# sThalham/PyraPose

Measured on AMD Instinct MI355X. Metric: images/sec 640x480 fwd+bwd (train step: fwd + losses + bwd + clipnorm-Adam), higher is better.
Workload: dtype bf16x3+f16c8

## Files before the change

include/pyrapose_hip.h:

```cpp
#ifndef PYRAPOSE_HIP_H
#define PYRAPOSE_HIP_H

#include <stddef.h>
#include <stdint.h>

#ifdef __cplusplus
extern "C" {
#endif

#define PP_OK 0
#define PP_ERR_ARG (-1)
#define PP_ERR_SHAPE (-2)
#define PP_ERR_ALIGN (-3)
#define PP_ERR_NOCTX (-4)
#define PP_ERR_UNSUPPORTED (-5)
#define PP_ERR_COMM (-6)

#define PP_MAX_SEG 5

typedef struct pp_ctx pp_ctx;

int pp_ctx_create(pp_ctx** out, int device, void* hip_stream);
void pp_ctx_destroy(pp_ctx* ctx);
int pp_ctx_set_stream(pp_ctx* ctx, void* hip_stream);
int pp_ctx_set_workspace(pp_ctx* ctx, void* device_buffer, size_t bytes);
int pp_row_block_list(pp_ctx* ctx, const float* x, int rows, int ld, int cols, unsigned char* flags, int* list);
int pp_row_block_list_planes(pp_ctx* ctx, const void* x_hi, const void* x_lo, int rows, int ld, int cols, unsigned char* flags, int* list);
int pp_row_block_list_planes_within(pp_ctx* ctx, const void* x_hi, const void* x_lo, int rows, int ld, int cols, const unsigned char* within,
                                    unsigned char* flags, int* list);
const char* pp_last_error_string(pp_ctx* ctx);
const char* pp_version(void);
int pp_device_info(pp_ctx* ctx, int* n_cu, char* name_host, int name_len);

typedef struct {
  int n_img;
  int n_seg;
  int h[PP_MAX_SEG];
  int w[PP_MAX_SEG];
} pp_rowspace;

typedef struct {
  pp_rowspace in;
  pp_rowspace out;
  int cin, cout;
  int kh, kw, stride;
  int pad_t, pad_l;
  int ld_x, ld_y, ld_w;
} pp_conv_desc;

int pp_conv2d_nhwc_fwd(pp_ctx* ctx, const pp_conv_desc* d, const float* x, const float* w,
                       const float* bias, const float* residual, int ld_res, int relu, float* y);

int pp_conv2d_nhwc_bwd_data(pp_ctx* ctx, const pp_conv_desc* d, const float* dy, const float* w,
                            const float* addend, int ld_add, const float* relu_src, int ld_rs, float* dx);

int pp_conv2d_nhwc_bwd_weight(pp_ctx* ctx, const pp_conv_desc* d, const float* x, const float* dy,
                              float* dw, float* dbias);

int pp_conv_split_weights_bf16x3(pp_ctx* ctx, const pp_conv_desc* d, const float* w, void* fwd_hi, void* fwd_lo,
                                 void* dgrad_hi, void* dgrad_lo);
typedef struct pp_split_job {
  const float* w;
  void* fwd_hi; void* fwd_lo; void* dg_hi; void* dg_lo;
  int taps, cin, cout, ld_w;
  int tile_begin, reserved;
} pp_split_job;
int pp_conv_split_weights_bf16x3_batch(pp_ctx* ctx, int n_jobs, const pp_split_job* jobs_dev, int total_tiles);
int pp_positive_row_blocks(pp_ctx* ctx, const pp_rowspace* rs, int A, int stride, const float* y_true, unsigned char* flags);
int pp_row_block_dilate(pp_ctx* ctx, const pp_conv_desc* d, const unsigned char* in_flags, unsigned char* out_flags);
int pp_split_planes_bf16x3(pp_ctx* ctx, size_t n, const float* src, void* hi, void* lo);
int pp_ctx_set_planes_format(pp_ctx* ctx, int fmt);
int pp_convert_planes(pp_ctx* ctx, size_t n, const void* src_hi, const void* src_lo, int src_fmt, void* dst_hi, void* dst_lo, int dst_fmt,
                      const float* scale2_dev, int scale_index, const void* relu_src_hi);
int pp_grad_scale_from_counts(pp_ctx* ctx, const int* counts_dev, int n_counts, float* scale2_dev);
int pp_grad_scale_from_counts_adj(pp_ctx* ctx, const int* counts_dev, int n_counts, float* scale2_dev, int log2_adjust);
int pp_split_planes_scaled_bf16x3(pp_ctx* ctx, size_t n, const float* src, void* hi, void* lo, const float* scale_dev);
int pp_ctx_set_grad_scale(pp_ctx* ctx, const float* scale2_dev);

typedef struct pp_conv_opts {
  void* capture_hi;
  void* capture_lo;
  const void* add_hi;
  const void* add_lo;
  const void* mask_hi;
  unsigned char* skip_flags;
  int* skip_list;
  const unsigned char* out_flags;
  int* out_list;
  int lazy_out;
  int lazy_in;
} pp_conv_opts;
#ifdef __cplusplus
static_assert(sizeof(pp_conv_opts) == 9 * sizeof(void*) + 2 * sizeof(int), "pp_conv_opts: pointers, then ints, no padding");
#else
_Static_assert(sizeof(pp_conv_opts) == 9 * sizeof(void*) + 2 * sizeof(int), "pp_conv_opts: pointers, then ints, no padding");
#endif

int pp_conv2d_nhwc_fwd_bf16x3(pp_ctx* ctx, const pp_conv_desc* d, const float* x, const void* x_hi, const void* x_lo,
                              const void* w_fwd_hi, const void* w_fwd_lo, const float* bias, const float* residual,
                              int ld_res, int relu, float* y, void* y_hi, void* y_lo, const pp_conv_opts* opts);
int pp_conv2d_nhwc_bwd_data_bf16x3(pp_ctx* ctx, const pp_conv_desc* d, const float* dy, const void* dy_hi,
                                   const void* dy_lo, const void* w_dgrad_hi, const void* w_dgrad_lo,
                                   const float* addend, int ld_add, const float* relu_src, int ld_rs, float* dx,
                                   void* dx_hi, void* dx_lo, const pp_conv_opts* opts);
int pp_conv2d_nhwc_bwd_weight_bf16x3(pp_ctx* ctx, const pp_conv_desc* d, const float* x, const float* dy,
                                     const void* x_hi, const void* x_lo, const void* dy_hi, const void* dy_lo,
                                     float* dw, float* dbias, const pp_conv_opts* opts);

#define PP_PLAN_FWD 0
#define PP_PLAN_BWD_DATA 1
#define PP_PLAN_BWD_WEIGHT 2
#define PP_PLAN_PLANES_IN 1u
#define PP_PLAN_PLANES_OUT 2u
#define PP_PLAN_F32_OUT 4u
#define PP_PLAN_CAPTURE 8u
#define PP_PLAN_LIST 16u
#define PP_PLAN_LAZY_IN 32u
#define PP_PLAN_LAZY_OUT 64u
int pp_conv_plan_text(const pp_conv_desc* d, int pass, unsigned forms, int planes_fmt, int n_cu, size_t ws_bytes, char* buf,
                      int buf_bytes);

typedef struct pp_comm pp_comm;
int pp_comm_available(void);
int pp_comm_unique_id(pp_ctx* ctx, void* id128);
int pp_comm_init(pp_ctx* ctx, int world, int rank, const void* id128, pp_comm** out);
int pp_comm_destroy(pp_comm* comm);
int pp_allreduce_bucket(pp_ctx* ctx, pp_comm* comm, float* buf, size_t count);
int pp_allreduce_counts(pp_ctx* ctx, pp_comm* comm, int* counts, int n);

int pp_maxpool3x3s2_fwd(pp_ctx* ctx, int n_img, int h, int w, int c, const float* x, int oh, int ow, float* y);
int pp_upsample_nearest_add_fwd(pp_ctx* ctx, int n_img, int sh, int sw, int th, int tw, int c,
                                const float* src, const float* other, float* out);
int pp_upsample_nearest_add_bwd(pp_ctx* ctx, int n_img, int sh, int sw, int th, int tw, int c,
                                const float* dtarget, const float* base, float* dsrc);
int pp_add_n(pp_ctx* ctx, size_t n, const float* a, const float* b, const float* c, float* out);
int pp_relu_fwd(pp_ctx* ctx, size_t n, const float* x, float* y);
typedef struct pp_tview {
  const float* f32;
  const void* hi;
  const void* lo;
} pp_tview;
int pp_add_n_v(pp_ctx* ctx, size_t n, const pp_tview* a, const pp_tview* b, const pp_tview* c, const pp_tview* out);
int pp_relu_fwd_v(pp_ctx* ctx, size_t n, const pp_tview* x, const pp_tview* y);
int pp_upsample_nearest_add_fwd_v(pp_ctx* ctx, int n_img, int sh, int sw, int th, int tw, int c, const pp_tview* src,
                                  const pp_tview* other, const pp_tview* out);
int pp_upsample_nearest_add_bwd_v(pp_ctx* ctx, int n_img, int sh, int sw, int th, int tw, int c, const pp_tview* dtarget,
                                  const pp_tview* base, const pp_tview* dsrc);
int pp_merge_planes_bf16x3(pp_ctx* ctx, size_t n, const void* hi, const void* lo, float* dst);
int pp_planes_stats(pp_ctx* ctx, const void* hi, const void* lo, long long rows, int ld, int cols, const unsigned char* within,
                    unsigned long long* stats5_dev);
int pp_pack_rgb_to_4(pp_ctx* ctx, size_t n_pixels, const float* x3, float* x4);
int pp_preprocess_caffe_u8(pp_ctx* ctx, int n_img, int H, int W, const int* sizes_hw_host, const unsigned char* images_u8,
                           float* x4);
int pp_warp_affine_u8(pp_ctx* ctx, int n_img, int H, int W, int channels, const double* mats_host, int interpolation, int border,
                      int cval, const unsigned char* src, unsigned char* dst);
int pp_resize_scale(int rows, int cols, int min_side, int max_side, double* scale);
int pp_resize_linear_u8(pp_ctx* ctx, int n_img, int SH, int SW, int channels, double scale, int DH, int DW, const unsigned char* src,
                        unsigned char* dst);
enum { PP_PHOTO_NONE = 0, PP_PHOTO_LUT = 1, PP_PHOTO_GRAY = 2, PP_PHOTO_HUESAT = 3, PP_PHOTO_BLEND = 4, PP_PHOTO_CONV = 5, PP_PHOTO_MEDIAN = 6,
       PP_PHOTO_BILATERAL = 7 };
typedef struct pp_photo_op {
  int kind;
  int k;
  int off0, off1;
  float f0, f1;
} pp_photo_op;
size_t pp_photo_workspace_bytes(int n_img, int H, int W);
int pp_photo_augment_u8(pp_ctx* ctx, int n_img, int H, int W, int channels, const int* op_offsets_host, const pp_photo_op* ops_host,
                        const unsigned char* pool_host, size_t pool_bytes, const unsigned char* pool_dev, const unsigned char* src,
                        unsigned char* dst, void* workspace, size_t workspace_bytes);
int pp_pack_rgb_to_4_padded(pp_ctx* ctx, int n_img, int H, int W, int Hp, int Wp, int pad, const float* x3, float* x4p);
int pp_preprocess_caffe_u8_padded(pp_ctx* ctx, int n_img, int H, int W, int Hp, int Wp, int pad, const int* sizes_hw_host,
                                  const unsigned char* images_u8, float* x4p);
int pp_stem7x7s2_fwd_bf16x3(pp_ctx* ctx, int n_img, int H, int W, int Hp, int Wp, const float* x4p, const void* w_hi,
                            const void* w_lo, int cout, const float* bias, int relu, float* y, int ld_y);

int pp_export_head(pp_ctx* ctx, const pp_rowspace* rs, int n_anchor, int n_val, const float* src, int ld,
                   int apply_sigmoid, float* out);

int pp_count_positives(pp_ctx* ctx, size_t rows_box, const float* y_box, size_t rows_cls, int c_cls,
                       const float* y_cls, size_t rows_mask, int c_mask, const float* y_mask, int* counts);
int pp_sigmoid_focal_fwd_bwd(pp_ctx* ctx, const pp_rowspace* rs, int n_anchor, int n_class,
                             const float* logits, int ld, const float* y_true, float alpha, float gamma,
                             const int* count, float loss_weight, float* loss_sum, float* dlogits);
int pp_orth_smoothl1_fwd_bwd(pp_ctx* ctx, const pp_rowspace* rs, int n_anchor, const float* pred, int ld,
                             const float* y_true, float weight, float sigma, const int* count,
                             float loss_weight, float* loss_sum, float* dpred);

typedef struct {
  long long offset;
  long long count;
  int ld;
  int trainable;
  long long scale_off;
// ... 178 lines not shown
```

pyrapose_amd/_lib.py:

```python
import ctypes as C
import os

_HERE = os.path.dirname(os.path.abspath(__file__))
LIB_PATH = os.path.join(_HERE, os.environ.get("PP_LIB") or "libpyrapose_hip.so")

PP_MAX_SEG = 5


class RowSpace(C.Structure):
    _fields_ = [("n_img", C.c_int), ("n_seg", C.c_int), ("h", C.c_int * PP_MAX_SEG), ("w", C.c_int * PP_MAX_SEG)]

    @classmethod
    def make(cls, n_img, shapes):
        rs = cls()
        rs.n_img = int(n_img)
        rs.n_seg = len(shapes)
        for i, (h, w) in enumerate(shapes):
            rs.h[i] = int(h)
            rs.w[i] = int(w)
        return rs

    def rows(self):
        return sum(self.n_img * self.h[i] * self.w[i] for i in range(self.n_seg))

# ... 13 lines not shown


class SplitJob(C.Structure):
    _fields_ = [("w", C.c_void_p), ("fwd_hi", C.c_void_p), ("fwd_lo", C.c_void_p), ("dg_hi", C.c_void_p), ("dg_lo", C.c_void_p),
                ("taps", C.c_int), ("cin", C.c_int), ("cout", C.c_int), ("ld_w", C.c_int), ("tile_begin", C.c_int), ("reserved", C.c_int)]


class TView(C.Structure):
    _fields_ = [("f32", C.c_void_p), ("hi", C.c_void_p), ("lo", C.c_void_p)]


class ConvOpts(C.Structure):
    _fields_ = [("capture_hi", C.c_void_p), ("capture_lo", C.c_void_p), ("add_hi", C.c_void_p), ("add_lo", C.c_void_p),
                ("mask_hi", C.c_void_p), ("skip_flags", C.c_void_p), ("skip_list", C.c_void_p), ("out_flags", C.c_void_p),
                ("out_list", C.c_void_p), ("lazy_out", C.c_int), ("lazy_in", C.c_int)]


def _load():
    if not os.path.exists(LIB_PATH):
        raise ImportError(
            "pyrapose_amd: %s not found. Build it with `python -c 'import __graft_entry__ as g; g.build()'` "
            "or `make -C pyrapose_amd/csrc`. There is no CPU fallback." % LIB_PATH)
    try:
        return C.CDLL(LIB_PATH)
    except OSError as e:
        raise ImportError("pyrapose_amd: cannot load %s: %s" % (LIB_PATH, e))


lib = _load()
if hasattr(lib, "pp_ctx_set_split_capture"):
    raise ImportError("pyrapose_amd: %s predates pp_conv_opts (it still exports pp_ctx_set_split_capture): rebuild it" % LIB_PATH)

_p = C.c_void_p
_i = C.c_int
_f = C.c_float
_d = C.c_double
_ll = C.c_longlong
_sz = C.c_size_t

_SIGS = {
    "pp_ctx_create": (_i, [C.POINTER(_p), _i, _p]),
    "pp_ctx_destroy": (None, [_p]),
    "pp_ctx_set_stream": (_i, [_p, _p]),
    "pp_last_error_string": (C.c_char_p, [_p]),
    "pp_version": (C.c_char_p, []),
    "pp_device_info": (_i, [_p, C.POINTER(_i), C.c_char_p, _i]),
    "pp_conv2d_nhwc_fwd": (_i, [_p, C.POINTER(ConvDesc), _p, _p, _p, _p, _i, _i, _p]),
    "pp_conv2d_nhwc_bwd_data": (_i, [_p, C.POINTER(ConvDesc), _p, _p, _p, _i, _p, _i, _p]),
    "pp_conv2d_nhwc_bwd_weight": (_i, [_p, C.POINTER(ConvDesc), _p, _p, _p, _p]),
    "pp_conv_split_weights_bf16x3": (_i, [_p, C.POINTER(ConvDesc), _p, _p, _p, _p, _p]),
    "pp_split_planes_bf16x3": (_i, [_p, _sz, _p, _p, _p]),
    "pp_ctx_set_planes_format": (_i, [_p, _i]),
    "pp_convert_planes": (_i, [_p, _sz, _p, _p, _i, _p, _p, _i, _p, _i, _p]),
    "pp_split_planes_scaled_bf16x3": (_i, [_p, _sz, _p, _p, _p, _p]),
    "pp_grad_scale_from_counts": (_i, [_p, _p, _i, _p]),
    "pp_grad_scale_from_counts_adj": (_i, [_p, _p, _i, _p, _i]),
    "pp_ctx_set_grad_scale": (_i, [_p, _p]),
    "pp_planes_stats": (_i, [_p, _p, _p, _ll, _i, _i, _p, _p]),
    "pp_comm_available": (_i, []),
    "pp_comm_unique_id": (_i, [_p, _p]),
    "pp_comm_init": (_i, [_p, _i, _i, _p, C.POINTER(_p)]),
    "pp_comm_destroy": (_i, [_p]),
    "pp_allreduce_bucket": (_i, [_p, _p, _p, C.c_size_t]),
    "pp_allreduce_counts": (_i, [_p, _p, _p, _i]),
    "pp_ctx_set_workspace": (_i, [_p, _p, C.c_size_t]),
    "pp_row_block_list": (_i, [_p, _p, _i, _i, _i, _p, _p]),
    "pp_positive_row_blocks": (_i, [_p, _p, _i, _i, _p, _p]),
    "pp_row_block_dilate": (_i, [_p, _p, _p, _p]),
    "pp_row_block_list_planes": (_i, [_p, _p, _p, _i, _i, _i, _p, _p]),
    "pp_row_block_list_planes_within": (_i, [_p, _p, _p, _i, _i, _i, _p, _p, _p]),
    "pp_add_n_v": (_i, [_p, _sz, C.POINTER(TView), C.POINTER(TView), C.POINTER(TView), C.POINTER(TView)]),
    "pp_relu_fwd_v": (_i, [_p, _sz, C.POINTER(TView), C.POINTER(TView)]),
    "pp_upsample_nearest_add_fwd_v": (_i, [_p, _i, _i, _i, _i, _i, _i, C.POINTER(TView), C.POINTER(TView), C.POINTER(TView)]),
    "pp_upsample_nearest_add_bwd_v": (_i, [_p, _i, _i, _i, _i, _i, _i, C.POINTER(TView), C.POINTER(TView), C.POINTER(TView)]),
    "pp_merge_planes_bf16x3": (_i, [_p, _sz, _p, _p, _p]),
    "pp_warp_affine_u8": (_i, [_p, _i, _i, _i, _i, C.POINTER(_d), _i, _i, _i, _p, _p]),
    "pp_photo_workspace_bytes": (_sz, [_i, _i, _i]),
    "pp_photo_augment_u8": (_i, [_p, _i, _i, _i, _i, _p, _p, _p, _sz, _p, _p, _p, _p, _sz]),
    "pp_resize_scale": (_i, [_i, _i, _i, _i, C.POINTER(_d)]),
    "pp_resize_linear_u8": (_i, [_p, _i, _i, _i, _i, _d, _i, _i, _p, _p]),
    "pp_conv_split_weights_bf16x3_batch": (_i, [_p, _i, _p, _i]),
    "pp_conv2d_nhwc_fwd_bf16x3": (_i, [_p, C.POINTER(ConvDesc), _p, _p, _p, _p, _p, _p, _p, _i, _i, _p, _p, _p, C.POINTER(ConvOpts)]),
    "pp_conv2d_nhwc_bwd_data_bf16x3": (_i, [_p, C.POINTER(ConvDesc), _p, _p, _p, _p, _p, _p, _i, _p, _i, _p, _p, _p, C.POINTER(ConvOpts)]),
    "pp_conv2d_nhwc_bwd_weight_bf16x3": (_i, [_p, C.POINTER(ConvDesc), _p, _p, _p, _p, _p, _p, _p, _p, C.POINTER(ConvOpts)]),
    "pp_conv_plan_text": (_i, [C.POINTER(ConvDesc), _i, C.c_uint, _i, _i, _sz, C.c_char_p, _i]),
    "pp_maxpool3x3s2_fwd": (_i, [_p, _i, _i, _i, _i, _p, _i, _i, _p]),
    "pp_upsample_nearest_add_fwd": (_i, [_p, _i, _i, _i, _i, _i, _i, _p, _p, _p]),
    "pp_upsample_nearest_add_bwd": (_i, [_p, _i, _i, _i, _i, _i, _i, _p, _p, _p]),
    "pp_add_n": (_i, [_p, _sz, _p, _p, _p, _p]),
    "pp_relu_fwd": (_i, [_p, C.c_size_t, _p, _p]),
    "pp_preprocess_caffe_u8": (_i, [_p, _i, _i, _i, C.POINTER(C.c_int), _p, _p]),
    "pp_preprocess_caffe_u8_padded": (_i, [_p, _i, _i, _i, _i, _i, _i, C.POINTER(C.c_int), _p, _p]),
    "pp_pack_rgb_to_4_padded": (_i, [_p, _i, _i, _i, _i, _i, _i, _p, _p]),
    "pp_stem7x7s2_fwd_bf16x3": (_i, [_p, _i, _i, _i, _i, _i, _p, _p, _p, _i, _p, _i, _p, _i]),
    "pp_pack_rgb_to_4": (_i, [_p, _sz, _p, _p]),
    "pp_export_head": (_i, [_p, C.POINTER(RowSpace), _i, _i, _p, _i, _i, _p]),
    "pp_count_positives": (_i, [_p, _sz, _p, _sz, _i, _p, _sz, _i, _p, _p]),
    "pp_sigmoid_focal_fwd_bwd": (_i, [_p, C.POINTER(RowSpace), _i, _i, _p, _i, _p, _f, _f, _p, _f, _p, _p]),
    "pp_orth_smoothl1_fwd_bwd": (_i, [_p, C.POINTER(RowSpace), _i, _p, _i, _p, _f, _f, _p, _f, _p, _p]),
    "pp_optimizer_create": (_i, [_p, C.POINTER(_p), C.POINTER(ParamDesc), _i, _ll]),
    "pp_optimizer_destroy": (None, [_p]),
    "pp_grad_global_norm": (_i, [_p, _p, _p, _p, _p, _p, _p]),
    "pp_adam_step_clipnorm": (_i, [_p, _p, _p, _p, _p, _p, _p, _p, _p, _f, _f, _f, _f, _f, _ll]),
    "pp_generate_base_anchors_host": (_i, [_i, C.POINTER(_f), _i, C.POINTER(_f), _i, C.POINTER(_d)]),
    "pp_anchors_shift_f64": (_i, [_p, _i, C.POINTER(_i), C.POINTER(_i), C.POINTER(_i), _i, C.POINTER(_d), _p]),
    "pp_anchors_shift_f32": (_i, [_p, _i, C.POINTER(_i), C.POINTER(_i), C.POINTER(_i), _i, C.POINTER(_d), _p]),
    "pp_compute_overlap_f64": (_i, [_p, _i, _p, _i, _p, _p]),
    "pp_compute_gt_annotations": (_i, [_p, _i, _p, _i, _p, _d, _d, _p, _p]),
    "pp_anchor_targets": (_i, [_p, _i, _p, _i, C.POINTER(_i), _p, _p, _p, _p, _p, _i, _i, C.POINTER(_i), C.POINTER(_i), _i, _d, _d,
                               _i, _i, _p, _p, _p]),
    "pp_project_box3d_host": (_i, [C.POINTER(_d), C.POINTER(_d), C.POINTER(_d), C.POINTER(_d)]),
    "pp_pil_nearest_index_host": (_i, [_i, _i, C.POINTER(_i)]),
    "pp_box3d_decode": (_i, [_p, _i, _i, _p, _p, _p]),
    "pp_score_threshold_compact": (_i, [_p, _i, _i, _i, _p, _f, _i, _p, _p]),
    "pp_filter_workspace_bytes": (_sz, [_i, _i, _i]),
    "pp_pose_error_workspace_bytes": (_sz, [_i, _i]),
    "pp_filter_detections": (_i, [_p, _i, _i, _p, _p, _p, _f, _f, _i, _p, _p, _p, _p, _p]),
    "pp_pose_add_f64": (_i, [_p, _i, _i, _p, _p, _p, _p, _p, _p, _p]),
    "pp_pose_adi_f64": (_i, [_p, _i, _i, _p, _p, _p, _p, _p, _p, _p]),
    "pp_filter_detections_batch": (_i, [_p, _i, _i, _i, _p, _p, _p, _f, _f, _i, _p, _p, _p, _p, _p]),
    "pp_render_workspace_bytes": (_sz, [_i, _i, _i, _i, _i]),
    "pp_render_depth_f32": (_i, [_p, _i, _i, _p, _i, _p, _p, _p, _p, _i, _i, _d, _d, _p, _sz, _p]),
    "pp_render_rgbd_workspace_bytes": (_sz, [_i, _i, _i, _i, _i]),
    "pp_render_rgbd": (_i, [_p, _i, _i, _p, _p, _p, _i, _p, _p, _p, _p, _i, _i, _d, _d, _i, _d, C.POINTER(_d), C.POINTER(_d), _p, _sz,
                            _p, _p, _p, _p]),
    "pp_render_rgbd_tex_workspace_bytes": (_sz, [_i, _i, _i, _i, _i, _i, _i]),
    "pp_render_rgbd_tex": (_i, [_p, _i, _i, _p, _p, _p, _i, _i, _i, _i, _p, _i, _p, _p, _p, _p, _i, _i, _d, _d, _i, _d, C.POINTER(_d),
                                C.POINTER(_d), _p, _sz, _p, _p, _p, _p]),
    "pp_scene_compose_u8": (_i, [_p, _i, _i, C.POINTER(_i), _p, _i, _i, _p, _p, _p, C.POINTER(C.c_ubyte), _i, _p]),
    "pp_vsd_workspace_bytes": (_sz, [_i, _i, _i]),
    "pp_vsd_f64": (_i, [_p, _i, _i, _i, _p, _ll, _p, _p, _p, _d, _d, _i, _p, _p, _p, _p]),
    "pp_vsd_multi_workspace_bytes": (_sz, [_i, _i, _i, _i]),
    "pp_vsd_multi_f64": (_i, [_p, _i, _i, _i, _p, _ll, _p, _p, _p, _d, _i, C.POINTER(_d), _i, _i, _p, _p, _p, _p, _p, _p]),
    "pp_scene_gt_workspace_bytes": (_sz, [_i, _i, _i]),
    "pp_scene_gt_info": (_i, [_p, _i, _i, C.POINTER(_i), _p, _i, _i, _i, _i, _i, _i, _p, _p, _p, _ll, _d, _p, _sz, _p, _p, _p, _p, _p,
                              _p, _p]),
    "pp_pose_reproj_f64": (_i, [_p, _i, _i, _p, _p, _p, _p, _p, _p, _p, _p]),
    "pp_pose_sym_workspace_bytes": (_sz, [_i, _i, _i]),
    "pp_pose_mssd_f64": (_i, [_p, _i, _i, _i, _p, _p, _p, _p, _p, _p, _p, _p, _p, _p]),
    "pp_pose_mspd_f64": (_i, [_p, _i, _i, _i, _p, _p, _p, _p, _p, _p, _p, _p, _p, _p, _p]),
    "pp_pnp_ransac_workspace_bytes": (_sz, [_i, _i]),
    "pp_pnp_ransac_f64": (_i, [_p, _i, _p, _i, _p, _p, _p, _i, _d, C.c_ulonglong, _i, _p, _p, _p, _p, _p, _p]),
    "pp_cloud_from_depth_workspace_bytes": (_sz, [_i, _i]),
    "pp_cloud_from_depth_f64": (_i, [_p, _i, _i, _p, _p, _i, _i, _p, _p, _d, _d, _d, _d, _d, _i, _p, _p, _p]),
    "pp_voxel_workspace_bytes": (_sz, [_i]),
    "pp_voxel_keys_f64": (_i, [_p, _i, _p, _d, _p, _p]),
    "pp_voxel_means_f64": (_i, [_p, _i, _p, _p, _p, _i, _p, _p, _p]),
    "pp_estimate_normals_workspace_bytes": (_sz, [_i, _i]),
    "pp_estimate_normals_f64": (_i, [_p, _i, _p, _d, _i, _p, _p, _p]),
    "pp_icp_workspace_bytes": (_sz, [_i, _i]),
    "pp_icp_f64": (_i, [_p, _i, _p, _p, _i, _p, _p, _p, _p, _d, _i, _d, _d, _i, _p, _sz, _p, _p, _p, _p, _p, _p, _p]),
    "pp_vote_stats_workspace_bytes": (_sz, [_i, _i]),
    "pp_vote_stats_f64": (_i, [_p, _i, _p, _i, _p, _i, _p, _p, _i, _d, _p, _p, _p, _p, _p, _p, _p]),
    "pp_pnp_refine_weighted_workspace_bytes": (_sz, [_i, _i]),
    "pp_pnp_refine_weighted_f64": (_i, [_p, _i, _p, _i, _p, _p, _p, _p, _p, _p, _i, _d, _d, _d, _p, _p, _p, _p, _p, _p, _p, _p, _p]),
    "pp_vote_cluster_workspace_bytes": (_sz, [_i, _i, _i, _i]),
    "pp_vote_cluster": (_i, [_p, _i, _i, _i, _i, _p, _p, _p, _p, _d, _i, _i, _i, _p, _p, _p, _p, _p, _p, _p]),
    "pp_pts_diameter_workspace_bytes": (_sz, [_i]),
    "pp_pts_diameter_f64": (_i, [_p, _i, _p, _p, _sz, _p, _p]),
    "pp_farthest_points_workspace_bytes": (_sz, [_i]),
    "pp_farthest_points_f64": (_i, [_p, _i, _i, _p, C.POINTER(_i), _p, _i, _i, _p, _p, _p, _sz, _p]),
    "pp_det_match": (_i, [_p, _i, _i, _i, _i, _p, _p, _p, _p, _p, _p, C.POINTER(_i), _p, _i, C.POINTER(_d), _i, _p, _p, _p]),
    "pp_det_pr_curve": (_i, [_p, _i, _i, _i, _ll, _p, _p, _p, _p, _p, _p, _p, _p, _p]),
    "pp_det_ap": (_i, [_p, _i, _i, _i, _p, _p, _p, _p, _i, _p, _p]),
}

# ... 26 lines not shown
```

pyrapose_amd/csrc/conv3.hip:

```cpp
#include "conv_common.h"
#include "conv4.h"

#define PP_CAT_(a, b) a##b
#define PP_CAT(a, b) PP_CAT_(a, b)
#if PP_FMT == 1
#define PP_API(name) PP_CAT(name, _fmt1)
#else
#define PP_API(name) PP_CAT(name, _fmt0)
#endif
namespace {
#include "planes_fmt.h"

#include "conv3_shared.h"

#ifndef PP_EPI_GF
#define PP_EPI_GF 4
#endif

template <int TM, int TN, bool AP, bool OP>
__global__ __launch_bounds__(256, (TM * TN >= 8) ? 2 : ((TM * TN == 4) ? 3 : 4)) void igemm3_kernel(
    const IgemmParams p, const float* __restrict__ g_src, const uint4* __restrict__ g_ahi, const uint4* __restrict__ g_alo,
    const uint4* __restrict__ g_whi, const uint4* __restrict__ g_wlo,
    const float* __restrict__ g_bias, const float* __restrict__ g_addend, const float* __restrict__ g_mask,
    float* __restrict__ g_out, uint2* __restrict__ g_ohi, uint2* __restrict__ g_olo, int w_rows, int w_ld8) {
// ... 48 lines not shown
        ra[i][1] = s4[1];
      } else {
        ra[i][0] = make_float4(0.f, 0.f, 0.f, 0.f);
        ra[i][1] = make_float4(0.f, 0.f, 0.f, 0.f);
      }
    }
#pragma unroll
    for (int i = 0; i < TN; ++i) {
      const int n = n0 + r0 + 64 * i;
      if (n < w_rows) {
        const long long off = ((long long)tap * w_rows + n) * w_ld8 + (red0 >> 3) + oct;
        rbh[i] = g_whi[off];
        rbl[i] = g_wlo[off];
      } else {
        rbh[i] = make_uint4(0u, 0u, 0u, 0u);
        rbl[i] = make_uint4(0u, 0u, 0u, 0u);
      }
    }
  };
  auto advance = [&]() {
    red0 += BK;
    if (red0 >= p.Cred) {
      red0 = 0;
      ++tap;
      ++tx;
      if (tx == p.kw) { tx = 0; ++ty; }
      set_tap();
    }
  };
  auto store_step = [&]() {
#pragma unroll
    for (int i = 0; i < TM; ++i) {
      uint4 hi, lo;
      if (AP) {
        hi = rah[i];
        lo = ral[i];
      } else {
        split8(ra[i][0], ra[i][1], &hi, &lo);
      }
      const int slot = oct * BM + ((r0 + 64 * i + 2 * oct) & (BM - 1));
      Ahi[slot] = hi;
      Alo[slot] = lo;
    }
#pragma unroll
    for (int i = 0; i < TN; ++i) {
      const int slot = oct * BN + ((r0 + 64 * i + 2 * oct) & (BN - 1));
      Bhi[slot] = rbh[i];
      Blo[slot] = rbl[i];
    }
  };

  floatx16 acc[TM][TN];
#pragma unroll
  for (int a = 0; a < TM; ++a)
#pragma unroll
    for (int b = 0; b < TN; ++b)
#pragma unroll
      for (int r = 0; r < 16; ++r) acc[a][b][r] = 0.f;

  const int il = lane & 31, h = lane >> 5;

  set_tap();
  load_step();
  store_step();
  __syncthreads();

  for (int step = 0; step < n_steps; ++step) {
    const bool more = step + 1 < n_steps;
    if (more) {
      advance();
      load_step();
    }
    mma_step<TM, TN, BM, BN, 0>(acc, Ahi, Alo, Bhi, Blo, wm * 32 * TM + il, wn * 32 * TN + il, h);
    __syncthreads();
    if (more) {
      store_step();
      __syncthreads();
    }
  }

  epilogue3<TM, TN, OP>(p, acc, smem, m0, n0, tid, wm, wn, il, h, g_bias, g_addend, g_mask, g_out, g_ohi, g_olo);
}

template <int TM, int TN, bool AP, bool OP, bool SC = false, bool RL = false>
__global__ __launch_bounds__(256, (TM * TN >= 8) ? 2 : ((TM * TN == 4) ? 3 : 4)) void igemm3f_kernel(
    const IgemmParams p, const void* __restrict__ g_a0, const void* __restrict__ g_a1, unsigned a_bytes,
    const void* __restrict__ g_whi, const void* __restrict__ g_wlo, unsigned w_bytes,
    const float* __restrict__ g_bias, const float* __restrict__ g_addend, const float* __restrict__ g_mask,
    float* __restrict__ g_out, uint2* __restrict__ g_ohi, uint2* __restrict__ g_olo, int w_rows, int w_ld8, int splits,
    float* __restrict__ g_ws, const int* __restrict__ g_rl = nullptr, const unsigned char* __restrict__ g_srcflags = nullptr) {
  constexpr int BM = 64 * TM, BN = 64 * TN, BK = 32, NO = BK / 8;
  constexpr int SMEM_U4 = 2 * NO * (BM + BN);
  constexpr int ES = 4;
  __shared__ __attribute__((aligned(16))) uint4 smem[SMEM_U4];
  uint4* Ahi = smem;
  uint4* Alo = Ahi + NO * BM;
  uint4* Bhi = Alo + NO * BM;
  uint4* Blo = Bhi + NO * BN;

  const int tid = threadIdx.x, lane = tid & 63, wave = tid >> 6;
  const int wm = wave >> 1, wn = wave & 1;
  int n_wg = (int)gridDim.x;
  if (RL) {
    n_wg = ((g_rl[0] + BM / 32 - 1) / (BM / 32)) * p.n_tiles_n * splits;
    if ((int)blockIdx.x >= n_wg) return;
  }
  const int lbs = xcd_remap((int)blockIdx.x, n_wg);
  const int split = lbs % splits, lb = lbs / splits;
  const int tile_n = lb % p.n_tiles_n, tile_m = lb / p.n_tiles_n;
  const int m0 = tile_m * BM, n0 = tile_n * BN;
  int rl_blk[BM / 32];
  if (RL) {
    const int count = g_rl[0];
#pragma unroll
    for (int j = 0; j < BM / 32; ++j) {
      const int e = tile_m * (BM / 32) + j;
      rl_blk[j] = e < count ? g_rl[1 + e] * 32 : ((p.M + 31) & ~31);
    }
  }
  const int oct = tid & 3, r0 = tid >> 2;
  const int n_taps = p.kh * p.kw;
  const int steps_per_tap = p.Cred / BK;
  const int all_steps = n_taps * steps_per_tap;
  const int s_begin = (int)((long long)all_steps * split / splits), s_end = (int)((long long)all_steps * (split + 1) / splits);

  const __amdgpu_buffer_rsrc_t rs_a0 = __builtin_amdgcn_make_buffer_rsrc(const_cast<void*>(g_a0), 0, a_bytes, 0x00020000);
  const __amdgpu_buffer_rsrc_t rs_a1 = __builtin_amdgcn_make_buffer_rsrc(const_cast<void*>(AP ? g_a1 : g_a0), 0, AP ? a_bytes - 16 : a_bytes, 0x00020000);
  const __amdgpu_buffer_rsrc_t rs_wh = __builtin_amdgcn_make_buffer_rsrc(const_cast<void*>(g_whi), 0, w_bytes, 0x00020000);
  const __amdgpu_buffer_rsrc_t rs_wl = __builtin_amdgcn_make_buffer_rsrc(const_cast<void*>(g_wlo), 0, w_bytes, 0x00020000);

  int a_base[TM], a_pitch[TM];
  unsigned a_valid[TM];
#pragma unroll
  for (int i = 0; i < TM; ++i) {
    const int t_row = r0 + 64 * i;
    const RowPos r = decode_row(p, RL ? rl_blk[t_row >> 5] + (t_row & 31) : m0 + t_row);
    a_base[i] = ((r.rowbase + r.ybase * r.SW + r.xbase) * p.ld_src + 8 * oct) * ES;
    a_pitch[i] = p.tsign * r.SW * p.ld_src * ES;
    unsigned v = 0;
    int t = 0;
    for (int ty = 0; ty < p.kh; ++ty)
      for (int tx = 0; tx < p.kw; ++tx, ++t) {
        const int sy = r.ybase + ty * p.tsign, sx = r.xbase + tx * p.tsign;
        bool ok = r.ok && (unsigned)sy < (unsigned)r.SH && (unsigned)sx < (unsigned)r.SW;
        if (RL && g_srcflags && ok) ok = g_srcflags[(r.rowbase + sy * r.SW + sx) >> 5] != 0;
        if (ok) v |= 1u << t;
      }
    a_valid[i] = v;
  }
  const int x_pitch = p.tsign * p.ld_src * ES;
  int b_base[TN];
#pragma unroll
  for (int i = 0; i < TN; ++i) {
    const int n = n0 + r0 + 64 * i;
    b_base[i] = n < w_rows ? (n * w_ld8 + oct) * 16 : PP_BUF_OOB;
  }
  const int b_tap = w_rows * w_ld8 * 16;

  float4 ra[TM][2];
  uint4 rah[TM], ral[TM];
  uint4 rbh[TN], rbl[TN];
  int tap = s_begin / steps_per_tap, red0 = (s_begin - tap * steps_per_tap) * BK;
  int ty = tap / p.kw, tx = tap - ty * p.kw;

  auto load_step = [&]() {
    const int a_uni = tx * x_pitch + red0 * ES;
#pragma unroll
    for (int i = 0; i < TM; ++i) {
      int vo = a_base[i] + __mul24(ty, a_pitch[i]) + a_uni;
      vo = ((a_valid[i] >> tap) & 1u) ? vo : PP_BUF_OOB;
      if (AP) {
        rah[i] = buf_load16(rs_a0, vo, 0);
        ral[i] = buf_load16(rs_a1, vo, 0);
      } else {
        const uint4 q0 = buf_load16(rs_a0, vo, 0), q1 = buf_load16(rs_a0, vo + 16, 0);
        ra[i][0] = *reinterpret_cast<const float4*>(&q0);
        ra[i][1] = *reinterpret_cast<const float4*>(&q1);
      }
    }
    const int b_uni = ((p.w_ty0 + p.w_tstep * ty) * p.w_kw + p.w_tx0 + p.w_tstep * tx) * b_tap + (red0 >> 3) * 16;
#pragma unroll
    for (int i = 0; i < TN; ++i) {
      rbh[i] = buf_load16(rs_wh, b_base[i], b_uni);
      rbl[i] = buf_load16(rs_wl, b_base[i], b_uni);
    }
  };
  auto advance = [&](bool more) {
    red0 += BK;
    const bool wrap = red0 >= p.Cred;
    red0 = wrap ? 0 : red0;
    tap += wrap ? 1 : 0;
    tx += wrap ? 1 : 0;
    const bool wx = tx == p.kw;
    tx = wx ? 0 : tx;
    ty += wx ? 1 : 0;
    red0 = more ? red0 : 0;
    tap = more ? tap : 0;
    tx = more ? tx : 0;
    ty = more ? ty : 0;
  };
  auto split_step = [&]() {
    if (!AP) {
#pragma unroll
      for (int i = 0; i < TM; ++i) split8(ra[i][0], ra[i][1], &rah[i], &ral[i]);
    }
  };
  auto store_step = [&]() {
#pragma unroll
    for (int i = 0; i < TM; ++i) {
      const int slot = oct * BM + ((r0 + 64 * i + 2 * oct) & (BM - 1));
      Ahi[slot] = rah[i];
      Alo[slot] = ral[i];
    }
#pragma unroll
    for (int i = 0; i < TN; ++i) {
      const int slot = oct * BN + ((r0 + 64 * i + 2 * oct) & (BN - 1));
      Bhi[slot] = rbh[i];
      Blo[slot] = rbl[i];
    }
  };

  floatx16 acc[TM][TN];
#pragma unroll
  for (int a = 0; a < TM; ++a)
#pragma unroll
    for (int b = 0; b < TN; ++b)
#pragma unroll
      for (int r = 0; r < 16; ++r) acc[a][b][r] = 0.f;

  const int il = lane & 31, h = lane >> 5;

  load_step();
  split_step();
  store_step();
  __syncthreads();

  for (int step = s_begin; step < s_end; ++step) {
    advance(step + 1 < s_end);
    load_step();
    __builtin_amdgcn_sched_barrier(0);
    mma_step<TM, TN, BM, BN, 2>(acc, Ahi, Alo, Bhi, Blo, wm * 32 * TM + il, wn * 32 * TN + il, h);
    split_step();
    __syncthreads();
    store_step();
    __syncthreads();
  }
  if (splits > 1) {
    float* slice = g_ws + (long long)split * (RL ? (((long long)p.M + 31) & ~31ll) : (long long)p.M) * p.ld_out;
#pragma unroll
    for (int a = 0; a < TM; ++a)
#pragma unroll
      for (int r = 0; r < 16; ++r) {
        const int trow = wm * 32 * TM + a * 32 + (r & 3) + 8 * (r >> 2) + 4 * h;
        const int m = m0 + trow;
        const bool row_ok = RL ? (rl_blk[trow >> 5] < p.M) : (m < p.M);
#pragma unroll
        for (int b = 0; b < TN; ++b) {
          const int co = n0 + wn * 32 * TN + b * 32 + il;
          if (row_ok && co < ((p.Nout + 3) & ~3)) slice[(long long)m * p.ld_out + co] = acc[a][b][r];
        }
      }
    return;
  }
  epilogue3<TM, TN, OP, PP_EPI_GF, SC, false, RL>(p, acc, smem, m0, n0, tid, wm, wn, il, h, g_bias, g_addend, g_mask, g_out, g_ohi, g_olo, rl_blk);
}

template <int TM, int TN, bool CAP, bool AP = false, bool OP = false>
__global__ __launch_bounds__(256, (TM * TN >= 8) ? 2 : ((TM * TN == 4) ? 3 : 4)) void igemm3x_kernel(
    const IgemmParams p, const void* __restrict__ g_a, const void* __restrict__ g_a1, unsigned a_bytes, const void* __restrict__ g_whi,
    const void* __restrict__ g_wlo, unsigned w_bytes, const float* __restrict__ g_bias, const float* __restrict__ g_addend,
    const float* __restrict__ g_mask, float* __restrict__ g_out, uint2* __restrict__ g_ohi, uint2* __restrict__ g_olo, int w_rows, int w_ld8,
    int splits, float* __restrict__ g_ws, void* __restrict__ g_chi, void* __restrict__ g_clo, const unsigned char* __restrict__ g_flags,
    int skip_halo) {
  static_assert(!(CAP && AP), "split capture is for f32 operands");
  constexpr int ES = 4;
  constexpr int BM = 64 * TM, BN = 64 * TN, BK = 32, NO = BK / 8;
  constexpr int AP1 = NO * BM + 1;
  constexpr int SMEM_U4 = 2 * AP1 + 2 * NO * BN;
  __shared__ __attribute__((aligned(16))) uint4 smem[SMEM_U4];
  uint4* Ahi = smem;
  uint4* Alo = Ahi + AP1;
  uint4* Bhi = Alo + AP1;
  uint4* Blo = Bhi + NO * BN;

  const int tid = threadIdx.x, lane = tid & 63, wave = tid >> 6;
  const int wm = wave >> 1, wn = wave & 1;
  const int lbs = xcd_remap((int)blockIdx.x, (int)gridDim.x);
  const int split = lbs % splits, lb = lbs / splits;
  const int tile_n = lb % p.n_tiles_n, tile_m = lb / p.n_tiles_n;
  const int m0 = p.m_off + tile_m * (BM - 2) - 1, n0 = tile_n * BN;
  const int oct = tid & 3, r0 = tid >> 2;
  const int il = lane & 31, h = lane >> 5;
  const int n_chunks = p.Cred / BK;
  const int all_groups = p.kh * n_chunks;
  const int g_begin = (int)((long long)all_groups * split / splits);
  int g_end = (int)((long long)all_groups * (split + 1) / splits);
  if (g_flags) {
    int lo = m0 - skip_halo, hi = m0 + BM - 1 + skip_halo;
    lo = lo < 0 ? 0 : lo;
    hi = hi > p.M - 1 ? p.M - 1 : hi;
    int any = 0;
    for (int b = lo >> 5; b <= (hi >> 5); ++b) any |= g_flags[b];
    g_end = any ? g_end : g_begin;
  }

  const __amdgpu_buffer_rsrc_t rs_a = __builtin_amdgcn_make_buffer_rsrc(const_cast<void*>(g_a), 0, a_bytes, 0x00020000);
  const __amdgpu_buffer_rsrc_t rs_a1 = __builtin_amdgcn_make_buffer_rsrc(const_cast<void*>(AP ? g_a1 : g_a), 0, AP ? a_bytes - 16 : a_bytes, 0x00020000);
  const __amdgpu_buffer_rsrc_t rs_wh = __builtin_amdgcn_make_buffer_rsrc(const_cast<void*>(g_whi), 0, w_bytes, 0x00020000);
  const __amdgpu_buffer_rsrc_t rs_wl = __builtin_amdgcn_make_buffer_rsrc(const_cast<void*>(g_wlo), 0, w_bytes, 0x00020000);

  int s_base[TM], s_pitch[TM];
#pragma unroll
  for (int i = 0; i < TM; ++i) {
    const int q = m0 + r0 + 64 * i;
    const RowPos r = decode_row(p, q < 0 ? 0 : q);
    const bool ok = q >= 0 && r.ok;
    const int x = r.xbase - p.off_x;
    s_base[i] = ((r.rowbase + r.ybase * r.SW + x) * p.ld_src + 8 * oct) * ES;
    int v = 0;
    for (int ty = 0; ty < p.kh; ++ty)
      if (ok && (unsigned)(r.ybase + ty * p.tsign) < (unsigned)r.SH) v |= 1 << ty;
    s_pitch[i] = (p.tsign * r.SW * p.ld_src * ES) | v;
  }
  unsigned f_valid[(TM + 1) / 2];
#pragma unroll
  for (int a = 0; a < (TM + 1) / 2; ++a) f_valid[a] = 0;
#pragma unroll
  for (int a = 0; a < TM; ++a) {
    const int q = m0 + wm * 32 * TM + a * 32 + il;
    const RowPos r = decode_row(p, q < 0 ? 0 : q);
    unsigned v = 0;
    int t = 0;
    for (int ty = 0; ty < p.kh; ++ty)
      for (int tx = 0; tx < 3; ++tx, ++t) {
        const int sy = r.ybase + ty * p.tsign, sx = r.xbase + tx * p.tsign;
        if (q >= 0 && r.ok && (unsigned)sy < (unsigned)r.SH && (unsigned)sx < (unsigned)r.SW) v |= 1u << t;
      }
    f_valid[a >> 1] |= v << (16 * (a & 1));
  }
  int b_base[TN];
#pragma unroll
  for (int i = 0; i < TN; ++i) {
    const int n = n0 + r0 + 64 * i;
    b_base[i] = n < w_rows ? (n * w_ld8 + oct) * 16 : PP_BUF_OOB;
  }
  const int b_tap = w_rows * w_ld8 * 16;

// ... 819 lines not shown
      break;
    case PP_IGEMM4X:
      if constexpr (TM == 2 && TN == 2) {
        auto go4 = [&](auto v) {
          hipLaunchKernelGGL((igemm4x_kernel<true, decltype(v)::value>), grid, dim3(512), 0, st, p, a.ahi, a.alo, a_bytes, a.whi, a.wlo, w_bytes, p.bias,
                             p.addend, p.mask_src, p.out, (uint2*)a.ohi, (uint2*)a.olo, a.w_rows, a.w_ld8);
        };
        if (pl.variant == 0) go4(std::integral_constant<int, 0>{});
        else if (pl.variant == 2) go4(std::integral_constant<int, 2>{});
        else if (pl.variant == 3) go4(std::integral_constant<int, 3>{});
        else if (pl.variant == 4) go4(std::integral_constant<int, 4>{});
        else if (pl.variant == 9) go4(std::integral_constant<int, 9>{});
        else go4(std::integral_constant<int, 1>{});
        if (pl.tail_splits > 1) {
          IgemmParams q = p;
          q.m_off = pl.tail_m_off;
          hipLaunchKernelGGL((igemm3x_kernel<TM, TN, false, true, false>), dim3(pl.tail_grid), wg, 0, st, q, a.ahi, a.alo, a_bytes, a.whi, a.wlo, w_bytes,
                             q.bias, q.addend, q.mask_src, q.out, no_hi, no_lo, a.w_rows, a.w_ld8, pl.tail_splits, a.ws, nullptr, nullptr,
                             (const unsigned char*)nullptr, pl.skip_halo);
          launch_splitk_finish(st, q, pl.tail_splits, a.ws, pl.finish_blocks, a.ohi, a.olo);
        }
      }
      return;
    case PP_IGEMM4X2:
      if constexpr (TM == 2 && TN == 2)
        hipLaunchKernelGGL((igemm4x_kernel<true, 1, 2>), grid, wg, 0, st, p, a.ahi, a.alo, a_bytes, a.whi, a.wlo, w_bytes, p.bias, p.addend, p.mask_src,
                           p.out, (uint2*)a.ohi, (uint2*)a.olo, a.w_rows, a.w_ld8);
      return;
    case PP_IGEMM4P:
      if constexpr (TM == 2 && TN == 2)
        PP_API(pp4_launch_igemm4p)(st, p, a.ahi, a.whi, a.wlo, a.w_rows, a.w_ld8, a.ohi, a.olo, splits, ws, pl.grid, pl.stages);
      break;
    case PP_IGEMM3X_PP:
      hipLaunchKernelGGL((igemm3x_kernel<TM, TN, false, true, true>), grid, wg, 0, st, p, a.ahi, a.alo, a_bytes, a.whi, a.wlo, w_bytes, p.bias, p.addend,
                         p.mask_src, p.out, (uint2*)a.ohi, (uint2*)a.olo, a.w_rows, a.w_ld8, splits, ws, nullptr, nullptr, a.flags, pl.skip_halo);
      break;
    case PP_IGEMM3X_PF:
      hipLaunchKernelGGL((igemm3x_kernel<TM, TN, false, true, false>), grid, wg, 0, st, p, a.ahi, a.alo, a_bytes, a.whi, a.wlo, w_bytes, p.bias, p.addend,
                         p.mask_src, p.out, no_hi, no_lo, a.w_rows, a.w_ld8, splits, ws, nullptr, nullptr, a.flags, pl.skip_halo);
      break;
    case PP_IGEMM3X_FP:
      if constexpr (TM <= 2)
        hipLaunchKernelGGL((igemm3x_kernel<TM, TN, false, false, true>), grid, wg, 0, st, p, (const void*)p.src, nullptr, a_bytes, a.whi, a.wlo, w_bytes,
                           p.bias, p.addend, p.mask_src, p.out, (uint2*)a.ohi, (uint2*)a.olo, a.w_rows, a.w_ld8, splits, ws, nullptr, nullptr, a.flags,
                           pl.skip_halo);
      break;
    case PP_IGEMM3X_FF:
      if constexpr (TM <= 2)
        hipLaunchKernelGGL((igemm3x_kernel<TM, TN, false>), grid, wg, 0, st, p, (const void*)p.src, nullptr, a_bytes, a.whi, a.wlo, w_bytes, p.bias,
                           p.addend, p.mask_src, p.out, no_hi, no_lo, a.w_rows, a.w_ld8, splits, ws, nullptr, nullptr, a.flags, pl.skip_halo);
      break;
    default: {
      void *const ohi = splits > 1 ? nullptr : a.ohi, *const olo = splits > 1 ? nullptr : a.olo;
      auto go = [&](auto ap, auto op) {
        constexpr bool AP = decltype(ap)::value, OP = decltype(op)::value;
        if (pl.family == PP_IGEMM3F)
          hipLaunchKernelGGL((igemm3f_kernel<TM, TN, AP, OP>), grid, wg, 0, st, p, AP ? a.ahi : (const void*)p.src, AP ? a.alo : nullptr, a_bytes, a.whi,
                             a.wlo, w_bytes, p.bias, p.addend, p.mask_src, p.out, (uint2*)ohi, (uint2*)olo, a.w_rows, a.w_ld8, splits, ws);
        else
          hipLaunchKernelGGL((igemm3_kernel<TM, TN, AP, OP>), grid, wg, 0, st, p, p.src, (const uint4*)(AP ? a.ahi : nullptr),
                             (const uint4*)(AP ? a.alo : nullptr), (const uint4*)a.whi, (const uint4*)a.wlo, p.bias, p.addend, p.mask_src, p.out,
                             (uint2*)ohi, (uint2*)olo, a.w_rows, a.w_ld8);
      };
      if (a.ahi && ohi) go(std::true_type{}, std::true_type{});
      else if (a.ahi) go(std::true_type{}, std::false_type{});
      else if (ohi) go(std::false_type{}, std::true_type{});
      else go(std::false_type{}, std::false_type{});
    }
  }
  if (pl.finish_blocks) launch_splitk_finish(st, p, splits, a.ws, pl.finish_blocks, a.ohi, a.olo);
}

static void dispatch3(pp_ctx* ctx, IgemmParams& p, const Igemm3Args& a) {
  const PpIgemmFacts f = igemm3_facts(ctx, p, a);
  const PpIgemmPlan pl = pp_plan_igemm(f);
  pp_plan_debug(f, pl);
  if (pl.tm == 4) launch_igemm3<4, 2>(ctx->stream, p, a, pl);
  else if (pl.tm == 2 && pl.tn == 2) launch_igemm3<2, 2>(ctx->stream, p, a, pl);
  else if (pl.tm == 1 && pl.tn == 2) launch_igemm3<1, 2>(ctx->stream, p, a, pl);
  else if (pl.tm == 2 && pl.tn == 1) launch_igemm3<2, 1>(ctx->stream, p, a, pl);
  else launch_igemm3<1, 1>(ctx->stream, p, a, pl);
}

static void dispatch3_rowlist(pp_ctx* ctx, IgemmParams& p, const Igemm3Args& a, int tm, const unsigned char* dy_flags, unsigned char* out_flags,
                              int* out_list, bool fill) {
  PpIgemmFacts f = igemm3_facts(ctx, p, a);
  f.listed = true;
  f.listed_tm = tm;
  const PpIgemmPlan pl = pp_plan_igemm(f);
  if (tm == 2) launch_igemm3_rowlist<2, 2>(ctx->stream, p, a, pl, dy_flags, out_flags, out_list, fill);
  else launch_igemm3_rowlist<1, 2>(ctx->stream, p, a, pl, dy_flags, out_flags, out_list, fill);
}


}
extern "C" int PP_API(pp_conv2d_nhwc_fwd_bf16x3)(pp_ctx* ctx, const pp_conv_desc* d, const float* x, const void* x_hi, const void* x_lo,
                                         const void* w_hi, const void* w_lo, const float* bias, const float* residual, int ld_res,
                                         int relu, float* y, void* y_hi, void* y_lo, const pp_conv_opts* opts) {
  PP_REQUIRE_CTX(ctx);
  int rc = pp_conv_opts_take(ctx, opts, PP_OPT_CAPTURE | PP_OPT_ADD | PP_OPT_OUT, "pp_conv2d_nhwc_fwd_bf16x3");
  if (rc) return rc;
  void *const chi = opts->capture_hi, *const clo = opts->capture_lo;
  const void *const ep_ah = opts->add_hi, *const ep_al = opts->add_lo;
  rc = check_desc(ctx, d, "pp_conv2d_nhwc_fwd_bf16x3");
  PP_CHECK_ARG(ctx, !(ep_ah && residual), PP_ERR_ARG, "pp_conv2d_nhwc_fwd_bf16x3: residual given both as f32 and as planes");
  PP_CHECK_ARG(ctx, !ep_ah || (ld_res % 4 == 0 && ld_res >= ((d->cout + 3) & ~3)), PP_ERR_SHAPE, "pp_conv2d_nhwc_fwd_bf16x3: residual planes");
  if (rc) return rc;
  PP_CHECK_ARG(ctx, !chi || (x && !x_hi && pp_is_packed(chi, clo)), PP_ERR_ARG, "pp_conv2d_nhwc_fwd_bf16x3: split capture needs the f32 operand");
  PP_CHECK_ARG(ctx, (x || (x_hi && x_lo)) && w_hi && w_lo && (y || (y_hi && y_lo)), PP_ERR_ARG, "pp_conv2d_nhwc_fwd_bf16x3: null tensor");
  PP_CHECK_ARG(ctx, (x_hi == nullptr) == (x_lo == nullptr), PP_ERR_ARG, "pp_conv2d_nhwc_fwd_bf16x3: x_hi and x_lo go together");
  PP_CHECK_ARG(ctx, d->cin % 32 == 0 && d->ld_x % 8 == 0, PP_ERR_SHAPE, "pp_conv2d_nhwc_fwd_bf16x3: cin %d must be a multiple of 32, ld_x of 8", d->cin);
  PP_CHECK_ARG(ctx, pp_is_packed(x_hi, x_lo) && pp_is_packed(y_hi, y_lo), PP_ERR_ALIGN,
               "pp_conv2d_nhwc_fwd_bf16x3: planes must be packed (lo = hi + 16 bytes, 16-byte aligned)");
  PP_CHECK_ARG(ctx, !y_hi || (d->cout % 8 == 0 && d->ld_y % 8 == 0), PP_ERR_SHAPE, "pp_conv2d_nhwc_fwd_bf16x3: output planes need cout, ld_y %% 8 == 0");
  PP_CHECK_ARG(ctx, !ep_ah || (ld_res % 8 == 0 && d->cout % 8 == 0), PP_ERR_SHAPE, "pp_conv2d_nhwc_fwd_bf16x3: residual planes need cout, ld_res %% 8 == 0");
  PP_CHECK_ARG(ctx, (!x || pp_is_aligned16(x)) && pp_is_aligned16(w_hi) && pp_is_aligned16(w_lo) && (!y || pp_is_aligned16(y)), PP_ERR_ALIGN,
               "pp_conv2d_nhwc_fwd_bf16x3: tensors must be 16-byte aligned");
  PP_CHECK_ARG(ctx, !residual || (ld_res % 4 == 0 && ld_res >= ((d->cout + 3) & ~3) && pp_is_aligned16(residual)), PP_ERR_SHAPE,
               "pp_conv2d_nhwc_fwd_bf16x3: residual");
  PP_CHECK_ARG(ctx, !bias || pp_is_aligned16(bias), PP_ERR_ALIGN, "pp_conv2d_nhwc_fwd_bf16x3: bias alignment");
  IgemmParams p;
  memset(&p, 0, sizeof(p));
  p.src = x; p.out = y; p.bias = bias; p.addend = residual; p.mask_src = nullptr;
  p.add_hi = ep_ah; p.add_lo = ep_al;
  igemm_geometry_fwd(ctx, d, p);
  p.ld_add = ld_res; p.ld_mask = 0;
  p.relu = relu;
  PP_CHECK_ARG(ctx, (y_hi == nullptr) == (y_lo == nullptr) && (!y_hi || (d->ld_y % 4 == 0 && pp_is_aligned16(y_hi) && pp_is_aligned16(y_lo))),
               PP_ERR_ARG, "pp_conv2d_nhwc_fwd_bf16x3: output planes");
  const Igemm3Args a = {x_hi, x_lo, w_hi, w_lo, d->cout, d->cin / 8, y_hi, y_lo, chi, clo, nullptr, ctx->ws};
  if (opts->out_flags) {
    const bool ok = fwd_listed_ok(d, igemm3_facts(ctx, p, a), residual != nullptr || ep_ah != nullptr);
    PP_CHECK_ARG(ctx, ok, PP_ERR_SHAPE, "pp_conv2d_nhwc_fwd_bf16x3: out_flags needs a 3x3 stride-1 'same' conv on plane-stored input");
    dispatch3_rowlist(ctx, p, a, 2, nullptr, const_cast<unsigned char*>(opts->out_flags) ,
                      opts->out_list, false);
    PP_CHECK_LAUNCH(ctx, "pp_conv2d_nhwc_fwd_bf16x3");
    return PP_OK;
  }
  dispatch3(ctx, p, a);
  PP_CHECK_LAUNCH(ctx, "pp_conv2d_nhwc_fwd_bf16x3");
  return PP_OK;
}
namespace {

}
extern "C" int PP_API(pp_row_block_dilate)(pp_ctx* ctx, const pp_conv_desc* d, const unsigned char* in_flags, unsigned char* out_flags) {
  PP_REQUIRE_CTX(ctx);
  int rc = check_desc(ctx, d, "pp_row_block_dilate");
  if (rc) return rc;
  PP_CHECK_ARG(ctx, in_flags && out_flags && in_flags != out_flags, PP_ERR_ARG, "pp_row_block_dilate: two distinct flag buffers");
  IgemmParams p;
  memset(&p, 0, sizeof(p));
  p.n_seg = d->in.n_seg;
  fill_segs(ctx, d, true, p.seg, &p.M, &p.src_rows);
  const bool same = d->stride == 1 && d->kh == 3 && d->kw == 3 && segs_same_grid(p.seg, p.n_seg);
  PP_CHECK_ARG(ctx, same, PP_ERR_SHAPE, "pp_row_block_dilate: 3x3 stride-1 conv on an unchanged grid");
  const int nb = (p.M + 31) / 32;
  hipLaunchKernelGGL(rl_dilate_kernel, dim3((unsigned)((nb + 255) / 256)), dim3(256), 0, ctx->stream, p, in_flags, out_flags, nb);
  PP_CHECK_LAUNCH(ctx, "pp_row_block_dilate");
  return PP_OK;
}
namespace {

}
extern "C" int PP_API(pp_stem7x7s2_fwd_bf16x3)(pp_ctx* ctx, int n_img, int H, int W, int Hp, int Wp, const float* x4p, const void* w_hi,
                                       const void* w_lo, int cout, const float* bias, int relu, float* y, int ld_y) {
  PP_REQUIRE_CTX(ctx);
  PP_CHECK_ARG(ctx, x4p && w_hi && w_lo && y && pp_is_aligned16(x4p) && pp_is_aligned16(y) && pp_is_aligned16(w_hi) && pp_is_aligned16(w_lo),
               PP_ERR_ARG, "pp_stem7x7s2_fwd_bf16x3: null / unaligned tensor");
  PP_CHECK_ARG(ctx, n_img > 0 && H > 0 && W > 0 && Hp >= H + 6 && Wp >= W + 8 && Wp % 2 == 0 && cout > 0 && ld_y % 4 == 0 && ld_y >= ((cout + 3) & ~3),
               PP_ERR_SHAPE, "pp_stem7x7s2_fwd_bf16x3: bad geometry");
  const int OH = (H + 6 - 7) / 2 + 1, OW = (W + 6 - 7) / 2 + 1;
  IgemmParams p;
  memset(&p, 0, sizeof(p));
  p.src = x4p; p.out = y; p.bias = bias;
  p.ld_src = 4; p.ld_out = ld_y;
  p.relu = relu;
  p.n_seg = 1;
  p.seg[0].row_begin = 0; p.seg[0].src_row_begin = 0;
  p.seg[0].OH = OH; p.seg[0].OW = OW; p.seg[0].SH = Hp; p.seg[0].SW = Wp;
  p.M = n_img * OH * OW;
  p.src_rows = (long long)n_img * Hp * Wp;
  p.Cred = 32; p.Nout = cout; p.w_tap_rows = 32;
  p.kh = 7; p.kw = 1;
  p.mul = 2; p.tsign = 1; p.off_y = 0; p.off_x = 0; p.div = 1;
  p.w_ty0 = 0; p.w_tx0 = 0; p.w_tstep = 1; p.w_kw = 1; p.w_taps = 7;
  const Igemm3Args a = {nullptr, nullptr, w_hi, w_lo, cout, 4, nullptr, nullptr, nullptr, nullptr, nullptr, ctx->ws};
  PP_CHECK_ARG(ctx, pp_igemm_fast_ok(igemm3_facts(ctx, p, a)), PP_ERR_SHAPE, "pp_stem7x7s2_fwd_bf16x3: frame too large for 31-bit offsets");
  dispatch3(ctx, p, a);
  PP_CHECK_LAUNCH(ctx, "pp_stem7x7s2_fwd_bf16x3");
  return PP_OK;
}
namespace {

}
extern "C" int PP_API(pp_conv2d_nhwc_bwd_data_bf16x3)(pp_ctx* ctx, const pp_conv_desc* d, const float* dy, const void* dy_hi, const void* dy_lo,
                                              const void* w_hi, const void* w_lo, const float* addend, int ld_add,
                                              const float* relu_src, int ld_rs, float* dx, void* dx_hi, void* dx_lo,
                                              const pp_conv_opts* opts) {
  PP_REQUIRE_CTX(ctx);
  int rc = pp_conv_opts_take(ctx, opts, PP_OPT_CAPTURE | PP_OPT_ADD | PP_OPT_MASK | PP_OPT_SKIP | PP_OPT_LAZY_OUT | PP_OPT_LAZY_IN,
                             "pp_conv2d_nhwc_bwd_data_bf16x3");
  if (rc) return rc;
  void *const chi = opts->capture_hi, *const clo = opts->capture_lo;
  unsigned char* const skip_flags = opts->skip_flags;
  const bool skip_scratch_ok = skip_flags != nullptr && opts->skip_list != nullptr;
  const void *const ep_ah = opts->add_hi, *const ep_al = opts->add_lo, *const ep_mh = opts->mask_hi;
  rc = check_desc(ctx, d, "pp_conv2d_nhwc_bwd_data_bf16x3");
  PP_CHECK_ARG(ctx, !(ep_ah && addend) && !(ep_mh && relu_src), PP_ERR_ARG,
               "pp_conv2d_nhwc_bwd_data_bf16x3: addend / relu_src given both as f32 and as planes");
  PP_CHECK_ARG(ctx, (!ep_ah || (ld_add >= d->cin && ld_add % 4 == 0)) && (!ep_mh || (ld_rs >= d->cin && ld_rs % 4 == 0)), PP_ERR_SHAPE,
               "pp_conv2d_nhwc_bwd_data_bf16x3: addend / relu_src planes");
  if (rc) return rc;
  PP_CHECK_ARG(ctx, !chi || (dy && !dy_hi && pp_is_packed(chi, clo)), PP_ERR_ARG, "pp_conv2d_nhwc_bwd_data_bf16x3: split capture needs the f32 operand");
  PP_CHECK_ARG(ctx, (dy || (dy_hi && dy_lo)) && w_hi && w_lo && (dx || (dx_hi && dx_lo)), PP_ERR_ARG, "pp_conv2d_nhwc_bwd_data_bf16x3: null tensor");
  PP_CHECK_ARG(ctx, (dy_hi == nullptr) == (dy_lo == nullptr) && d->ld_y % 8 == 0, PP_ERR_ARG, "pp_conv2d_nhwc_bwd_data_bf16x3: planes / ld_y");
  PP_CHECK_ARG(ctx, pp_is_packed(dy_hi, dy_lo) && pp_is_packed(dx_hi, dx_lo), PP_ERR_ALIGN,
               "pp_conv2d_nhwc_bwd_data_bf16x3: planes must be packed (lo = hi + 16 bytes, 16-byte aligned)");
  PP_CHECK_ARG(ctx, (!dx_hi || (d->cin % 8 == 0 && d->ld_x % 8 == 0)) && (!ep_ah || ld_add % 8 == 0) && (!ep_mh || ld_rs % 8 == 0), PP_ERR_SHAPE,
               "pp_conv2d_nhwc_bwd_data_bf16x3: planes need channel counts and leading dimensions %% 8 == 0");
  const int cred = (d->cout + 31) / 32 * 32;
  PP_CHECK_ARG(ctx, d->cin % 16 == 0 && d->ld_y >= cred && d->ld_y % 4 == 0, PP_ERR_SHAPE,
               "pp_conv2d_nhwc_bwd_data_bf16x3: dy needs ld_y >= %d (cout rounded up to 32, zero padded)", cred);
  PP_CHECK_ARG(ctx, (!dy || pp_is_aligned16(dy)) && pp_is_aligned16(w_hi) && pp_is_aligned16(w_lo) && (!dx || pp_is_aligned16(dx)), PP_ERR_ALIGN,
               "pp_conv2d_nhwc_bwd_data_bf16x3: tensors must be 16-byte aligned");
  PP_CHECK_ARG(ctx, (!addend || (ld_add >= d->cin && ld_add % 4 == 0 && pp_is_aligned16(addend))) &&
                        (!relu_src || (ld_rs >= d->cin && ld_rs % 4 == 0 && pp_is_aligned16(relu_src))),
               PP_ERR_SHAPE, "pp_conv2d_nhwc_bwd_data_bf16x3: addend / relu_src");
  IgemmParams p;
  memset(&p, 0, sizeof(p));
  p.src = dy; p.out = dx; p.bias = nullptr; p.addend = addend; p.mask_src = relu_src;
  p.add_hi = ep_ah; p.add_lo = ep_al; p.mask_hi = ep_mh;
  igemm_geometry_bwd_data(ctx, d, p);
  p.ld_add = ld_add; p.ld_mask = ld_rs;
  p.relu = 0;
  PP_CHECK_ARG(ctx, (dx_hi == nullptr) == (dx_lo == nullptr) && (!dx_hi || (d->ld_x % 4 == 0 && pp_is_aligned16(dx_hi) && pp_is_aligned16(dx_lo))),
               PP_ERR_ARG, "pp_conv2d_nhwc_bwd_data_bf16x3: output planes");
  const Igemm3Args a = {dy_hi, dy_lo, w_hi, w_lo, d->cin, cred / 8, dx_hi, dx_lo, chi, clo, skip_flags, ctx->ws};
  DgradRoute route;
  dgrad_route(d, p, igemm3_facts(ctx, p, a), skip_scratch_ok, &route);
  PP_CHECK_ARG(ctx, !opts->lazy_in || route.listed, PP_ERR_ARG,
               "pp_conv2d_nhwc_bwd_data_bf16x3: dy was declared lazy (unwritten outside its flagged blocks) but the listed-block launch "
               "does not apply to this call");
  const int nb = (p.M + 31) / 32;
  if (skip_scratch_ok && !route.listed) PP_HIP(ctx, hipMemsetAsync(skip_flags + nb, 1, (size_t)nb, ctx->stream));
  const Igemm3Args ac = {dy_hi, dy_lo, w_hi, w_lo, d->cin, cred / 8, dx_hi, dx_lo, nullptr, nullptr, nullptr, ctx->ws};
  if (route.classes && chi) split_capture_pass(ctx->stream, p, chi, clo);
  dgrad_launches(
      route, p,
      [&](IgemmParams& q, bool is_class, bool listed) {
        if (listed) dispatch3_rowlist(ctx, q, a, route.listed_tm, skip_flags, skip_flags + nb, opts->skip_list + nb + 1, !opts->lazy_out);
        else dispatch3(ctx, q, is_class ? ac : a);
      },
      [&](IgemmParams& q) {
        hipLaunchKernelGGL(class_fill_kernel, dim3(pp_finish_blocks(q.M, q.Nout, pp_cus(ctx->n_cu))), dim3(256), 0, ctx->stream, q, addend, relu_src,
                           dx, dx_hi, dx_lo);
      });
  PP_CHECK_LAUNCH(ctx, "pp_conv2d_nhwc_bwd_data_bf16x3");
  return PP_OK;
}
namespace {

typedef short shortx4 __attribute__((ext_vector_type(4)));


template <int TM, int TN, bool AP>
__global__ __launch_bounds__(256, (TM * TN == 4) ? 2 : 3) void wgrad3_kernel(const Wgrad3Params p, const float* __restrict__ g_src,
                                                                            const float* __restrict__ g_dy,
                                                                            const uint4* __restrict__ g_xhi, const uint4* __restrict__ g_xlo,
                                                                            const uint4* __restrict__ g_dhi, const uint4* __restrict__ g_dlo,
                                                                            float* __restrict__ g_dw, float* __restrict__ g_dbias) {
  constexpr int BM = 64 * TM, BN = 64 * TN, BK = 32;
  constexpr int PA = BM + 32, PB = BN + 32;
  __shared__ __attribute__((aligned(16))) unsigned short smem[2 * BK * (PA + PB)];
  unsigned short* Xhi = smem;
  unsigned short* Xlo = Xhi + BK * PA;
  unsigned short* Ghi = Xlo + BK * PA;
  unsigned short* Glo = Ghi + BK * PB;

  const int tid = threadIdx.x, lane = tid & 63, wave = tid >> 6;
  const float inv_g = p.inv_scale ? *p.inv_scale : 1.f;
  const int wm = wave >> 1, wn = wave & 1;
  int b = xcd_remap((int)blockIdx.x, (int)gridDim.x);
  const int tile_n = b % p.n_tiles_n;
  b /= p.n_tiles_n;
  const int tile_k = b % p.n_tiles_k;
  const int split = b / p.n_tiles_k;
  const int tap = tile_k / p.k_tiles_per_tap;
  const int ci0 = (tile_k - tap * p.k_tiles_per_tap) * BM;
  const int ty = tap / p.kw, tx = tap - ty * p.kw;
  const int n0 = tile_n * BN;
  const int m_begin = split * p.rows_per_split;
  const int m_end = min(p.M, m_begin + p.rows_per_split);
  const int n_steps = (m_end - m_begin + BK - 1) / BK;

  const int prow = tid >> 3, q8 = tid & 7;
  constexpr int QA = BM / 32, QB = BN / 32;
  struct WRow { int m, n, y, x, seg_end, sb, OH, OW, SH, SW; } w;
  auto decode = [&](int m) {
    w.m = m;
    int rbeg = p.seg[0].row_begin;
    w.sb = p.seg[0].src_row_begin; w.OH = p.seg[0].OH; w.OW = p.seg[0].OW; w.SH = p.seg[0].SH; w.SW = p.seg[0].SW;
    w.seg_end = p.n_seg > 1 ? p.seg[1].row_begin : p.M;
    for (int s = 1; s < p.n_seg; ++s) {
      if (m >= p.seg[s].row_begin) {
        rbeg = p.seg[s].row_begin; w.sb = p.seg[s].src_row_begin; w.OH = p.seg[s].OH; w.OW = p.seg[s].OW;
        w.SH = p.seg[s].SH; w.SW = p.seg[s].SW;
        w.seg_end = (s + 1 < p.n_seg) ? p.seg[s + 1].row_begin : p.M;
      }
    }
    const int local = m < p.M ? m - rbeg : 0;
    const int hw = w.OH * w.OW;
    w.n = local / hw;
    const int rem = local - w.n * hw;
    w.y = rem / w.OW;
    w.x = rem - w.y * w.OW;
  };
  decode(m_begin + prow);

  constexpr int OA = (BM / 64 > 0) ? BM / 64 : 1, OB = (BN / 64 > 0) ? BN / 64 : 1;
  float4 ra[QA], rb[QB];
  uint4 pah[OA], pal[OA], pbh[OB], pbl[OB];
  float4 bsum[QB];
#pragma unroll
  for (int j = 0; j < QB; ++j) bsum[j] = make_float4(0.f, 0.f, 0.f, 0.f);
  const bool do_bias = (g_dbias != nullptr) && (tile_k == 0);

  auto load_step = [&]() {
    const int sy = w.y * p.stride + ty - p.pad_t;
    const int sx = w.x * p.stride + tx - p.pad_l;
    const bool in_rng = w.m < m_end;
    const bool ok = in_rng && ((unsigned)sy < (unsigned)w.SH) && ((unsigned)sx < (unsigned)w.SW);
    const long long xrow = (long long)(w.sb + w.n * w.SH * w.SW + sy * w.SW + sx) * p.ld_src + ci0;
    if (AP) {
#pragma unroll
      for (int j = 0; j < OA; ++j) {
        const long long o8 = 2 * ((xrow >> 3) + q8 + 8 * j);
        pah[j] = ok ? g_xhi[o8] : make_uint4(0u, 0u, 0u, 0u);
        pal[j] = ok ? g_xlo[o8] : make_uint4(0u, 0u, 0u, 0u);
      }
#pragma unroll
      for (int j = 0; j < OB; ++j) {
// ... 501 lines not shown
```

pyrapose_amd/csrc/conv3_dispatch.hip:

```cpp
#include "conv_common.h"

extern "C" int pp_row_block_list_fmt0(pp_ctx* ctx, const float* x, int rows, int ld, int cols, unsigned char* flags, int* list);
extern "C" int pp_row_block_list_fmt1(pp_ctx* ctx, const float* x, int rows, int ld, int cols, unsigned char* flags, int* list);
extern "C" int pp_row_block_list_planes_within_fmt0(pp_ctx* ctx, const void* x_hi, const void* x_lo, int rows, int ld, int cols, const unsigned char* within, unsigned char* flags, int* list);
extern "C" int pp_row_block_list_planes_within_fmt1(pp_ctx* ctx, const void* x_hi, const void* x_lo, int rows, int ld, int cols, const unsigned char* within, unsigned char* flags, int* list);
extern "C" int pp_row_block_list_planes_fmt0(pp_ctx* ctx, const void* x_hi, const void* x_lo, int rows, int ld, int cols, unsigned char* flags, int* list);
extern "C" int pp_row_block_list_planes_fmt1(pp_ctx* ctx, const void* x_hi, const void* x_lo, int rows, int ld, int cols, unsigned char* flags, int* list);
extern "C" int pp_split_planes_bf16x3_fmt0(pp_ctx* ctx, size_t n, const float* src, void* hi, void* lo);
extern "C" int pp_split_planes_bf16x3_fmt1(pp_ctx* ctx, size_t n, const float* src, void* hi, void* lo);
extern "C" int pp_split_planes_scaled_bf16x3_fmt0(pp_ctx* ctx, size_t n, const float* src, void* hi, void* lo, const float* scale_dev);
extern "C" int pp_split_planes_scaled_bf16x3_fmt1(pp_ctx* ctx, size_t n, const float* src, void* hi, void* lo, const float* scale_dev);
extern "C" int pp_grad_scale_from_counts_fmt0(pp_ctx* ctx, const int* counts_dev, int n_counts, float* scale2_dev);
extern "C" int pp_grad_scale_from_counts_adj_fmt0(pp_ctx* ctx, const int* counts_dev, int n_counts, float* scale2_dev, int log2_adjust);
extern "C" int pp_grad_scale_from_counts_adj_fmt1(pp_ctx* ctx, const int* counts_dev, int n_counts, float* scale2_dev, int log2_adjust);
extern "C" int pp_grad_scale_from_counts_fmt1(pp_ctx* ctx, const int* counts_dev, int n_counts, float* scale2_dev);
extern "C" int pp_conv_split_weights_bf16x3_batch_fmt0(pp_ctx* ctx, int n_jobs, const pp_split_job* jobs_dev, int total_tiles);
extern "C" int pp_conv_split_weights_bf16x3_batch_fmt1(pp_ctx* ctx, int n_jobs, const pp_split_job* jobs_dev, int total_tiles);
extern "C" int pp_conv_split_weights_bf16x3_fmt0(pp_ctx* ctx, const pp_conv_desc* d, const float* w, void* fwd_hi, void* fwd_lo, void* dgrad_hi, void* dgrad_lo);
extern "C" int pp_conv_split_weights_bf16x3_fmt1(pp_ctx* ctx, const pp_conv_desc* d, const float* w, void* fwd_hi, void* fwd_lo, void* dgrad_hi, void* dgrad_lo);
extern "C" int pp_conv2d_nhwc_fwd_bf16x3_fmt0(pp_ctx* ctx, const pp_conv_desc* d, const float* x, const void* x_hi, const void* x_lo, const void* w_fwd_hi, const void* w_fwd_lo, const float* bias, const float* residual, int ld_res, int relu, float* y, void* y_hi, void* y_lo, const pp_conv_opts* opts);
extern "C" int pp_conv2d_nhwc_fwd_bf16x3_fmt1(pp_ctx* ctx, const pp_conv_desc* d, const float* x, const void* x_hi, const void* x_lo, const void* w_fwd_hi, const void* w_fwd_lo, const float* bias, const float* residual, int ld_res, int relu, float* y, void* y_hi, void* y_lo, const pp_conv_opts* opts);
extern "C" int pp_row_block_dilate_fmt0(pp_ctx* ctx, const pp_conv_desc* d, const unsigned char* in_flags, unsigned char* out_flags);
extern "C" int pp_row_block_dilate_fmt1(pp_ctx* ctx, const pp_conv_desc* d, const unsigned char* in_flags, unsigned char* out_flags);
extern "C" int pp_stem7x7s2_fwd_bf16x3_fmt0(pp_ctx* ctx, int n_img, int H, int W, int Hp, int Wp, const float* x4p, const void* w_hi, const void* w_lo, int cout, const float* bias, int relu, float* y, int ld_y);
extern "C" int pp_stem7x7s2_fwd_bf16x3_fmt1(pp_ctx* ctx, int n_img, int H, int W, int Hp, int Wp, const float* x4p, const void* w_hi, const void* w_lo, int cout, const float* bias, int relu, float* y, int ld_y);
extern "C" int pp_conv2d_nhwc_bwd_data_bf16x3_fmt0(pp_ctx* ctx, const pp_conv_desc* d, const float* dy, const void* dy_hi, const void* dy_lo, const void* w_dgrad_hi, const void* w_dgrad_lo, const float* addend, int ld_add, const float* relu_src, int ld_rs, float* dx, void* dx_hi, void* dx_lo, const pp_conv_opts* opts);
extern "C" int pp_conv2d_nhwc_bwd_data_bf16x3_fmt1(pp_ctx* ctx, const pp_conv_desc* d, const float* dy, const void* dy_hi, const void* dy_lo, const void* w_dgrad_hi, const void* w_dgrad_lo, const float* addend, int ld_add, const float* relu_src, int ld_rs, float* dx, void* dx_hi, void* dx_lo, const pp_conv_opts* opts);
extern "C" int pp_conv2d_nhwc_bwd_weight_bf16x3_fmt0(pp_ctx* ctx, const pp_conv_desc* d, const float* x, const float* dy, const void* x_hi, const void* x_lo, const void* dy_hi, const void* dy_lo, float* dw, float* dbias, const pp_conv_opts* opts);
extern "C" int pp_conv2d_nhwc_bwd_weight_bf16x3_fmt1(pp_ctx* ctx, const pp_conv_desc* d, const float* x, const float* dy, const void* x_hi, const void* x_lo, const void* dy_hi, const void* dy_lo, float* dw, float* dbias, const pp_conv_opts* opts);

extern "C" int pp_row_block_list(pp_ctx* ctx, const float* x, int rows, int ld, int cols, unsigned char* flags, int* list) {
  return (ctx && ctx->planes_fmt == 1) ? pp_row_block_list_fmt1(ctx, x, rows, ld, cols, flags, list) : pp_row_block_list_fmt0(ctx, x, rows, ld, cols, flags, list);
}
extern "C" int pp_row_block_list_planes_within(pp_ctx* ctx, const void* x_hi, const void* x_lo, int rows, int ld, int cols, const unsigned char* within, unsigned char* flags, int* list) {
  return (ctx && ctx->planes_fmt == 1) ? pp_row_block_list_planes_within_fmt1(ctx, x_hi, x_lo, rows, ld, cols, within, flags, list) : pp_row_block_list_planes_within_fmt0(ctx, x_hi, x_lo, rows, ld, cols, within, flags, list);
}
extern "C" int pp_row_block_list_planes(pp_ctx* ctx, const void* x_hi, const void* x_lo, int rows, int ld, int cols, unsigned char* flags, int* list) {
  return (ctx && ctx->planes_fmt == 1) ? pp_row_block_list_planes_fmt1(ctx, x_hi, x_lo, rows, ld, cols, flags, list) : pp_row_block_list_planes_fmt0(ctx, x_hi, x_lo, rows, ld, cols, flags, list);
}
extern "C" int pp_split_planes_bf16x3(pp_ctx* ctx, size_t n, const float* src, void* hi, void* lo) {
  return (ctx && ctx->planes_fmt == 1) ? pp_split_planes_bf16x3_fmt1(ctx, n, src, hi, lo) : pp_split_planes_bf16x3_fmt0(ctx, n, src, hi, lo);
}
extern "C" int pp_split_planes_scaled_bf16x3(pp_ctx* ctx, size_t n, const float* src, void* hi, void* lo, const float* scale_dev) {
  return (ctx && ctx->planes_fmt == 1) ? pp_split_planes_scaled_bf16x3_fmt1(ctx, n, src, hi, lo, scale_dev) : pp_split_planes_scaled_bf16x3_fmt0(ctx, n, src, hi, lo, scale_dev);
}
extern "C" int pp_grad_scale_from_counts(pp_ctx* ctx, const int* counts_dev, int n_counts, float* scale2_dev) {
  return (ctx && ctx->planes_fmt == 1) ? pp_grad_scale_from_counts_fmt1(ctx, counts_dev, n_counts, scale2_dev) : pp_grad_scale_from_counts_fmt0(ctx, counts_dev, n_counts, scale2_dev);
}
extern "C" int pp_grad_scale_from_counts_adj(pp_ctx* ctx, const int* counts_dev, int n_counts, float* scale2_dev, int log2_adjust) {
  return (ctx && ctx->planes_fmt == 1) ? pp_grad_scale_from_counts_adj_fmt1(ctx, counts_dev, n_counts, scale2_dev, log2_adjust) : pp_grad_scale_from_counts_adj_fmt0(ctx, counts_dev, n_counts, scale2_dev, log2_adjust);
}
extern "C" int pp_conv_split_weights_bf16x3_batch(pp_ctx* ctx, int n_jobs, const pp_split_job* jobs_dev, int total_tiles) {
  return (ctx && ctx->planes_fmt == 1) ? pp_conv_split_weights_bf16x3_batch_fmt1(ctx, n_jobs, jobs_dev, total_tiles) : pp_conv_split_weights_bf16x3_batch_fmt0(ctx, n_jobs, jobs_dev, total_tiles);
}
extern "C" int pp_conv_split_weights_bf16x3(pp_ctx* ctx, const pp_conv_desc* d, const float* w, void* fwd_hi, void* fwd_lo, void* dgrad_hi, void* dgrad_lo) {
  return (ctx && ctx->planes_fmt == 1) ? pp_conv_split_weights_bf16x3_fmt1(ctx, d, w, fwd_hi, fwd_lo, dgrad_hi, dgrad_lo) : pp_conv_split_weights_bf16x3_fmt0(ctx, d, w, fwd_hi, fwd_lo, dgrad_hi, dgrad_lo);
}
extern "C" int pp_conv2d_nhwc_fwd_bf16x3(pp_ctx* ctx, const pp_conv_desc* d, const float* x, const void* x_hi, const void* x_lo, const void* w_fwd_hi, const void* w_fwd_lo, const float* bias, const float* residual, int ld_res, int relu, float* y, void* y_hi, void* y_lo, const pp_conv_opts* opts) {
  return (ctx && ctx->planes_fmt == 1) ? pp_conv2d_nhwc_fwd_bf16x3_fmt1(ctx, d, x, x_hi, x_lo, w_fwd_hi, w_fwd_lo, bias, residual, ld_res, relu, y, y_hi, y_lo, opts) : pp_conv2d_nhwc_fwd_bf16x3_fmt0(ctx, d, x, x_hi, x_lo, w_fwd_hi, w_fwd_lo, bias, residual, ld_res, relu, y, y_hi, y_lo, opts);
}
extern "C" int pp_row_block_dilate(pp_ctx* ctx, const pp_conv_desc* d, const unsigned char* in_flags, unsigned char* out_flags) {
  return (ctx && ctx->planes_fmt == 1) ? pp_row_block_dilate_fmt1(ctx, d, in_flags, out_flags) : pp_row_block_dilate_fmt0(ctx, d, in_flags, out_flags);
}
extern "C" int pp_stem7x7s2_fwd_bf16x3(pp_ctx* ctx, int n_img, int H, int W, int Hp, int Wp, const float* x4p, const void* w_hi, const void* w_lo, int cout, const float* bias, int relu, float* y, int ld_y) {
  return (ctx && ctx->planes_fmt == 1) ? pp_stem7x7s2_fwd_bf16x3_fmt1(ctx, n_img, H, W, Hp, Wp, x4p, w_hi, w_lo, cout, bias, relu, y, ld_y) : pp_stem7x7s2_fwd_bf16x3_fmt0(ctx, n_img, H, W, Hp, Wp, x4p, w_hi, w_lo, cout, bias, relu, y, ld_y);
}
extern "C" int pp_conv2d_nhwc_bwd_data_bf16x3(pp_ctx* ctx, const pp_conv_desc* d, const float* dy, const void* dy_hi, const void* dy_lo, const void* w_dgrad_hi, const void* w_dgrad_lo, const float* addend, int ld_add, const float* relu_src, int ld_rs, float* dx, void* dx_hi, void* dx_lo, const pp_conv_opts* opts) {
  return (ctx && ctx->planes_fmt == 1) ? pp_conv2d_nhwc_bwd_data_bf16x3_fmt1(ctx, d, dy, dy_hi, dy_lo, w_dgrad_hi, w_dgrad_lo, addend, ld_add, relu_src, ld_rs, dx, dx_hi, dx_lo, opts) : pp_conv2d_nhwc_bwd_data_bf16x3_fmt0(ctx, d, dy, dy_hi, dy_lo, w_dgrad_hi, w_dgrad_lo, addend, ld_add, relu_src, ld_rs, dx, dx_hi, dx_lo, opts);
}
extern "C" int pp_conv2d_nhwc_bwd_weight_bf16x3(pp_ctx* ctx, const pp_conv_desc* d, const float* x, const float* dy, const void* x_hi, const void* x_lo, const void* dy_hi, const void* dy_lo, float* dw, float* dbias, const pp_conv_opts* opts) {
  return (ctx && ctx->planes_fmt == 1) ? pp_conv2d_nhwc_bwd_weight_bf16x3_fmt1(ctx, d, x, dy, x_hi, x_lo, dy_hi, dy_lo, dw, dbias, opts) : pp_conv2d_nhwc_bwd_weight_bf16x3_fmt0(ctx, d, x, dy, x_hi, x_lo, dy_hi, dy_lo, dw, dbias, opts);
}

extern "C" int pp_conv_plan_text(const pp_conv_desc* d, int pass, unsigned forms, int planes_fmt, int n_cu, size_t ws_bytes, char* buf,
                                 int buf_bytes) {
  if (!buf || buf_bytes <= 0 || pass < PP_PLAN_FWD || pass > PP_PLAN_BWD_WEIGHT) return PP_ERR_ARG;
  const int rc = check_desc(nullptr, d, "pp_conv_plan_text");
  if (rc) return rc;
  const bool planes_in = forms & PP_PLAN_PLANES_IN, planes_out = forms & PP_PLAN_PLANES_OUT, f32_out = (forms & PP_PLAN_F32_OUT) || !planes_out,
             capture = forms & PP_PLAN_CAPTURE, list = forms & PP_PLAN_LIST, lazy_in = forms & PP_PLAN_LAZY_IN;
  const bool ws = ws_bytes > 0;
  int at = 0;
  buf[0] = 0;
  if (pass == PP_PLAN_BWD_WEIGHT) {
    if (d->cin % 64 != 0) return PP_ERR_SHAPE;
    Wgrad3Params p;
    memset(&p, 0, sizeof(p));
    wgrad_geometry(nullptr, d, p);
    const PpWgradFacts f = wgrad_facts(p, planes_in, list, lazy_in, planes_fmt, n_cu, ws, (long long)ws_bytes, true, true);
    return pp_plan_print(buf, buf_bytes, at, f, pp_plan_wgrad(f), true);
  }
  IgemmParams p;
  memset(&p, 0, sizeof(p));
  if (pass == PP_PLAN_FWD) {
    if (d->cin % 32 != 0) return PP_ERR_SHAPE;
    igemm_geometry_fwd(nullptr, d, p);
    PpIgemmFacts f = igemm_facts(p, d->cout, d->cin / 8, planes_in, !planes_in, planes_out, f32_out, capture, false, n_cu, ws, (long long)ws_bytes);
    if (list) {
      if (!fwd_listed_ok(d, f, false)) return PP_ERR_SHAPE;
      f.listed = true;
      f.listed_tm = 2;
    }
    return pp_plan_print(buf, buf_bytes, at, f, pp_plan_igemm(f), true);
  }
  if (d->cin % 16 != 0) return PP_ERR_SHAPE;
  igemm_geometry_bwd_data(nullptr, d, p);
  const int w_rows = d->cin, w_ld8 = p.Cred / 8;
  const PpIgemmFacts f = igemm_facts(p, w_rows, w_ld8, planes_in, !planes_in, planes_out, f32_out, capture, list, n_cu, ws, (long long)ws_bytes);
  DgradRoute route;
  dgrad_route(d, p, f, list, &route);
  if (lazy_in && !route.listed) return pp_plan_append(buf, buf_bytes, at, "igemm3 refused: lazy dy without a listed-block launch\n");
  dgrad_launches(
      route, p,
      [&](IgemmParams& q, bool is_class, bool listed) {
        PpIgemmFacts fq = igemm_facts(q, w_rows, w_ld8, planes_in, !planes_in, planes_out, f32_out, capture && !is_class, list && !is_class, n_cu, ws,
                                      (long long)ws_bytes);
        fq.listed = listed;
        fq.listed_tm = route.listed_tm;
        at = pp_plan_print(buf, buf_bytes, at, fq, pp_plan_igemm(fq), true);
      },
      [&](IgemmParams& q) {
        at = pp_plan_append(buf, buf_bytes, at, "class M %d N %d: no taps class_fill | grid=%u\n", q.M, q.Nout,
                            pp_finish_blocks(q.M, q.Nout, pp_cus(n_cu)));
      });
  return at;
}
```

pyrapose_amd/csrc/conv_common.h:

```cpp
#pragma once
#include <stdlib.h>

#include <type_traits>

#include "conv_plan.h"
#include "pp_internal.h"

typedef float floatx16 __attribute__((ext_vector_type(16)));

struct SegGeo {
  int row_begin;
  int src_row_begin;
  int OH, OW;
  int SH, SW;
};

struct IgemmParams {
  const float* src;
  const float* wgt;
  float* out;
  const float* bias;
  const float* addend;
  const float* mask_src;
  int ld_src, ld_w, ld_out, ld_add, ld_mask;
// ... 126 lines not shown
               d->ld_w, d->cout);
  PP_CHECK_ARG(ctx, d->ld_x % 4 == 0 && d->ld_x >= d->cin, PP_ERR_SHAPE, "%s: ld_x %d < cin %d or not a multiple of 4", who, d->ld_x, d->cin);
  PP_CHECK_ARG(ctx, d->ld_y % 4 == 0 && d->ld_y >= ((d->cout + 3) & ~3), PP_ERR_SHAPE,
               "%s: ld_y %d must be a multiple of 4 and >= cout %d rounded up to 4", who, d->ld_y, d->cout);
  PP_CHECK_ARG(ctx, d->pad_t >= 0 && d->pad_l >= 0 && d->pad_t < d->kh && d->pad_l < d->kw, PP_ERR_SHAPE, "%s: bad padding", who);
  for (int s = 0; s < d->in.n_seg; ++s) {
    PP_CHECK_ARG(ctx, (d->out.h[s] - 1) * d->stride - d->pad_t < d->in.h[s] && (d->out.w[s] - 1) * d->stride - d->pad_l < d->in.w[s],
                 PP_ERR_SHAPE, "%s: output %dx%d does not fit input %dx%d", who, d->out.h[s], d->out.w[s], d->in.h[s], d->in.w[s]);
  }
  if (d->in.n_seg > 1) PP_CHECK_ARG(ctx, d->stride == 1, PP_ERR_SHAPE, "%s: multi-level row spaces need stride 1", who);
  return PP_OK;
}


static void igemm_geometry_fwd(pp_ctx* ctx, const pp_conv_desc* d, IgemmParams& p) {
  p.ld_src = d->ld_x; p.ld_w = d->ld_w; p.ld_out = d->ld_y;
  p.n_seg = d->in.n_seg;
  fill_segs(ctx, d, true, p.seg, &p.M, &p.src_rows);
  p.Cred = d->cin; p.Nout = d->cout; p.w_tap_rows = d->cin;
  p.kh = d->kh; p.kw = d->kw;
  p.mul = d->stride; p.tsign = 1; p.off_y = -d->pad_t; p.off_x = -d->pad_l; p.div = 1;
  p.w_ty0 = 0; p.w_tx0 = 0; p.w_tstep = 1; p.w_kw = d->kw; p.w_taps = d->kh * d->kw;
}
static void igemm_geometry_bwd_data(pp_ctx* ctx, const pp_conv_desc* d, IgemmParams& p) {
  p.ld_src = d->ld_y; p.ld_w = d->ld_w; p.ld_out = d->ld_x;
  p.n_seg = d->in.n_seg;
  fill_segs(ctx, d, false, p.seg, &p.M, &p.src_rows);
  p.Cred = (d->cout + 31) / 32 * 32; p.Nout = d->cin; p.w_tap_rows = d->cin;
  p.kh = d->kh; p.kw = d->kw;
  p.mul = 1; p.tsign = -1; p.off_y = d->pad_t; p.off_x = d->pad_l; p.div = d->stride;
  p.w_ty0 = 0; p.w_tx0 = 0; p.w_tstep = 1; p.w_kw = d->kw; p.w_taps = d->kh * d->kw;
}
static void wgrad_geometry(pp_ctx* ctx, const pp_conv_desc* d, Wgrad3Params& p) {
  p.ld_src = d->ld_x; p.ld_dy = d->ld_y; p.ld_w = d->ld_w;
  p.n_seg = d->in.n_seg;
  fill_segs(ctx, d, true, p.seg, &p.M, &p.src_rows);
  p.Cin = d->cin; p.Cout = d->cout;
  p.kh = d->kh; p.kw = d->kw; p.stride = d->stride; p.pad_t = d->pad_t; p.pad_l = d->pad_l;
}

static bool segs_same_grid(const SegGeo* seg, int n_seg) {
  bool same = true;
  for (int i = 0; i < n_seg && same; ++i) same = seg[i].OH == seg[i].SH && seg[i].OW == seg[i].SW && seg[i].row_begin == seg[i].src_row_begin;
  return same;
}

static PpIgemmFacts igemm_facts(const IgemmParams& p, int w_rows, int w_ld8, bool planes_in, bool f32_in, bool planes_out, bool f32_out,
                                bool capture, bool flags, int n_cu, bool ws, long long ws_bytes) {
  PpIgemmFacts f = {};
  f.M = p.M; f.Nout = p.Nout; f.Cred = p.Cred; f.kh = p.kh; f.kw = p.kw; f.ld_out = p.ld_out; f.ld_src = p.ld_src;
  f.w_rows = w_rows; f.w_ld8 = w_ld8; f.w_taps = p.w_taps; f.div = p.div; f.mul = p.mul; f.sc_on = p.sc_on; f.w_tstep = p.w_tstep; f.w_tx0 = p.w_tx0;
  f.src_rows = p.src_rows;
  for (int i = 0; i < p.n_seg; ++i) f.max_sw = p.seg[i].SW > f.max_sw ? p.seg[i].SW : f.max_sw;
  f.same_grid = segs_same_grid(p.seg, p.n_seg);
  f.planes_in = planes_in; f.f32_in = f32_in; f.planes_out = planes_out; f.f32_out = f32_out; f.capture = capture; f.flags = flags;
  f.n_cu = pp_cus(n_cu); f.ws = ws; f.ws_bytes = ws_bytes;
  return f;
}

static PpWgradFacts wgrad_facts(Wgrad3Params& p, bool planes, bool list, bool lazy_in, int fmt, int n_cu, bool ws, long long ws_bytes,
                                bool dw_aligned, bool dbias_aligned) {
  PpWgradFacts f = {};
  f.M = p.M; f.Cin = p.Cin; f.Cout = p.Cout; f.kh = p.kh; f.kw = p.kw; f.stride = p.stride; f.pad_t = p.pad_t; f.pad_l = p.pad_l;
  f.ld_src = p.ld_src; f.ld_dy = p.ld_dy; f.ld_w = p.ld_w; f.src_rows = p.src_rows;
  f.min_ow = f.min_hw = 1 << 30;
  f.list_levels_aligned = true;
  long long pos = 0;
  for (int i = 0; i < p.n_seg; ++i) {
    f.min_ow = p.seg[i].OW < f.min_ow ? p.seg[i].OW : f.min_ow;
    f.min_hw = p.seg[i].OH * p.seg[i].OW < f.min_hw ? p.seg[i].OH * p.seg[i].OW : f.min_hw;
    if (i + 1 < p.n_seg && p.seg[i + 1].row_begin % 32 != 0) f.list_levels_aligned = false;
    const long long rows = (i + 1 < p.n_seg ? p.seg[i + 1].row_begin : p.M) - p.seg[i].row_begin;
    p.pos_begin[i] = (int)pos;
    pos += rows / p.seg[i].OW * (p.seg[i].OW + 1);
  }
  p.Mp = (int)pos;
  f.Mp = pos;
  f.same_grid = segs_same_grid(p.seg, p.n_seg);
  f.planes = planes; f.list = list; f.lazy_in = lazy_in; f.fmt = fmt;
  f.n_cu = pp_cus(n_cu); f.ws = ws; f.ws_bytes = ws_bytes; f.dw_aligned = dw_aligned; f.dbias_aligned = dbias_aligned;
  return f;
}

static bool igemm_parity_classes(const pp_conv_desc* d, const IgemmParams& p, bool all_planes, IgemmParams cls[4]) {
  const int H = d->in.h[0], W = d->in.w[0];
  for (int c = 0; c < 4; ++c) {
    const int cy = c >> 1, cx = c & 1;
    IgemmParams& r = cls[c];
    r = p;
    r.div = 1;
    const int ty0 = (cy + d->pad_t) & 1, tx0 = (cx + d->pad_l) & 1;
    r.kh = ty0 < d->kh ? (d->kh - ty0 + 1) / 2 : 0;
    r.kw = tx0 < d->kw ? (d->kw - tx0 + 1) / 2 : 0;
    r.off_y = (cy + d->pad_t - ty0) / 2;
    r.off_x = (cx + d->pad_l - tx0) / 2;
    r.w_ty0 = ty0; r.w_tx0 = tx0; r.w_tstep = 2; r.w_kw = d->kw;
    if (r.kh == 0 || r.kw == 0) r.kh = r.kw = 0;
    r.seg[0].OH = (H - cy + 1) / 2;
    r.seg[0].OW = (W - cx + 1) / 2;
    r.M = d->in.n_img * r.seg[0].OH * r.seg[0].OW;
    r.sc_on = 1; r.sc_H = H; r.sc_W = W; r.sc_cy = cy; r.sc_cx = cx;
    if (r.M > 0 && r.kh > 0 &&
        !(pp_igemm_fast_ok(igemm_facts(r, d->cin, r.Cred / 8, all_planes, !all_planes, all_planes, !all_planes, false, false, 0, false, 0)) && r.M < (1 << 24)))
      return false;
  }
  return true;
}

static bool fwd_listed_ok(const pp_conv_desc* d, const PpIgemmFacts& f, bool residual) {
  return f.planes_in && f.f32_out != f.planes_out && !f.capture && !residual && d->stride == 1 && d->kh == 3 && d->kw == 3 && d->pad_t == 1 &&
         d->pad_l == 1 && pp_igemm_fast_ok(f) && f.same_grid;
}

struct DgradRoute {
  bool listed;
  int listed_tm;
  bool classes;
  IgemmParams cls[4];
};
static void dgrad_route(const pp_conv_desc* d, const IgemmParams& p, const PpIgemmFacts& f, bool skip_scratch, DgradRoute* r) {
  const bool all_f32 = f.f32_in && f.f32_out && !f.planes_in && !f.planes_out, all_planes = f.planes_in && f.planes_out && !f.f32_out;
  const PpDgradRouteFacts rf = {d->stride, d->kh, d->kw, d->pad_t, d->pad_l, d->in.n_seg, all_f32, all_planes, f.capture, p.bias != nullptr,
                                f.flags, skip_scratch, pp_igemm_fast_ok(f), f.same_grid};
  r->listed = pp_dgrad_listed_ok(rf);
  r->listed_tm = pp_conv_switches().sparse_dgrad == 22 ? 2 : 1;
  r->classes = pp_dgrad_classes_ok(rf) && igemm_parity_classes(d, p, all_planes, r->cls);
}
template <class Gemm, class Fill>
static void dgrad_launches(DgradRoute& r, IgemmParams& p, Gemm gemm, Fill fill) {
  if (!r.classes) {
    gemm(p, false, r.listed);
    return;
  }
  for (int c = 0; c < 4; ++c) {
    if (r.cls[c].M <= 0) continue;
    if (r.cls[c].kh > 0) gemm(r.cls[c], true, false);
    else fill(r.cls[c]);
  }
}
```

pyrapose_amd/csrc/conv_plan.h:

```cpp
#pragma once
#include <stdarg.h>
#include <stdio.h>
#include <stdlib.h>

struct PpConvSwitches {
  int gscale_log2;
  bool fast;
  bool xreuse;
  int sparse_dgrad_splits;
  int sparse_dgrad;
  int x_order;
  int dma_min;
  int dma_frac;
  bool dma_tail;
  int dma_tail_frac;
  bool x4;
  bool s2_classes;
  int wgrad3w_min;
  int wgrad3_sp_steps;
};
inline int pp_env_int(const char* name, int dflt) { const char* e = getenv(name); return e ? atoi(e) : dflt; }
inline bool pp_env_not0(const char* name) { const char* e = getenv(name); return !(e && e[0] == '0'); }
inline bool pp_env_is1(const char* name) { const char* e = getenv(name); return e && e[0] == '1'; }
inline const PpConvSwitches& pp_conv_switches() {
  static const PpConvSwitches s = []() {
    PpConvSwitches v;
    const int g = pp_env_int("PP_GSCALE_LOG2", 8);
    v.gscale_log2 = g < -20 ? -20 : (g > 30 ? 30 : g);
    v.fast = pp_env_not0("PP_CONV3_FAST");
    v.xreuse = pp_env_not0("PP_CONV3_XREUSE");
    v.sparse_dgrad_splits = pp_env_int("PP_SPARSE_DGRAD_SPLITS", 2);
    v.sparse_dgrad = pp_env_int("PP_SPARSE_DGRAD", 22);
    v.x_order = pp_env_int("PP_CONV3_X_ORDER", 1);
    v.dma_min = pp_env_int("PP_CONV3_DMA_MIN", 512);
    v.dma_frac = pp_env_int("PP_CONV3_DMA_FRAC", 1000);
    v.dma_tail = pp_env_not0("PP_CONV3_DMA_TAIL");
    v.dma_tail_frac = pp_env_int("PP_CONV3_DMA_TAIL_FRAC", 60);
    v.x4 = pp_env_is1("PP_CONV3_X4");
    v.s2_classes = pp_env_not0("PP_CONV3_S2CLASSES");
    const int wm = pp_env_int("PP_WGRAD3W_MIN", 0);
    v.wgrad3w_min = wm > 0 ? wm : 512;
    const int ss = pp_env_int("PP_WGRAD3_SP_STEPS", 0);
    v.wgrad3_sp_steps = ss > 0 ? ss : 1;
    return v;
  }();
  return s;
}
inline bool pp_sw_debug() { return getenv("PP_CONV_DEBUG") != nullptr; }
inline bool pp_sw_dma() { return pp_env_not0("PP_CONV3_DMA"); }
inline int pp_sw_dma_var() { return pp_env_int("PP_CONV3_DMA_VAR", 1); }
inline bool pp_sw_dma2() { return pp_env_is1("PP_CONV3_DMA2"); }
inline int pp_sw_dma2_min() { return pp_env_int("PP_CONV3_DMA2_MIN", 512); }
inline bool pp_sw_conv4p() { return pp_env_is1("PP_CONV4P"); }
inline int pp_sw_conv4p_nst() { const char* e = getenv("PP_CONV4P_NST"); return e && atoi(e) == 3 ? 3 : 4; }
inline int pp_sw_conv4p_splits() { return pp_env_int("PP_CONV4P_SPLITS", 0); }
inline bool pp_sw_wgrad_det() { return pp_env_is1("PP_WGRAD3_DETERMINISTIC"); }
inline int pp_sw_wgrad3r() { const char* e = getenv("PP_WGRAD3R"); return !e ? -1 : ((e[0] == '1' || e[0] == '2') ? e[0] - '0' : 0); }
inline bool pp_sw_tile(const char* name, char* a, char* b) {
  const char* e = getenv(name);
  if (!(e && e[0] && e[1] == ',' && e[2])) return false;
  *a = e[0];
  *b = e[2];
  return true;
}
inline int pp_sw_splits(const char* name) { const char* e = getenv(name); return e ? atoi(e) : 0; }

inline int pp_cus(int n_cu) { return n_cu > 0 ? n_cu : 256; }

inline double est_rounds(long long blocks, int slots, int cus) {
  static const double thr[5] = {1.0, 0.62, 0.78, 0.81, 0.82};
  const long long per_round = (long long)cus * slots;
  const long long full = blocks / per_round;
  const long long rem = blocks - full * per_round;
  const int s_idx = slots < 4 ? slots : 4;
  double t = (double)full * slots / thr[s_idx];
  if (rem > 0) {
    const int c = (int)((rem + cus - 1) / cus);
    t += (double)c / thr[c < 4 ? c : 4];
  }
  return t;
}

inline unsigned pp_finish_blocks(long long rows, int Nout, int n_cu) {
  const long long total = rows * ((Nout + 3) >> 2);
  long long blocks = (total + 255) / 256;
  if (blocks > (long long)n_cu * 8) blocks = (long long)n_cu * 8;
  return (unsigned)blocks;
}

struct PpIgemmFacts {
  int M, Nout, Cred, kh, kw, ld_out, ld_src, w_rows, w_ld8, w_taps, div, mul, sc_on, w_tstep, w_tx0;
  long long src_rows;
  int max_sw;
  bool same_grid;
  bool planes_in, f32_in, planes_out, f32_out, capture, flags;
  bool listed;
  int listed_tm;
  int n_cu;
  bool ws;
  long long ws_bytes;
};

enum PpIgemmFamily {
  PP_IGEMM3, PP_IGEMM3F, PP_IGEMM3F_CLASS, PP_IGEMM3X_CAPTURE, PP_IGEMM3X_PP, PP_IGEMM3X_PF, PP_IGEMM3X_FP, PP_IGEMM3X_FF, PP_IGEMM4X,
  PP_IGEMM4X2, PP_IGEMM4P, PP_IGEMM3F_LIST
};
static const char* const pp_igemm_family_name[] = {
    "igemm3", "igemm3f", "igemm3f[parity class]", "igemm3x[capture]", "igemm3x[planes->planes]", "igemm3x[planes->f32]",
    "igemm3x[f32->planes]", "igemm3x[f32->f32]", "igemm4x", "igemm4x<NWM=2>", "igemm4p", "igemm3f[row list]"};

struct PpIgemmPlan {
  int family;
  int tm, tn, splits;
  int n_tiles_n;
  unsigned grid;
  int x_ty_inner, skip_halo;
  int full_rt, tail_splits, variant;
  int tail_m_off;
  unsigned tail_grid;
  int stages;
  bool capture_first;
  unsigned finish_blocks;
  long long ws_need;
  int n_steps;
  bool may_split;
};

inline bool pp_igemm_fast_ok(const PpIgemmFacts& f) {
  const long long a_bytes = f.src_rows * (long long)f.ld_src * 4;
  const long long w_bytes = (long long)f.w_taps * f.w_rows * f.w_ld8 * 16;
  return pp_conv_switches().fast && f.div == 1 && f.kh * f.kw <= 31 && a_bytes < (1ll << 31) && w_bytes < (1ll << 31) &&
         (long long)f.max_sw * f.ld_src * 4 < (1ll << 23) && f.src_rows > 0;
}

inline bool pp_igemm_x_ok(const PpIgemmFacts& f) {
  return pp_conv_switches().xreuse && pp_igemm_fast_ok(f) && !f.sc_on && f.kw == 3 && f.mul == 1 && f.div == 1 && (f.f32_in || f.planes_in) &&
         (!f.planes_in || f.ld_src % 8 == 0) && f.w_tstep == 1 && f.w_tx0 == 0 && f.same_grid;
}

inline void pp_pick_tile3(const PpIgemmFacts& f, int n_steps, bool may_split, bool x_ok, int* tm, int* tn, int* splits) {
  static const int cand[5][2] = {{4, 2}, {2, 2}, {1, 2}, {2, 1}, {1, 1}};
  static const double eff[5] = {1.1, 1.0, 0.9, 0.9, 0.8};
  static const int slots[5] = {2, 3, 4, 4, 4};
  static const int split_cand[8] = {1, 2, 3, 4, 6, 8, 12, 16};
  const int M = f.M, Nout = f.Nout, ld_out = f.ld_out, cus = f.n_cu;
  const long long ws_bytes = f.ws_bytes;
  double best = 1e300;
  *splits = 1;
  for (int i = 0; i < 5; ++i) {
    const int bm = 64 * cand[i][0], bn = 64 * cand[i][1];
    const long long blocks = (long long)((M + bm - 1) / bm) * ((Nout + bn - 1) / bn);
    for (int si = 0; si < (may_split ? 8 : 1); ++si) {
      const int sp = split_cand[si];
      if (sp > 1 && (n_steps / sp < 8 || (long long)sp * M * ld_out * 4 > ws_bytes)) break;
      const double steps = (double)((n_steps + sp - 1) / sp) + 8.0;
      double t = est_rounds(blocks * sp, slots[i], cus) * steps * cand[i][0] * cand[i][1] / eff[i];
      if (sp > 1) {
        const double us = (double)M * Nout * (8.0 * sp + 12.0) / 4.0e6 + 4.0;
        t += us / 2.1 * 4.0;
      }
      if (t < best * 0.97) {
        best = t;
        *tm = cand[i][0];
        *tn = cand[i][1];
        *splits = sp;
      }
    }
  }
  if (x_ok && *tm == 4 && *splits == 1 && !pp_conv_switches().x4) {
    *tm = 2;
    *tn = 2;
  }
  char a, b;
  if (pp_sw_tile("PP_CONV3_TILE", &a, &b)) {
    *tm = a - '0';
    *tn = b - '0';
  }
  if (const int v = pp_sw_splits("PP_CONV3_SPLITS")) {
    if (v >= 1 && (v == 1 || (may_split && n_steps / v >= 1 && (long long)v * M * ld_out * 4 <= ws_bytes))) *splits = v;
  }
  if (*tm == 4) *tn = 2;
  else if (!((*tm == 2 || *tm == 1) && (*tn == 2 || *tn == 1))) *tm = *tn = 1;
}

inline void pp_plan_listed(const PpIgemmFacts& f, PpIgemmPlan* pl) {
  const int nb = (f.M + 31) / 32, BM = 64 * f.listed_tm, BN = 128;
  const int want_splits = pp_conv_switches().sparse_dgrad_splits;
  int splits = 1;
  if (f.ws && want_splits > 1 && (f.planes_out || f.f32_out)) {
    const long long slice_bytes = (long long)nb * 32 * f.ld_out * 4;
    splits = want_splits;
    while (splits > 1 && (pl->n_steps / splits < 24 || slice_bytes * splits > f.ws_bytes)) --splits;
// ... 54 lines not shown
  pl.grid = (unsigned)(((f.M + BM - 1) / BM) * pl.n_tiles_n * splits);
  pl.finish_blocks = splits > 1 ? pp_finish_blocks(f.M, f.Nout, n_cu) : 0u;
  pl.ws_need = splits > 1 ? (long long)splits * f.M * f.ld_out * 4 : 0;
  if (f.sc_on) {
    pl.family = PP_IGEMM3F_CLASS;
    return pl;
  }
  if (x_ok && (tm <= 2 || (f.planes_in && !f.capture))) {
    const int n_tiles_mx = (f.M + BM - 3) / (BM - 2);
    pl.skip_halo = f.max_sw + 1;
    pl.grid = (unsigned)(n_tiles_mx * pl.n_tiles_n * splits);
    pl.x_ty_inner = sw.x_order;
    const bool op = f.planes_out && splits == 1;
    if (tm <= 2 && f.capture) {
      pl.family = PP_IGEMM3X_CAPTURE;
      return pl;
    }
    if (tm == 2 && tn == 2 && pp_sw_dma() && f.planes_in && op && !f.flags && splits == 1 && f.kh == 3 && sw.x_order == 1 && f.w_rows % 128 == 0 &&
        f.Cred % 32 == 0) {
      const int BM4 = 256;
      const int n_tiles_m4 = (f.M + BM4 - 3) / (BM4 - 2);
      const int ntn = (f.Nout + 127) / 128;
      const int n_blk = n_tiles_m4 * ntn;
      const bool one_and_a_bit = n_blk > n_cu && n_blk < 2 * n_cu && (n_blk - n_cu) * 100 >= sw.dma_frac * n_cu;
      if (n_blk >= sw.dma_min || one_and_a_bit) {
        int full_rt = n_tiles_m4;
        const int rounds = (n_tiles_m4 * ntn) / n_cu;
        const int last = (n_tiles_m4 * ntn) % n_cu;
        if (sw.dma_tail && last != 0 && last * 100 < sw.dma_tail_frac * n_cu && rounds >= 2 && f.ws) full_rt = rounds * n_cu / ntn;
        const int m_split = full_rt * (BM4 - 2);
        int tail_splits = 0;
        if (full_rt < n_tiles_m4) {
          const int rem = f.M - m_split;
          const int n_rt = (rem + BM - 3) / (BM - 2);
          const int groups = f.kh * (f.Cred / 32);
          int sp = (3 * n_cu + n_rt * ntn - 1) / (n_rt * ntn);
          while (sp > 1 && (groups / sp < 4 || (long long)sp * rem * f.ld_out * 4 > f.ws_bytes)) --sp;
          if (sp > 1) tail_splits = sp;
          else full_rt = n_tiles_m4;
        }
        const int var = pp_sw_dma_var();
        pl.family = PP_IGEMM4X;
        pl.variant = (var == 0 || var == 2 || var == 3 || var == 4 || var == 9) ? var : 1;
        pl.n_tiles_n = ntn;
        pl.full_rt = full_rt;
        pl.grid = (unsigned)(full_rt * ntn);
        pl.tail_splits = tail_splits;
        if (tail_splits > 1) {
          const int rem = f.M - full_rt * (BM4 - 2);
          pl.tail_m_off = full_rt * (BM4 - 2);
          pl.tail_grid = (unsigned)(((rem + BM - 3) / (BM - 2)) * ntn * tail_splits);
          pl.finish_blocks = pp_finish_blocks(rem, f.Nout, n_cu);
          pl.ws_need = (long long)tail_splits * rem * f.ld_out * 4;
        }
        return pl;
      }
      if (pp_sw_dma2() && n_tiles_mx * ntn >= pp_sw_dma2_min()) {
        pl.family = PP_IGEMM4X2;
        pl.n_tiles_n = ntn;
        pl.grid = (unsigned)(n_tiles_mx * ntn);
        return pl;
      }
    }
    pl.family = f.planes_in ? (op ? PP_IGEMM3X_PP : PP_IGEMM3X_PF) : (op ? PP_IGEMM3X_FP : PP_IGEMM3X_FF);
    return pl;
  }
  pl.capture_first = f.capture;
  pl.family = fast ? PP_IGEMM3F : PP_IGEMM3;
  return pl;
}

struct PpDgradRouteFacts {
  int stride, kh, kw, pad_t, pad_l, n_seg;
  bool all_f32, all_planes, capture, bias, skip, skip_scratch, fast_ok, same_grid;
};
inline bool pp_dgrad_listed_ok(const PpDgradRouteFacts& r) {
  return r.skip && r.skip_scratch && pp_conv_switches().sparse_dgrad && (r.all_f32 || r.all_planes) && !r.capture && r.stride == 1 && r.kh == 3 &&
         r.kw == 3 && r.pad_t == 1 && r.pad_l == 1 && !r.bias && r.fast_ok && r.same_grid;
}
inline bool pp_dgrad_classes_ok(const PpDgradRouteFacts& r) {
  return r.stride == 2 && pp_conv_switches().s2_classes && (r.all_f32 || r.all_planes) && r.n_seg == 1;
}

struct PpWgradFacts {
  int M, Cin, Cout, kh, kw, stride, pad_t, pad_l, ld_src, ld_dy, ld_w;
  long long src_rows;
  int min_ow, min_hw;
  bool same_grid;
  bool list_levels_aligned;
  long long Mp;
  bool planes, list, lazy_in;
  int fmt;
  int n_cu;
  bool ws;
  long long ws_bytes;
  bool dw_aligned, dbias_aligned;
};

enum PpWgradFamily { PP_WGRAD3, PP_WGRAD3F_PLANES_LIST, PP_WGRAD3F_PLANES, PP_WGRAD3F_F32_LIST, PP_WGRAD3F_F32, PP_WGRAD3R, PP_WGRAD3W };
static const char* const pp_wgrad_family_name[] = {"wgrad3", "wgrad3f[planes, list]", "wgrad3f[planes]", "wgrad3f[f32, list]", "wgrad3f[f32]",
                                                   "wgrad3r", "wgrad3w"};

struct PpWgradPlan {
  int family;
  bool refused;
  int tm, tn;
  bool fast;
  int k_tiles_per_tap, n_tiles_k, n_tiles_n, tiles;
  int model_splits;
  int splits, rows_per_split, max_wraps, sp_min_steps;
  bool use_ws;
  long long ws_slice;
  unsigned grid, finish_blocks;
  long long ws_need;
};

inline bool pp_plan_wgrad3r(const PpWgradFacts& f, int variant, PpWgradPlan* pl) {
  if (!(f.kh == 3 && f.kw == 3 && f.stride == 1 && f.pad_t == 1 && f.pad_l == 1 && f.Cin % 128 == 0 && f.planes)) return false;
  if (variant == 2 && f.list) return false;
  if (!f.same_grid) return false;
  if (f.list && !f.list_levels_aligned) return false;
  const long long x_bytes = f.src_rows * (long long)f.ld_src * 4, d_bytes = (long long)f.M * f.ld_dy * 4;
  if (!(f.min_ow >= (f.list ? 12 : 2) && x_bytes < (1ll << 31) && d_bytes < (1ll << 31) && f.Mp < (1 << 24) && f.src_rows > 0)) return false;
  pl->k_tiles_per_tap = f.Cin / 128;
  pl->n_tiles_k = 3 * pl->k_tiles_per_tap;
  pl->n_tiles_n = (f.Cout + 127) / 128;
  const int tiles = pl->tiles = pl->n_tiles_k * pl->n_tiles_n;
  const int R = f.list ? f.M : (int)f.Mp;
  int max_splits = (R + 255) / 256;
  if (max_splits > 128) max_splits = 128;
  if (max_splits < 1) max_splits = 1;
  const double atomic_steps_per_split = 0.5 * (double)tiles * 3.0 * 128.0 * 128.0 * 4.0 / 1.3e6 / 1.0;
  int splits = 1;
  double best = 1e300;
  for (int sp = 1; sp <= max_splits; ++sp) {
    const double steps = (double)((R + sp - 1) / sp + 31) / 32.0 + 6.0;
    const double rounds = (double)(((long long)tiles * sp + f.n_cu - 1) / f.n_cu);
    const double cost = rounds * steps + atomic_steps_per_split * sp;
    if (cost < best * 0.995) {
      best = cost;
      splits = sp;
    }
  }
  if (const int v = pp_sw_splits("PP_WGRAD3R_SPLITS")) {
    if (v >= 1 && v <= max_splits) splits = v;
  }
  int rps = (R + splits - 1) / splits;
  rps = (rps + 31) / 32 * 32;
  splits = (R + rps - 1) / rps;
  pl->family = variant == 2 ? PP_WGRAD3W : PP_WGRAD3R;
  pl->tm = pl->tn = 2;
  pl->fast = true;
  pl->model_splits = pl->splits = splits;
  pl->rows_per_split = rps;
  pl->grid = (unsigned)(tiles * splits);
  return true;
}

inline PpWgradPlan pp_plan_wgrad(const PpWgradFacts& f) {
  const PpConvSwitches& sw = pp_conv_switches();
  PpWgradPlan pl = {};
  pl.sp_min_steps = sw.wgrad3_sp_steps;
  const bool det = pp_sw_wgrad_det();
  {
    const int e_r = pp_sw_wgrad3r();
    int variant = 0;
// ... 27 lines not shown
  }
  const int slots = fast ? ((TM * TN == 4) ? 3 : 4) : ((TM * TN == 4) ? 2 : 3);
  const double tile_work = (double)(TM * TN) / 4.0;
  const long long ws_slice = pl.ws_slice = (long long)f.kh * f.kw * f.Cin * f.ld_w + f.ld_w;
  const bool use_ws = pl.use_ws = fast && f.ws && f.ws_bytes >= ws_slice * 4 && f.dw_aligned && f.dbias_aligned && det;
  if (use_ws) {
    const long long fit = f.ws_bytes / (ws_slice * 4);
    if (max_splits > fit) max_splits = (int)fit;
  }
  const double atomic_us_per_split = use_ws ? (double)tiles * BM * BN * 4.0 * 2.0 / 4.0e6 : 0.5 * (double)tiles * BM * BN * 4.0 / 1.3e6;
  int splits = 1;
  double best = 1e300;
  for (int sp = 1; sp <= max_splits; ++sp) {
    const double steps = (double)((f.M + sp - 1) / sp + 31) / 32.0;
    const double cost = est_rounds((long long)tiles * sp, slots, cus) * steps * tile_work * 0.8 + atomic_us_per_split * sp;
    if (cost < best * 0.995) {
      best = cost;
      splits = sp;
    }
  }
  if (const int v = pp_sw_splits("PP_WGRAD3_SPLITS")) {
    if (v >= 1 && v <= max_splits) splits = v;
  }
  pl.model_splits = splits;
  int rps = (f.M + splits - 1) / splits;
  rps = (rps + 31) / 32 * 32;
  splits = (f.M + rps - 1) / rps;
  pl.splits = splits;
  pl.rows_per_split = rps;
  pl.grid = (unsigned)(tiles * splits);
  pl.family = !fast ? PP_WGRAD3
                    : (f.planes ? (f.list ? PP_WGRAD3F_PLANES_LIST : PP_WGRAD3F_PLANES) : (f.list ? PP_WGRAD3F_F32_LIST : PP_WGRAD3F_F32));
  if (use_ws && splits > 1) {
    const long long n4 = (ws_slice - f.ld_w) / 4;
    long long blocks = (n4 + f.ld_w / 4 + 255) / 256;
    if (blocks > (long long)cus * 8) blocks = (long long)cus * 8;
    pl.finish_blocks = (unsigned)blocks;
    pl.ws_need = (long long)splits * ws_slice * 4;
  }
  return pl;
}

inline int pp_plan_append(char* buf, int cap, int at, const char* fmt, ...) {
  if (at >= cap) return at;
  va_list ap;
  va_start(ap, fmt);
  const int n = vsnprintf(buf + at, (size_t)(cap - at), fmt, ap);
  va_end(ap);
  return n < 0 ? at : (at + n < cap ? at + n : cap);
}
inline int pp_plan_print(char* buf, int cap, int at, const PpIgemmFacts& f, const PpIgemmPlan& pl, bool detail) {
  if (pl.family == PP_IGEMM4P)
    at = pp_plan_append(buf, cap, at, "igemm4p M %d N %d steps %d -> %lld tiles x %d splits on %d CUs, %d stages", f.M, f.Nout, pl.n_steps,
                        (long long)((f.M + 127) / 128) * ((f.Nout + 127) / 128), pl.splits, f.n_cu, pl.stages);
  else if (pl.family == PP_IGEMM3F_LIST)
    at = pp_plan_append(buf, cap, at, "igemm3 M %d N %d steps %d -> tile %dx%d splits %d (listed blocks)", f.M, f.Nout, pl.n_steps, 64 * pl.tm,
                        64 * pl.tn, pl.splits);
  else
    at = pp_plan_append(buf, cap, at, "igemm3 M %d N %d steps %d -> tile %dx%d splits %d (may_split %d: ws %d planes_out %d out %d)", f.M, f.Nout,
                        pl.n_steps, 64 * pl.tm, 64 * pl.tn, pl.splits, (int)pl.may_split, (int)f.ws, (int)f.planes_out, (int)f.f32_out);
  at = pp_plan_append(buf, cap, at, " %s", pp_igemm_family_name[pl.family]);
  if (detail)
    at = pp_plan_append(buf, cap, at, " | grid=%u n_tiles_n=%d x_ty_inner=%d skip_halo=%d full_rt=%d tail_splits=%d tail_grid=%u tail_m_off=%d "
                        "variant=%d stages=%d capture_first=%d finish_blocks=%u ws_need=%lld",
                        pl.grid, pl.n_tiles_n, pl.x_ty_inner, pl.skip_halo, pl.full_rt, pl.tail_splits, pl.tail_grid, pl.tail_m_off, pl.variant,
                        pl.stages, (int)pl.capture_first, pl.finish_blocks, pl.ws_need);
  return pp_plan_append(buf, cap, at, "\n");
}
inline int pp_plan_print(char* buf, int cap, int at, const PpWgradFacts& f, const PpWgradPlan& pl, bool detail) {
  if (pl.refused) return pp_plan_append(buf, cap, at, "wgrad3 refused: lazy dy without a listed-block reduction\n");
  if (pl.family == PP_WGRAD3R || pl.family == PP_WGRAD3W)
    at = pp_plan_append(buf, cap, at, "wgrad3r tiles %d (3 taps each) splits %d (M %d)%s", pl.tiles, pl.splits, f.M, f.list ? " listed blocks" : "");
  else
    at = pp_plan_append(buf, cap, at, "wgrad3 tile %dx%d tiles %d splits %d (M %d) fast %d", 64 * pl.tm, 64 * pl.tn, pl.tiles, pl.model_splits, f.M,
                        (int)pl.fast);
  at = pp_plan_append(buf, cap, at, " %s", pp_wgrad_family_name[pl.family]);
  if (detail)
    at = pp_plan_append(buf, cap, at, " | grid=%u tile=%dx%d splits=%d rows_per_split=%d max_wraps=%d sp_min_steps=%d use_ws=%d ws_slice=%lld "
                        "finish_blocks=%u ws_need=%lld",
                        pl.grid, 64 * pl.tm, 64 * pl.tn, pl.splits, pl.rows_per_split, pl.max_wraps, pl.sp_min_steps, (int)pl.use_ws, pl.ws_slice,
                        pl.finish_blocks, pl.ws_need);
  return pp_plan_append(buf, cap, at, "\n");
}
template <class Facts, class Plan>
inline void pp_plan_debug(const Facts& f, const Plan& pl) {
  if (!pp_sw_debug()) return;
  char line[512];
  pp_plan_print(line, (int)sizeof(line), 0, f, pl, false);
  fputs(line, stderr);
}
```

pyrapose_amd/engine.py:

```python
import os as _os
from collections import OrderedDict

import numpy as np
import torch

from . import arch, ops
from ._lib import ParamDesc, RowSpace


def _ru(v, m):
    return (v + m - 1) // m * m


def tf_same_pad(n_in, k, s):
    out = -(-n_in // s)
    total = max((out - 1) * s + k - n_in, 0)
    return total // 2


class Op(object):
    __slots__ = ("fn", "kind", "name", "flops", "wrange", "lane", "reads", "waits", "done_ev", "out_blocks")

    def __init__(self, fn, kind, name="", flops=0.0, wrange=None, lane=0):
        self.fn, self.kind, self.name, self.flops, self.wrange, self.lane = fn, kind, name, flops, wrange, lane
# ... 199 lines not shown
                    raise ValueError("optimizer state of %s: shape %s, expected %s" % (key, a.shape, (s.cout,)))
                host[e["offset"]: e["offset"] + s.cout] = a
        buf.copy_(torch.from_numpy(host))


class Engine(object):
    def __init__(self, ctx, num_classes, batch, height, width, backbone="resnet50", weights=None, train=True, seed=0,
                 lr=1e-5, clipnorm=0.001, freeze_backbone=False, conv_mode=None, pyramid="sparse", anchor_params=None,
                 loss_params=None):
        self._own_ctx = ops.Context(ctx.device, ctx.stream)
        ctx = self._own_ctx
        self.ctx, self.C, self.B, self.H, self.W = ctx, int(num_classes), int(batch), int(height), int(width)
        lp = dict(box=(0.125, 3.0), cls=(0.25, 2.0), mask=(0.25, 2.0))
        lp.update(loss_params or {})
        self.loss_params = {k: (float(v[0]), float(v[1])) for k, v in lp.items()}
        assert pyramid in arch.PYRAMIDS, pyramid
        self.pyramid = pyramid
        from .utils import anchors as _ua
        if anchor_params is None:
            anchor_params = _ua.AnchorParameters.default if pyramid != "p3p7" else _ua.AnchorParameters.p3p7
        self.anchor_params = anchor_params
        self.A = anchor_params.num_anchors()
        assert len(anchor_params.sizes) == len(arch.PYRAMID_LEVELS[pyramid]), "anchor_params need one size / stride per pyramid level"
        self.backbone = backbone
        self.train = train
        self.lr, self.clipnorm = lr, clipnorm
        self.beta1, self.beta2, self.eps = 0.9, 0.999, 1e-7
        self.specs = arch.all_specs(self.C, backbone, pyramid, self.A)
        if freeze_backbone:
            for s in self.specs:
                if s.bn:
                    s.trainable = False
        self.params = ParamStore(self.specs, train)
        self.params.load(weights if weights is not None else arch.init_weights(self.C, seed, backbone, pyramid, self.A))
        mode = conv_mode or _os.environ.get("PP_CONV_MODE", "mixed")
        assert mode in ("f32", "bf16x3", "f16c8", "mixed"), mode
        if mode in ("f16c8", "mixed") and _os.environ.get("PP_PLANES", "1") == "0":
            mode = "bf16x3"
        self.arith = mode
        self.conv_mode = "f32" if mode == "f32" else "bf16x3"
        self.po = self.conv_mode == "bf16x3" and _os.environ.get("PP_PLANES", "1") != "0"
        self.use_act_planes = False
        self.capture = (self.conv_mode == "bf16x3" and not self.po and _os.environ.get("PP_CAPTURE", "0") == "1")
        self.sparse_bwd = tuple(t for t in _os.environ.get("PP_SPARSE_BWD", "reg").split(",") if t and t != "0") \
            if self.conv_mode == "bf16x3" else ()
        self.sparse_fwd = (self.train and self.po and "reg" in self.sparse_bwd and _os.environ.get("PP_SPARSE_FWD", "0") == "1")
        self._sparse_fwd_now = False
        self.capture_min_cin = int(_os.environ.get("PP_CAPTURE_MIN_CIN", "64"))
        self.capture_skip = tuple(t for t in _os.environ.get("PP_CAPTURE_SKIP", "").split(",") if t)
        self.planes = OrderedDict()
        self.fwd_ops, self.graph_ops, self.bwd_ops = [], [], []
        os = _os
        self.n_lanes = max(1, min(3, int(os.environ.get("PP_LANES", "2"))))
        self.streams = [ctx.stream] + [torch.cuda.Stream(device=ctx.device) for _ in range(self.n_lanes - 1)]
        self.ctxs = [ctx] + [ops.Context(ctx.device, st) for st in self.streams[1:]]
        ws_mb = int(os.environ.get("PP_SPLITK_MB", "256"))
        if self.conv_mode == "bf16x3" and ws_mb > 0:
            for c in self.ctxs:
                c.set_workspace(ws_mb << 20)
        self.gscale = None
        import math as _math
        ratio = max(self.loss_params["box"][0] / 0.125, self.loss_params["cls"][0] / 0.25, self.loss_params["mask"][0] / 0.25, 1.0)
        self.gscale_adjust = -int(_math.ceil(_math.log2(ratio)))
        from ._lib import MISSING as _missing
        if self.train and self.po and self.arith in ("f16c8", "mixed") and "pp_grad_scale_from_counts" not in _missing:
            self.gscale = torch.ones((2,), dtype=torch.float32, device="cuda")
            for c in self.ctxs:
                ops.set_grad_scale(c.twin(1), self.gscale)
        self._lane = 0
        self.trunk_lanes = os.environ.get("PP_TRUNK_LANES", "1") != "0"
        self.prefix_lane = None
        self.n_prefix_early = 0
        self._prefetched = None
        frozen_prefix = all(not sp.trainable for sp in self.specs if sp.name == "conv1" or sp.name.startswith("res2"))
        if self.train and frozen_prefix and self.conv_mode == "bf16x3" and os.environ.get("PP_PREFETCH", "0") == "1":
            pst = torch.cuda.Stream(device=ctx.device)
            self.streams.append(pst)
            self.ctxs.append(ops.Context(ctx.device, pst))
            if ws_mb > 0:
                self.ctxs[-1].set_workspace(ws_mb << 20)
            self.prefix_lane = len(self.streams) - 1
        self.acts = OrderedDict()
        self._plane_grads = []
        self.step_count = 0
        self._build_forward()
        self.levels = arch.level_shapes(self.H, self.W, arch.PYRAMID_LEVELS[pyramid])
        assert [tuple(s) for s in self.pyr.shapes] == [tuple(s) for s in self.levels], (self.pyr.shapes, self.levels)
        self.N = sum(h * w for h, w in self.levels) * self.A
        self.M3 = self.levels[0][0] * self.levels[0][1]
        f32 = dict(dtype=torch.float32, device="cuda")
        self.out_box = torch.empty((self.B, self.N, 16), **f32)
        self.out_cls = torch.empty((self.B, self.N, self.C), **f32)
        self.out_mask = torch.empty((self.B, self.M3, self.C), **f32)
        self.anchors_f32 = None
        if train:
            self.counts = torch.zeros((4,), dtype=torch.int32, device="cuda")
            self.loss_sums = torch.zeros((4,), **f32)
            self.gnorm_sq = torch.zeros((1,), **f32)
            self.y_box = torch.zeros((self.B, self.N, 17), **f32)
            self.y_cls = torch.zeros((self.B, self.N, self.C + 1), **f32)
            self.y_mask = torch.zeros((self.B, self.M3, self.C + 1), **f32)
            self.opt = ops.Optimizer(ctx, self.params.descs(), self.params.total)
            self._build_backward()
        self.grad_sync = None
        self.refresh_planes()

    def close(self):
        opt = getattr(self, "opt", None)
        if opt is not None:
            opt.close()
            self.opt = None
        st = getattr(self, "streams", None)
        if st and getattr(self, "ctxs", None):
            for side in st[1:]:
                st[0].wait_stream(side)
        for c in getattr(self, "ctxs", []):
            c.close()
        self.ctxs = []
        self.fwd_ops, self.bwd_ops, self.graph_ops = [], [], []

    def _enter(self):
        cur = torch.cuda.current_stream(self.ctx.device)
        if cur.cuda_stream != self.streams[0].cuda_stream:
            self.streams[0].wait_stream(cur)
        return cur

    def _leave(self, cur):
        if cur.cuda_stream != self.streams[0].cuda_stream:
            cur.wait_stream(self.streams[0])

    def _new_act(self, name, shapes, C, ld=None, needs_grad=False, relu=False, t=None, pl=None, planes=False, fmt=0):
        a = Act(name, self.B, shapes, C, ld, t, needs_grad, relu, pl, planes, fmt)
        self.acts[name] = a
        return a

    def _fmt(self, spec_name):
        if self.arith == "f16c8":
            return 1
        if self.arith == "mixed":
            return 0 if spec_name.startswith(("conv1", "res")) else 1
        return 0

    def _convert(self, x, fmt):
        if x.pl is None or x.fmt == fmt:
            return x
        cache = x.__dict__.setdefault("_converted", {})
        if fmt in cache:
            return cache[fmt]
        out = self._new_act(x.name + ":fmt%d" % fmt, x.shapes, x.C, x.ld, x.needs_grad, False, planes=True, fmt=fmt)
        lane = self._lane
        ctx = self.ctxs[lane]
        self._push(Op(lambda: ops.convert_planes(ctx, x.pl, x.fmt, out.pl, fmt), "pointwise", "convert:" + x.name, lane=lane), (x,), out)
        self.graph_ops.append(dict(kind="convert", y=out, x=x))
        cache[fmt] = out
        return out

    def _on(self, lane):
        eng = self

        class _Lane(object):
            def __enter__(self_):
                self_.prev = eng._lane
                eng._lane = (lane % eng.n_lanes) if eng.trunk_lanes else eng._lane

            def __exit__(self_, *exc):
                eng._lane = self_.prev
# ... 300 lines not shown
        vx, vo = x.view(), out.view()
        self._push(Op(lambda: ops.relu_fwd_v(ctx, vx, vo), "pointwise", name, lane=lane), (x,), out)
        self.graph_ops.append(dict(kind="relu", y=out, x=x))
        return out

    def _upadd(self, name, src, other):
        (sh, sw), (th, tw) = src.shapes[0], other.shapes[0]
        other = self._convert(other, src.fmt)
        out = self._new_act(name, [(th, tw)], src.C, src.ld, src.needs_grad or other.needs_grad, planes=self.po, fmt=src.fmt)
        lane, B = self._lane, self.B
        ctx = self.ctxs[lane].twin(src.fmt)
        vs, vt, vo = src.view(), other.view(), out.view()
        self._push(Op(lambda: ops.upsample_add_fwd_v(ctx, B, sh, sw, th, tw, src.C, vs, vt, vo), "pointwise", name, lane=lane),
                   (src, other), out)
        self.graph_ops.append(dict(kind="upadd", y=out, src=src, other=other))
        return out

    def _add(self, name, ins):
        ins = [ins[0]] + [self._convert(i, ins[0].fmt) for i in ins[1:]]
        out = self._new_act(name, ins[0].shapes, ins[0].C, ins[0].ld, any(i.needs_grad for i in ins), planes=self.po, fmt=ins[0].fmt)
        lane = self._lane
        ctx = self.ctxs[lane].twin(ins[0].fmt)
        va, vb, vc = ins[0].view(), ins[1].view(), (ins[2].view() if len(ins) > 2 else None)
        vo = out.view()
        self._push(Op(lambda: ops.add_n_v(ctx, va, vb, vc, vo), "pointwise", name, lane=lane), ins, out)
        self.graph_ops.append(dict(kind="add", y=out, ins=ins))
        return out

    def _new_grad(self, rows, ld, fmt=0):
        if self.po and ld % 8 == 0:
            g = Grad(None, _new_planes(rows, ld), fmt)
            self._plane_grads.append(g)
            return g
        return Grad(torch.empty((rows, ld), dtype=torch.float32, device="cuda"))

    def _finalize(self, act, producer=None):
        ctx = self.ctx.twin(act.fmt)
        grads = [c[1] for c in act.contribs if c[0] in ("tensor", "masked")]
        dgrads = [c for c in act.contribs if c[0] == "dgrad"]
        if any(c[0] == "masked" for c in act.contribs):
            assert len(act.contribs) == 1, act.name
            return grads[0]
        if not grads and not dgrads:
            return None
        acc = None
        if len(grads) == 1:
            acc = grads[0]
        elif len(grads) > 1:
            acc = self._new_grad(act.rows, act.ld, act.fmt)
            srcs, rest = grads[:3], grads[3:]
            while True:
                va, vb, vc = srcs[0].view(), (srcs[1].view() if len(srcs) > 1 else None), (srcs[2].view() if len(srcs) > 2 else None)
                vo = ops.tview(acc.t, acc.pl)
                self.bwd_ops.append(Op(lambda va=va, vb=vb, vc=vc, vo=vo: ops.add_n_v(ctx, va, vb, vc, vo), "pointwise", "add:" + act.name))
                if not rest:
                    break
                srcs, rest = [acc] + rest[:2], rest[2:]
        if act.relu and not dgrads:
            raise NotImplementedError("relu output %s without a data-gradient consumer" % act.name)
        if not dgrads:
            return acc
        for i, (_, op, gy) in enumerate(dgrads):
            last = i == len(dgrads) - 1
            mask = act if (act.relu and last) else None
            pl = op.get("planes")
            if pl is not None and pl["dg_hi"] is not None:
                gcap = op.get("g_cap")
                sk = op.get("skip")
                in_place = (sk is not None and i > 0 and mask is None and acc is not None and gcap is None
                            and _os.environ.get("PP_SPARSE_INPLACE", "1") != "0")
                out = acc if in_place else self._new_grad(act.rows, act.ld, act.fmt)
                lazy_out = (sk is not None and len(dgrads) == 1 and acc is None and gcap is None and gy.pl is not None and out.pl is not None
                            and self._lazy_reader(producer) and _os.environ.get("PP_SPARSE_WITHIN", "1") != "0"
                            and _os.environ.get("PP_SPARSE_LAZY", "1") != "0" and _os.environ.get("PP_SPARSE_DGRAD", "22") != "0")
                lazy_in = bool(gy.lazy)
                dy_t, dy_pl = (None, gy.pl) if gy.pl is not None else (gy.t, None)
                a_t = a_pl = m_t = m_hi = None
                if acc is not None:
                    a_t, a_pl = (acc.t, None) if acc.t is not None else (None, acc.pl)
                if mask is not None:
                    m_t, m_hi = (mask.t, None) if mask.t is not None else (None, mask.pl[0])
                if gcap is not None:
                    assert dy_t is not None
                self.bwd_ops.append(Op(lambda d=op["desc"], dy_t=dy_t, dy_pl=dy_pl, dh=pl["dg_hi"], dl=pl["dg_lo"], a_t=a_t, a_pl=a_pl, m_t=m_t,
                                       m_hi=m_hi, out=out, gcap=gcap, sk=sk, lazy_out=lazy_out, lazy_in=lazy_in:
                                       ops.conv_bwd_data3(ctx, d, dy_t, dh, dl, a_t, m_t, out.t, dy_pl, out.pl, gcap, sk, a_pl, m_hi,
                                                          lazy_out=lazy_out, lazy_in=lazy_in), "conv_dgrad",
                                       op["spec"].name, op["flops"]))
                out.within = sk[0][sk[0].numel() // 2:] if (sk is not None and acc is None and _os.environ.get("PP_SPARSE_WITHIN", "1") != "0") else None
                out.lazy = lazy_out
                assert not lazy_out or out.within is not None
                pw = op.pop("pending_wgrad", None)
                if pw is not None:
                    self.bwd_ops.append(pw)
            else:
                assert gy.t is not None and (acc is None or acc.t is not None) and (mask is None or mask.t is not None), act.name
                out = Grad(torch.empty((act.rows, act.ld), dtype=torch.float32, device="cuda"))
                self.bwd_ops.append(Op(lambda d=op["desc"], gy=gy, w=op["w"], a=(acc.t if acc is not None else None),
                                       m=(mask.t if mask is not None else None), out=out:
                                       ops.conv_bwd_data(ctx, d, gy.t, w, a, m, out.t), "conv_dgrad", op["spec"].name, op["flops"]))
            acc = out
        return acc

    def _lazy_reader(self, producer):
        if producer is None or producer.get("kind") != "conv" or producer.get("residual") is not None:
            return False
        s_, pl_, x_, y_ = producer["spec"], producer.get("planes"), producer["x"], producer["y"]
        geo = (_os.environ.get("PP_CONV3_FAST", "1") != "0" and min(h * w for h, w in x_.shapes) >= 32 and x_.rows < (1 << 24)
               and x_.rows * x_.ld * 4 < (1 << 31) and y_.rows * y_.ld * 4 < (1 << 31) and list(x_.shapes) == list(y_.shapes))
        return self._sparse_layer(s_) and pl_ is not None and pl_["dg_hi"] is not None and x_.pl is not None and y_.pl is not None and geo

    def _build_backward(self):
        ctx, P = self.ctx, self.params
        f32 = dict(dtype=torch.float32, device="cuda")
        self.g_reg = torch.zeros((self.reg_out.rows, self.reg_out.ld), **f32)
        self.g_cls = torch.zeros((self.cls_out.rows, self.cls_out.ld), **f32)
        self.g_mask = torch.zeros((self.mask_out.rows, self.mask_out.ld), **f32)
        for out, gt in ((self.reg_out, self.g_reg), (self.cls_out, self.g_cls), (self.mask_out, self.g_mask)):
            g = Grad(gt, None, out.fmt)
            if self.po and out.ld % 8 == 0:
                g.pl = _new_planes(out.rows, out.ld)
                sctx, sc = ctx.twin(out.fmt), (self.gscale if out.fmt == 1 else None)
                self.bwd_ops.append(Op(lambda gt=gt, pl=g.pl, sctx=sctx, sc=sc: ops.split_planes3(sctx, gt, pl[0], pl[1], sc), "pointwise",
                                       "split:" + out.name))
            out.contribs.append(("tensor", g))
        for op in reversed(self.graph_ops):
            kind = op["kind"]
            if kind == "stop":
                break
            y = op["y"]
            if not y.needs_grad:
                continue
            g = self._finalize(y, op)
            if g is None:
                continue
            if kind == "convert":
                x = op["x"]
                if x.needs_grad:
                    gx = self._new_grad(x.rows, x.ld, x.fmt)
                    assert g.pl is not None and gx.pl is not None, x.name
                    sc, idx = (self.gscale, 1) if (g.fmt == 1 and x.fmt == 0) else ((self.gscale, 0) if (g.fmt == 0 and x.fmt == 1) else (None, 0))
                    lone = x.relu and not any(o is not op and o.get("kind") == "conv" and o.get("x") is x for o in self.graph_ops)
                    mhi = x.pl[0] if lone else None
                    self.bwd_ops.append(Op(lambda g=g, gx=gx, sc=sc, idx=idx, mhi=mhi: ops.convert_planes(ctx, g.pl, g.fmt, gx.pl, gx.fmt, sc, idx, mhi),
                                           "pointwise", "convert_bwd:" + x.name))
                    x.contribs.append(("masked" if lone else "tensor", gx))
                continue
            if kind == "conv":
                s, x = op["spec"], op["x"]
                lctx = ctx.twin(y.fmt)
                if self._sparse_layer(s) and g.contiguous() and len(g.shape()) == 2:
                    nb = (g.shape()[0] + 31) // 32
                    skip = op["skip"] = (torch.zeros((2 * nb,), dtype=torch.uint8, device="cuda"),
                                         torch.zeros((2 * (nb + 1),), dtype=torch.int32, device="cuda"))
                    cols = min((y.C + 3) // 4 * 4, g.shape()[1])
                    if g.t is not None:
                        self.bwd_ops.append(Op(lambda gt=g.t, cols=cols, skip=skip, lctx=lctx: ops.row_block_list(lctx, gt, cols, skip[0], skip[1]),
                                               "pointwise", "rowblocks:" + s.name))
                    else:
                        self.bwd_ops.append(Op(lambda gp=g.pl, cols=cols, skip=skip, within=g.within, lctx=lctx:
                                               ops.row_block_list_planes(lctx, gp, cols, skip[0], skip[1], within),
                                               "pointwise", "rowblocks:" + s.name))
                if s.trainable:
                    dw = P.view(P.grad, s.name + "/kernel")
                    db = P.view(P.grad, s.name + "/bias") if s.bias else None
                    ek = P.entries[s.name + "/kernel"]
                    eb = P.entries[s.name + "/bias"]
                    wr = (ek["offset"], eb["offset"] + eb["count"])
                    wl = 1 % self.n_lanes
                    wctx = self.ctxs[wl].twin(y.fmt)
                    pl_ = op.get("planes")
# ... 325 lines not shown
```

pyrapose_amd/ops.py:

```python
import collections
import ctypes as C

import numpy as np
import torch

from ._lib import ConvDesc, ConvOpts, ParamDesc, RowSpace, TView, check, lib
from ._lib import check as check_status


def _ptr(t):
    if t is None:
        return None
    assert t.is_cuda, "pyrapose_amd ops need device tensors"
    return C.c_void_p(t.data_ptr())


class Context:

    def __init__(self, device=0, stream=None):
        if not torch.cuda.is_available():
            raise RuntimeError("pyrapose_amd: no GPU visible (torch.cuda.is_available() is False); "
                               "the HIP path has no CPU fallback")
        self.device = int(device)
        torch.cuda.set_device(self.device)
        self.handle = C.c_void_p()
        s = stream if stream is not None else torch.cuda.current_stream(self.device)
        self.stream = s
        check(lib.pp_ctx_create(C.byref(self.handle), self.device, C.c_void_p(s.cuda_stream)), None, "pp_ctx_create")

        self.planes_fmt = 0
        self._twin = None

    def use_stream(self, stream):
        for c in (self, self._twin):
            if c is not None:
                c.stream = stream
                check(lib.pp_ctx_set_stream(c.handle, C.c_void_p(stream.cuda_stream)), c.handle, "pp_ctx_set_stream")

    def twin(self, fmt):
        if int(fmt) == self.planes_fmt:
            return self
        if self._twin is None:
            t = Context(self.device, self.stream)
            set_planes_format(t, fmt)
            t._twin = self
            ws = getattr(self, "workspace", None)
            t.workspace = ws
            if ws is not None:
                check(lib.pp_ctx_set_workspace(t.handle, _ptr(ws), ws.numel() * 4), t.handle, "pp_ctx_set_workspace")
            self._twin = t
        assert self._twin.planes_fmt == int(fmt)
        return self._twin

    def set_workspace(self, nbytes):
        self.workspace = torch.empty((int(nbytes) // 4,), dtype=torch.float32, device="cuda:%d" % self.device) if nbytes else None
        for c in (self, self._twin):
            if c is not None:
                c.workspace = self.workspace
                check(lib.pp_ctx_set_workspace(c.handle, _ptr(self.workspace), (int(nbytes) // 4) * 4 if nbytes else 0), c.handle,
                      "pp_ctx_set_workspace")

    def device_info(self):
        n = C.c_int(0)
        buf = C.create_string_buffer(128)
        check(lib.pp_device_info(self.handle, C.byref(n), buf, 128), self.handle)
        return n.value, buf.value.decode()

    def close(self):
        t, self._twin = self._twin, None
        if t is not None and t.handle:
            t._twin = None
            t.close()
        if self.handle:
            lib.pp_ctx_destroy(self.handle)
            self.handle = C.c_void_p()


def make_conv_desc(n_img, in_shapes, out_shapes, cin, cout, k, stride, pad_t, pad_l, ld_x, ld_y, ld_w):
    d = ConvDesc()
    d.in_ = RowSpace.make(n_img, in_shapes)
    d.out = RowSpace.make(n_img, out_shapes)
    d.cin, d.cout, d.kh, d.kw, d.stride = cin, cout, k, k, stride
    d.pad_t, d.pad_l, d.ld_x, d.ld_y, d.ld_w = pad_t, pad_l, ld_x, ld_y, ld_w
    return d


PLAN_FWD, PLAN_BWD_DATA, PLAN_BWD_WEIGHT = 0, 1, 2
PLAN_PLANES_IN, PLAN_PLANES_OUT, PLAN_F32_OUT, PLAN_CAPTURE, PLAN_LIST, PLAN_LAZY_IN, PLAN_LAZY_OUT = 1, 2, 4, 8, 16, 32, 64


def conv_plan_text(d, pass_, forms=0, planes_fmt=1, n_cu=256, ws_bytes=0):
    buf = C.create_string_buffer(4096)
    n = lib.pp_conv_plan_text(C.byref(d), int(pass_), int(forms), int(planes_fmt), int(n_cu), int(ws_bytes), buf, len(buf))
    check(min(n, 0), None, "pp_conv_plan_text")
    return buf.value.decode()


def conv_fwd(ctx, d, x, w, bias, residual, relu, y):
    ld_res = residual.stride(0) if residual is not None else 0
    check(lib.pp_conv2d_nhwc_fwd(ctx.handle, C.byref(d), _ptr(x), _ptr(w), _ptr(bias), _ptr(residual), ld_res,
                                 int(bool(relu)), _ptr(y)), ctx.handle, "pp_conv2d_nhwc_fwd")


def conv_bwd_data(ctx, d, dy, w, addend, relu_src, dx):
    ld_add = addend.stride(0) if addend is not None else 0
    ld_rs = relu_src.stride(0) if relu_src is not None else 0
    check(lib.pp_conv2d_nhwc_bwd_data(ctx.handle, C.byref(d), _ptr(dy), _ptr(w), _ptr(addend), ld_add, _ptr(relu_src),
                                      ld_rs, _ptr(dx)), ctx.handle, "pp_conv2d_nhwc_bwd_data")


def conv_bwd_weight(ctx, d, x, dy, dw, dbias):
    check(lib.pp_conv2d_nhwc_bwd_weight(ctx.handle, C.byref(d), _ptr(x), _ptr(dy), _ptr(dw), _ptr(dbias)), ctx.handle,
          "pp_conv2d_nhwc_bwd_weight")


def conv_split_weights3(ctx, d, w, fwd_hi, fwd_lo, dg_hi, dg_lo):
    check(lib.pp_conv_split_weights_bf16x3(ctx.handle, C.byref(d), _ptr(w), _ptr(fwd_hi), _ptr(fwd_lo), _ptr(dg_hi), _ptr(dg_lo)),
          ctx.handle, "pp_conv_split_weights_bf16x3")


class SplitWeightsBatch(object):

    def __init__(self, jobs):
        from ._lib import SplitJob
        jobs = list(jobs)
        arr = (SplitJob * max(len(jobs), 1))()
        tiles = 0
        self._keep = jobs
        for i, (d, w, fh, fl, dh, dl) in enumerate(jobs):
            if d.cin % 32:
                raise ValueError("SplitWeightsBatch: cin %d must be a multiple of 32" % d.cin)
            j = arr[i]
            j.w, j.fwd_hi, j.fwd_lo, j.dg_hi, j.dg_lo = [(t.data_ptr() if t is not None else None) for t in (w, fh, fl, dh, dl)]
            j.taps, j.cin, j.cout, j.ld_w, j.tile_begin = d.kh * d.kw, d.cin, d.cout, d.ld_w, tiles
            tiles += j.taps * (d.cin // 32) * ((d.cout + 31) // 32)
        self.n, self.tiles = len(jobs), tiles
        host = torch.frombuffer(bytearray(bytes(arr)), dtype=torch.uint8)
        self.table = host.cuda()

    def run(self, ctx):
        check(lib.pp_conv_split_weights_bf16x3_batch(ctx.handle, self.n, _ptr(self.table), self.tiles), ctx.handle,
              "pp_conv_split_weights_bf16x3_batch")


def new_planes(rows, ld, device="cuda", fill=0):
    assert ld % 8 == 0, ld
    base = torch.full((rows, ld // 8, 2, 8), fill, dtype=torch.int16, device=device)
    return base[:, :, 0, :], base[:, :, 1, :]


def planes_ld(planes):
    return planes[0].stride(0) // 2


def set_planes_format(ctx, fmt):
    check(lib.pp_ctx_set_planes_format(ctx.handle, int(fmt)), ctx.handle, "pp_ctx_set_planes_format")
    ctx.planes_fmt = int(fmt)


def convert_planes(ctx, src, src_fmt, dst, dst_fmt, scale2=None, scale_index=0, relu_src_hi=None):
    n = src[0].numel()
    check(lib.pp_convert_planes(ctx.handle, n, _ptr(src[0]), _ptr(src[1]), int(src_fmt), _ptr(dst[0]), _ptr(dst[1]), int(dst_fmt), _ptr(scale2),
                                int(scale_index), _ptr(relu_src_hi)), ctx.handle, "pp_convert_planes")


def planes_to_f32(planes, fmt=0):
    hi, lo = planes
    rows = hi.shape[0]
    if fmt == 0:
        return (hi.contiguous().view(torch.bfloat16).float() + lo.contiguous().view(torch.bfloat16).float()).reshape(rows, -1)
# ... 63 lines not shown
    t, planes = v._keep
    return (t if t is not None else planes[0]).numel()


def add_n_v(ctx, a, b, c, out):
    null = TView()
    check(lib.pp_add_n_v(ctx.handle, _numel(a), C.byref(a), C.byref(b if b is not None else null), C.byref(c if c is not None else null),
                         C.byref(out)), ctx.handle, "pp_add_n_v")


def relu_fwd_v(ctx, x, y):
    check(lib.pp_relu_fwd_v(ctx.handle, _numel(x), C.byref(x), C.byref(y)), ctx.handle, "pp_relu_fwd_v")


def upsample_add_fwd_v(ctx, n_img, sh, sw, th, tw, c, src, other, out):
    null = TView()
    check(lib.pp_upsample_nearest_add_fwd_v(ctx.handle, n_img, sh, sw, th, tw, c, C.byref(src), C.byref(other if other is not None else null),
                                            C.byref(out)), ctx.handle, "pp_upsample_nearest_add_fwd_v")


def upsample_add_bwd_v(ctx, n_img, sh, sw, th, tw, c, dtarget, base, dsrc):
    null = TView()
    check(lib.pp_upsample_nearest_add_bwd_v(ctx.handle, n_img, sh, sw, th, tw, c, C.byref(dtarget), C.byref(base if base is not None else null),
                                            C.byref(dsrc)), ctx.handle, "pp_upsample_nearest_add_bwd_v")


def merge_planes3(ctx, planes, dst):
    check(lib.pp_merge_planes_bf16x3(ctx.handle, dst.numel(), _ptr(planes[0]), _ptr(planes[1]), _ptr(dst)), ctx.handle, "pp_merge_planes_bf16x3")


def planes_stats(ctx, planes, cols, stats, within=None):
    hi, lo = planes
    check(lib.pp_planes_stats(ctx.handle, _ptr(hi), _ptr(lo), int(hi.shape[0]), planes_ld(planes), int(cols), _ptr(within), _ptr(stats)), ctx.handle,
          "pp_planes_stats")
    return stats


def positive_row_blocks(ctx, rs, n_anchor, y_true, flags):
    check(lib.pp_positive_row_blocks(ctx.handle, C.byref(rs), int(n_anchor), int(y_true.shape[-1]), _ptr(y_true), _ptr(flags)), ctx.handle,
          "pp_positive_row_blocks")
    return flags


def row_block_dilate(ctx, d, in_flags, out_flags):
    check(lib.pp_row_block_dilate(ctx.handle, C.byref(d), _ptr(in_flags), _ptr(out_flags)), ctx.handle, "pp_row_block_dilate")
    return out_flags


def _conv_opts(capture=None, add=None, mask_hi=None, skip=None, out=None, lazy_out=False, lazy_in=False):
    if capture is None and add is None and mask_hi is None and skip is None and out is None and not (lazy_out or lazy_in):
        return None
    o = ConvOpts()
    o.capture_hi, o.capture_lo = map(_ptr, capture or (None, None))
    o.add_hi, o.add_lo = map(_ptr, add or (None, None))
    o.mask_hi = _ptr(mask_hi)
    o.skip_flags, o.skip_list = map(_ptr, skip or (None, None))
    o.out_flags, o.out_list = map(_ptr, out or (None, None))
    o.lazy_out, o.lazy_in = int(bool(lazy_out)), int(bool(lazy_in))
    return C.byref(o)


def conv_fwd3(ctx, d, x, w_hi, w_lo, bias, residual, relu, y, x_planes=None, y_planes=None, x_capture=None, res_planes=None,
              out_blocks=None):
    ld_res = residual.stride(0) if residual is not None else (planes_ld(res_planes) if res_planes is not None else 0)
    xh, xl = x_planes if x_planes is not None else (None, None)
    yh, yl = y_planes if y_planes is not None else (None, None)
    check(lib.pp_conv2d_nhwc_fwd_bf16x3(ctx.handle, C.byref(d), _ptr(x), _ptr(xh), _ptr(xl), _ptr(w_hi), _ptr(w_lo), _ptr(bias),
                                        _ptr(residual), ld_res, int(bool(relu)), _ptr(y), _ptr(yh), _ptr(yl),
                                        _conv_opts(capture=x_capture, add=res_planes, out=out_blocks)), ctx.handle,
          "pp_conv2d_nhwc_fwd_bf16x3")


def conv_bwd_data3(ctx, d, dy, w_hi, w_lo, addend, relu_src, dx, dy_planes=None, dx_planes=None, dy_capture=None, dy_skip=None,
                   addend_planes=None, relu_src_hi=None, lazy_out=False, lazy_in=False):
    ld_add = addend.stride(0) if addend is not None else (planes_ld(addend_planes) if addend_planes is not None else 0)
    ld_rs = relu_src.stride(0) if relu_src is not None else (relu_src_hi.stride(0) // 2 if relu_src_hi is not None else 0)
    dh, dl = dy_planes if dy_planes is not None else (None, None)
    xh, xl = dx_planes if dx_planes is not None else (None, None)
    check(lib.pp_conv2d_nhwc_bwd_data_bf16x3(ctx.handle, C.byref(d), _ptr(dy), _ptr(dh), _ptr(dl), _ptr(w_hi), _ptr(w_lo), _ptr(addend),
                                             ld_add, _ptr(relu_src), ld_rs, _ptr(dx), _ptr(xh), _ptr(xl),
                                             _conv_opts(capture=dy_capture, add=addend_planes, mask_hi=relu_src_hi, skip=dy_skip,
                                                        lazy_out=lazy_out, lazy_in=lazy_in)), ctx.handle,
          "pp_conv2d_nhwc_bwd_data_bf16x3")


def conv_bwd_weight3(ctx, d, x, dy, dw, dbias, x_planes=None, dy_planes=None, dy_skip=None, lazy_in=False):
    xh, xl = x_planes if x_planes is not None else (None, None)
    dh, dl = dy_planes if dy_planes is not None else (None, None)
    check(lib.pp_conv2d_nhwc_bwd_weight_bf16x3(ctx.handle, C.byref(d), _ptr(x), _ptr(dy), _ptr(xh), _ptr(xl), _ptr(dh), _ptr(dl),
                                               _ptr(dw), _ptr(dbias), _conv_opts(skip=dy_skip, lazy_in=lazy_in)), ctx.handle,
          "pp_conv2d_nhwc_bwd_weight_bf16x3")


def maxpool3x3s2(ctx, n_img, h, w, c, x, oh, ow, y):
    check(lib.pp_maxpool3x3s2_fwd(ctx.handle, n_img, h, w, c, _ptr(x), oh, ow, _ptr(y)), ctx.handle, "pp_maxpool3x3s2_fwd")


def upsample_add_fwd(ctx, n_img, sh, sw, th, tw, c, src, other, out):
    check(lib.pp_upsample_nearest_add_fwd(ctx.handle, n_img, sh, sw, th, tw, c, _ptr(src), _ptr(other), _ptr(out)),
          ctx.handle, "pp_upsample_nearest_add_fwd")


def upsample_add_bwd(ctx, n_img, sh, sw, th, tw, c, dtarget, base, dsrc):
    check(lib.pp_upsample_nearest_add_bwd(ctx.handle, n_img, sh, sw, th, tw, c, _ptr(dtarget), _ptr(base), _ptr(dsrc)),
          ctx.handle, "pp_upsample_nearest_add_bwd")


def add_n(ctx, a, b, c, out):
    check(lib.pp_add_n(ctx.handle, a.numel(), _ptr(a), _ptr(b), _ptr(c), _ptr(out)), ctx.handle, "pp_add_n")


def relu_fwd(ctx, x, y):
    check(lib.pp_relu_fwd(ctx.handle, x.numel(), _ptr(x), _ptr(y)), ctx.handle, "pp_relu_fwd")


def warp_affine_u8(ctx, images_u8, matrices, interpolation="linear", border="replicate", cval=0, out=None):
    B, H, W = images_u8.shape[:3]
    ch = images_u8.shape[3] if images_u8.dim() == 4 else 1
    m = np.ascontiguousarray(np.asarray(matrices, np.float64).reshape(B, -1)[:, :6])
    if out is None:
        out = torch.empty_like(images_u8)
    check(lib.pp_warp_affine_u8(ctx.handle, B, H, W, ch, m.ctypes.data_as(C.POINTER(C.c_double)), {"nearest": 0, "linear": 1}[interpolation],
                                {"constant": 0, "replicate": 1}[border], int(cval), _ptr(images_u8), _ptr(out)), ctx.handle, "pp_warp_affine_u8")
    return out


def photo_augment_u8(ctx, images_u8, programs, out=None):
    if images_u8.dim() != 4:
        raise ValueError("photo_augment_u8: a [B,H,W,3] batch, got %s" % (tuple(images_u8.shape),))
    B, H, W, ch = images_u8.shape
    assert images_u8.dtype == torch.uint8 and images_u8.is_contiguous()
    if len(programs) != B:
        raise ValueError("photo_augment_u8: %d programs for %d images" % (len(programs), B))
    if out is None:
        out = torch.empty_like(images_u8)
    nbytes = int(programs.pool.size)
    pool_dev = programs.pinned_pool().to(images_u8.device, non_blocking=True)
    ws = torch.empty(lib.pp_photo_workspace_bytes(B, H, W), dtype=torch.uint8, device=images_u8.device)
    offs, recs = programs.op_offsets, programs.ops
    check(lib.pp_photo_augment_u8(ctx.handle, B, H, W, ch, offs.ctypes.data, recs.ctypes.data if recs.size else None,
                                  programs.pool.ctypes.data if nbytes else None, nbytes, _ptr(pool_dev), _ptr(images_u8), _ptr(out), _ptr(ws),
                                  ws.numel()), ctx.handle, "pp_photo_augment_u8")
    return out


def resize_scale(rows, cols, min_side=480, max_side=640):
    s = C.c_double(0)
    check(lib.pp_resize_scale(int(rows), int(cols), int(min_side), int(max_side), C.byref(s)), None, "pp_resize_scale")
    return s.value


def resize_linear_u8(ctx, images_u8, scale):
    B, H, W = images_u8.shape[:3]
    ch = images_u8.shape[3] if images_u8.dim() == 4 else 1
    dh, dw = int(np.rint(H * scale)), int(np.rint(W * scale))
    out = torch.empty((B, dh, dw) + ((ch,) if images_u8.dim() == 4 else ()), dtype=torch.uint8, device=images_u8.device)
    check(lib.pp_resize_linear_u8(ctx.handle, B, H, W, ch, float(scale), dh, dw, _ptr(images_u8), _ptr(out)), ctx.handle, "pp_resize_linear_u8")
    return out


def preprocess_caffe_u8(ctx, images_u8, sizes_hw, x4):
    Bn, H, W, _ = images_u8.shape
    assert images_u8.dtype == torch.uint8 and images_u8.is_contiguous()
    arr = (C.c_int * (2 * Bn))(*[int(v) for hw in sizes_hw for v in hw])
    check(lib.pp_preprocess_caffe_u8(ctx.handle, Bn, H, W, arr, _ptr(images_u8), _ptr(x4)), ctx.handle, "pp_preprocess_caffe_u8")

# ... 789 lines not shown
```

Measured before the change: 603.6.

## Merge stride-2 dgrad parity classes into a single kernel launch

Adds a merged stride-2 backward-data path. All four output parity classes are ordered by tap count and dispatched from one grid, and each workgroup picks its class from block-range offsets. Before, each class was launched separately with its own fill path. This cuts launch count and lets the class grids fill the GPU together, at the cost of per-block class lookup and no capture or skip support on this route. The engine selects it for stride-2 convs without capture or skip, when the library reports merging enabled and the planner does not refuse.

```diff
diff --git a/include/pyrapose_hip.h b/include/pyrapose_hip.h
--- a/include/pyrapose_hip.h
+++ b/include/pyrapose_hip.h
@@ -103,6 +103,11 @@
                                    const void* dy_lo, const void* w_dgrad_hi, const void* w_dgrad_lo,
                                    const float* addend, int ld_add, const float* relu_src, int ld_rs, float* dx,
                                    void* dx_hi, void* dx_lo, const pp_conv_opts* opts);
+int pp_conv2d_nhwc_bwd_data_s2_bf16x3(pp_ctx* ctx, const pp_conv_desc* d, const float* dy, const void* dy_hi,
+                                      const void* dy_lo, const void* w_dgrad_hi, const void* w_dgrad_lo,
+                                      const float* addend, int ld_add, const float* relu_src, int ld_rs, float* dx,
+                                      void* dx_hi, void* dx_lo, const pp_conv_opts* opts);
+int pp_conv_s2_merged(void);
 int pp_conv2d_nhwc_bwd_weight_bf16x3(pp_ctx* ctx, const pp_conv_desc* d, const float* x, const float* dy,
                                      const void* x_hi, const void* x_lo, const void* dy_hi, const void* dy_lo,
                                      float* dw, float* dbias, const pp_conv_opts* opts);
@@ -110,6 +115,7 @@
 #define PP_PLAN_FWD 0
 #define PP_PLAN_BWD_DATA 1
 #define PP_PLAN_BWD_WEIGHT 2
+#define PP_PLAN_BWD_DATA_S2 3
 #define PP_PLAN_PLANES_IN 1u
 #define PP_PLAN_PLANES_OUT 2u
 #define PP_PLAN_F32_OUT 4u
diff --git a/pyrapose_amd/_lib.py b/pyrapose_amd/_lib.py
--- a/pyrapose_amd/_lib.py
+++ b/pyrapose_amd/_lib.py
@@ -119,6 +119,8 @@
     "pp_conv_split_weights_bf16x3_batch": (_i, [_p, _i, _p, _i]),
     "pp_conv2d_nhwc_fwd_bf16x3": (_i, [_p, C.POINTER(ConvDesc), _p, _p, _p, _p, _p, _p, _p, _i, _i, _p, _p, _p, C.POINTER(ConvOpts)]),
     "pp_conv2d_nhwc_bwd_data_bf16x3": (_i, [_p, C.POINTER(ConvDesc), _p, _p, _p, _p, _p, _p, _i, _p, _i, _p, _p, _p, C.POINTER(ConvOpts)]),
+    "pp_conv2d_nhwc_bwd_data_s2_bf16x3": (_i, [_p, C.POINTER(ConvDesc), _p, _p, _p, _p, _p, _p, _i, _p, _i, _p, _p, _p, C.POINTER(ConvOpts)]),
+    "pp_conv_s2_merged": (_i, []),
     "pp_conv2d_nhwc_bwd_weight_bf16x3": (_i, [_p, C.POINTER(ConvDesc), _p, _p, _p, _p, _p, _p, _p, _p, C.POINTER(ConvOpts)]),
     "pp_conv_plan_text": (_i, [C.POINTER(ConvDesc), _i, C.c_uint, _i, _i, _sz, C.c_char_p, _i]),
     "pp_maxpool3x3s2_fwd": (_i, [_p, _i, _i, _i, _i, _p, _i, _i, _p]),
diff --git a/pyrapose_amd/csrc/conv3.hip b/pyrapose_amd/csrc/conv3.hip
--- a/pyrapose_amd/csrc/conv3.hip
+++ b/pyrapose_amd/csrc/conv3.hip
@@ -154,13 +154,13 @@
   epilogue3<TM, TN, OP>(p, acc, smem, m0, n0, tid, wm, wn, il, h, g_bias, g_addend, g_mask, g_out, g_ohi, g_olo);
 }
 
-template <int TM, int TN, bool AP, bool OP, bool SC = false, bool RL = false>
-__global__ __launch_bounds__(256, (TM * TN >= 8) ? 2 : ((TM * TN == 4) ? 3 : 4)) void igemm3f_kernel(
-    const IgemmParams p, const void* __restrict__ g_a0, const void* __restrict__ g_a1, unsigned a_bytes,
+template <int TM, int TN, bool AP, bool OP, bool SC, bool RL, bool MG>
+__device__ __forceinline__ void igemm3f_body(
+    const IgemmParams& p, const int bid, const int n_wg_in, const void* __restrict__ g_a0, const void* __restrict__ g_a1, unsigned a_bytes,
     const void* __restrict__ g_whi, const void* __restrict__ g_wlo, unsigned w_bytes,
     const float* __restrict__ g_bias, const float* __restrict__ g_addend, const float* __restrict__ g_mask,
     float* __restrict__ g_out, uint2* __restrict__ g_ohi, uint2* __restrict__ g_olo, int w_rows, int w_ld8, int splits,
-    float* __restrict__ g_ws, const int* __restrict__ g_rl = nullptr, const unsigned char* __restrict__ g_srcflags = nullptr) {
+    float* __restrict__ g_ws, const int* __restrict__ g_rl, const unsigned char* __restrict__ g_srcflags) {
   constexpr int BM = 64 * TM, BN = 64 * TN, BK = 32, NO = BK / 8;
   constexpr int SMEM_U4 = 2 * NO * (BM + BN);
   constexpr int ES = 4;
@@ -172,12 +172,12 @@
 
   const int tid = threadIdx.x, lane = tid & 63, wave = tid >> 6;
   const int wm = wave >> 1, wn = wave & 1;
-  int n_wg = (int)gridDim.x;
+  int n_wg = n_wg_in;
   if (RL) {
     n_wg = ((g_rl[0] + BM / 32 - 1) / (BM / 32)) * p.n_tiles_n * splits;
-    if ((int)blockIdx.x >= n_wg) return;
-  }
-  const int lbs = xcd_remap((int)blockIdx.x, n_wg);
+    if (bid >= n_wg) return;
+  }
+  const int lbs = xcd_remap(bid, n_wg);
   const int split = lbs % splits, lb = lbs / splits;
   const int tile_n = lb % p.n_tiles_n, tile_m = lb / p.n_tiles_n;
   const int m0 = tile_m * BM, n0 = tile_n * BN;
@@ -233,7 +233,7 @@
   uint4 rah[TM], ral[TM];
   uint4 rbh[TN], rbl[TN];
   int tap = s_begin / steps_per_tap, red0 = (s_begin - tap * steps_per_tap) * BK;
-  int ty = tap / p.kw, tx = tap - ty * p.kw;
+  int ty = tap / (MG ? max(p.kw, 1) : p.kw), tx = tap - ty * p.kw;
 
   auto load_step = [&]() {
     const int a_uni = tx * x_pitch + red0 * ES;
@@ -302,9 +302,11 @@
 
   const int il = lane & 31, h = lane >> 5;
 
-  load_step();
-  split_step();
-  store_step();
+  if (!MG || s_begin < s_end) {
+    load_step();
+    split_step();
+    store_step();
+  }
   __syncthreads();
 
   for (int step = s_begin; step < s_end; ++step) {
@@ -335,6 +337,34 @@
     return;
   }
   epilogue3<TM, TN, OP, PP_EPI_GF, SC, false, RL>(p, acc, smem, m0, n0, tid, wm, wn, il, h, g_bias, g_addend, g_mask, g_out, g_ohi, g_olo, rl_blk);
+}
+
+template <int TM, int TN, bool AP, bool OP, bool SC = false, bool RL = false>
+__global__ __launch_bounds__(256, (TM * TN >= 8) ? 2 : ((TM * TN == 4) ? 3 : 4)) void igemm3f_kernel(
+    const IgemmParams p, const void* __restrict__ g_a0, const void* __restrict__ g_a1, unsigned a_bytes,
+    const void* __restrict__ g_whi, const void* __restrict__ g_wlo, unsigned w_bytes,
+    const float* __restrict__ g_bias, const float* __restrict__ g_addend, const float* __restrict__ g_mask,
+    float* __restrict__ g_out, uint2* __restrict__ g_ohi, uint2* __restrict__ g_olo, int w_rows, int w_ld8, int splits,
+    float* __restrict__ g_ws, const int* __restrict__ g_rl = nullptr, const unsigned char* __restrict__ g_srcflags = nullptr) {
+  igemm3f_body<TM, TN, AP, OP, SC, RL, false>(p, (int)blockIdx.x, (int)gridDim.x, g_a0, g_a1, a_bytes, g_whi, g_wlo, w_bytes, g_bias, g_addend,
+                                              g_mask, g_out, g_ohi, g_olo, w_rows, w_ld8, splits, g_ws, g_rl, g_srcflags);
+}
+
+template <int TM, int TN, bool AP, bool OP>
+__global__ __launch_bounds__(256, (TM * TN >= 8) ? 2 : ((TM * TN == 4) ? 3 : 4)) void igemm3m_kernel(
+    const IgemmParams p0, const PpS2Merged g, const void* __restrict__ g_a0, const void* __restrict__ g_a1, unsigned a_bytes,
+    const void* __restrict__ g_whi, const void* __restrict__ g_wlo, unsigned w_bytes, const float* __restrict__ g_addend,
+    const float* __restrict__ g_mask, float* __restrict__ g_out, uint2* __restrict__ g_ohi, uint2* __restrict__ g_olo, int w_rows, int w_ld8) {
+  const int bid = (int)blockIdx.x;
+  PpS2Class c = g.c[0];
+#pragma unroll
+  for (int j = 1; j < 4; ++j)
+    if (j < g.n_cls && bid >= g.c[j].blk_begin) c = g.c[j];
+  IgemmParams p = p0;
+  p.n_seg = 1;
+  igemm_set_class(p, c);
+  igemm3f_body<TM, TN, AP, OP, true, false, true>(p, bid - c.blk_begin, c.tiles, g_a0, g_a1, a_bytes, g_whi, g_wlo, w_bytes, nullptr, g_addend, g_mask,
+                                                  g_out, g_ohi, g_olo, w_rows, w_ld8, 1, nullptr, nullptr, nullptr);
 }
 
 template <int TM, int TN, bool CAP, bool AP = false, bool OP = false>
@@ -1320,6 +1350,27 @@
   else launch_igemm3<1, 1>(ctx->stream, p, a, pl);
 }
 
+template <int TM, int TN>
+static void launch_igemm3m(hipStream_t st, IgemmParams& p, const Igemm3Args& a, const DgradS2Route& r) {
+  const dim3 grid(r.g.grid), wg(256);
+  const unsigned a_bytes = (unsigned)(p.src_rows * (long long)p.ld_src * 4), w_bytes = (unsigned)((long long)p.w_taps * a.w_rows * a.w_ld8 * 16);
+  p.n_tiles_n = r.pl.n_tiles_n;
+  if (a.ahi)
+    hipLaunchKernelGGL((igemm3m_kernel<TM, TN, true, true>), grid, wg, 0, st, p, r.g, a.ahi, a.alo, a_bytes, a.whi, a.wlo, w_bytes, p.addend, p.mask_src,
+                       p.out, (uint2*)a.ohi, (uint2*)a.olo, a.w_rows, a.w_ld8);
+  else
+    hipLaunchKernelGGL((igemm3m_kernel<TM, TN, false, false>), grid, wg, 0, st, p, r.g, (const void*)p.src, nullptr, a_bytes, a.whi, a.wlo, w_bytes,
+                       p.addend, p.mask_src, p.out, (uint2*)nullptr, (uint2*)nullptr, a.w_rows, a.w_ld8);
+}
+static void dispatch3m(pp_ctx* ctx, IgemmParams& p, const Igemm3Args& a, const DgradS2Route& r) {
+  pp_plan_debug(r.f, r.pl, r.g);
+  if (r.pl.tm == 4) launch_igemm3m<4, 2>(ctx->stream, p, a, r);
+  else if (r.pl.tm == 2 && r.pl.tn == 2) launch_igemm3m<2, 2>(ctx->stream, p, a, r);
+  else if (r.pl.tm == 1 && r.pl.tn == 2) launch_igemm3m<1, 2>(ctx->stream, p, a, r);
+  else if (r.pl.tm == 2 && r.pl.tn == 1) launch_igemm3m<2, 1>(ctx->stream, p, a, r);
+  else launch_igemm3m<1, 1>(ctx->stream, p, a, r);
+}
+
 static void dispatch3_rowlist(pp_ctx* ctx, IgemmParams& p, const Igemm3Args& a, int tm, const unsigned char* dy_flags, unsigned char* out_flags,
                               int* out_list, bool fill) {
   PpIgemmFacts f = igemm3_facts(ctx, p, a);
@@ -1431,40 +1482,40 @@
 }
 namespace {
 
-}
-extern "C" int PP_API(pp_conv2d_nhwc_bwd_data_bf16x3)(pp_ctx* ctx, const pp_conv_desc* d, const float* dy, const void* dy_hi, const void* dy_lo,
-                                              const void* w_hi, const void* w_lo, const float* addend, int ld_add,
-                                              const float* relu_src, int ld_rs, float* dx, void* dx_hi, void* dx_lo,
-                                              const pp_conv_opts* opts) {
+static int bwd_data_impl(pp_ctx* ctx, const char* who, bool merged, const pp_conv_desc* d, const float* dy, const void* dy_hi, const void* dy_lo,
+                         const void* w_hi, const void* w_lo, const float* addend, int ld_add, const float* relu_src, int ld_rs, float* dx,
+                         void* dx_hi, void* dx_lo, const pp_conv_opts* opts) {
   PP_REQUIRE_CTX(ctx);
-  int rc = pp_conv_opts_take(ctx, opts, PP_OPT_CAPTURE | PP_OPT_ADD | PP_OPT_MASK | PP_OPT_SKIP | PP_OPT_LAZY_OUT | PP_OPT_LAZY_IN,
-                             "pp_conv2d_nhwc_bwd_data_bf16x3");
+  int rc = pp_conv_opts_take(ctx, opts,
+                             merged ? (PP_OPT_ADD | PP_OPT_MASK)
+                                    : (PP_OPT_CAPTURE | PP_OPT_ADD | PP_OPT_MASK | PP_OPT_SKIP | PP_OPT_LAZY_OUT | PP_OPT_LAZY_IN),
+                             who);
   if (rc) return rc;
   void *const chi = opts->capture_hi, *const clo = opts->capture_lo;
   unsigned char* const skip_flags = opts->skip_flags;
   const bool skip_scratch_ok = skip_flags != nullptr && opts->skip_list != nullptr;
   const void *const ep_ah = opts->add_hi, *const ep_al = opts->add_lo, *const ep_mh = opts->mask_hi;
-  rc = check_desc(ctx, d, "pp_conv2d_nhwc_bwd_data_bf16x3");
+  rc = check_desc(ctx, d, who);
   PP_CHECK_ARG(ctx, !(ep_ah && addend) && !(ep_mh && relu_src), PP_ERR_ARG,
-               "pp_conv2d_nhwc_bwd_data_bf16x3: addend / relu_src given both as f32 and as planes");
+               "%s: addend / relu_src given both as f32 and as planes", who);
   PP_CHECK_ARG(ctx, (!ep_ah || (ld_add >= d->cin && ld_add % 4 == 0)) && (!ep_mh || (ld_rs >= d->cin && ld_rs % 4 == 0)), PP_ERR_SHAPE,
-               "pp_conv2d_nhwc_bwd_data_bf16x3: addend / relu_src planes");
+               "%s: addend / relu_src planes", who);
   if (rc) return rc;
-  PP_CHECK_ARG(ctx, !chi || (dy && !dy_hi && pp_is_packed(chi, clo)), PP_ERR_ARG, "pp_conv2d_nhwc_bwd_data_bf16x3: split capture needs the f32 operand");
-  PP_CHECK_ARG(ctx, (dy || (dy_hi && dy_lo)) && w_hi && w_lo && (dx || (dx_hi && dx_lo)), PP_ERR_ARG, "pp_conv2d_nhwc_bwd_data_bf16x3: null tensor");
-  PP_CHECK_ARG(ctx, (dy_hi == nullptr) == (dy_lo == nullptr) && d->ld_y % 8 == 0, PP_ERR_ARG, "pp_conv2d_nhwc_bwd_data_bf16x3: planes / ld_y");
+  PP_CHECK_ARG(ctx, !chi || (dy && !dy_hi && pp_is_packed(chi, clo)), PP_ERR_ARG, "%s: split capture needs the f32 operand", who);
+  PP_CHECK_ARG(ctx, (dy || (dy_hi && dy_lo)) && w_hi && w_lo && (dx || (dx_hi && dx_lo)), PP_ERR_ARG, "%s: null tensor", who);
+  PP_CHECK_ARG(ctx, (dy_hi == nullptr) == (dy_lo == nullptr) && d->ld_y % 8 == 0, PP_ERR_ARG, "%s: planes / ld_y", who);
   PP_CHECK_ARG(ctx, pp_is_packed(dy_hi, dy_lo) && pp_is_packed(dx_hi, dx_lo), PP_ERR_ALIGN,
-               "pp_conv2d_nhwc_bwd_data_bf16x3: planes must be packed (lo = hi + 16 bytes, 16-byte aligned)");
+               "%s: planes must be packed (lo = hi + 16 bytes, 16-byte aligned)", who);
   PP_CHECK_ARG(ctx, (!dx_hi || (d->cin % 8 == 0 && d->ld_x % 8 == 0)) && (!ep_ah || ld_add % 8 == 0) && (!ep_mh || ld_rs % 8 == 0), PP_ERR_SHAPE,
-               "pp_conv2d_nhwc_bwd_data_bf16x3: planes need channel counts and leading dimensions %% 8 == 0");
+               "%s: planes need channel counts and leading dimensions %% 8 == 0", who);
   const int cred = (d->cout + 31) / 32 * 32;
   PP_CHECK_ARG(ctx, d->cin % 16 == 0 && d->ld_y >= cred && d->ld_y % 4 == 0, PP_ERR_SHAPE,
-               "pp_conv2d_nhwc_bwd_data_bf16x3: dy needs ld_y >= %d (cout rounded up to 32, zero padded)", cred);
+               "%s: dy needs ld_y >= %d (cout rounded up to 32, zero padded)", who, cred);
   PP_CHECK_ARG(ctx, (!dy || pp_is_aligned16(dy)) && pp_is_aligned16(w_hi) && pp_is_aligned16(w_lo) && (!dx || pp_is_aligned16(dx)), PP_ERR_ALIGN,
-               "pp_conv2d_nhwc_bwd_data_bf16x3: tensors must be 16-byte aligned");
+               "%s: tensors must be 16-byte aligned", who);
   PP_CHECK_ARG(ctx, (!addend || (ld_add >= d->cin && ld_add % 4 == 0 && pp_is_aligned16(addend))) &&
                         (!relu_src || (ld_rs >= d->cin && ld_rs % 4 == 0 && pp_is_aligned16(relu_src))),
-               PP_ERR_SHAPE, "pp_conv2d_nhwc_bwd_data_bf16x3: addend / relu_src");
+               PP_ERR_SHAPE, "%s: addend / relu_src", who);
   IgemmParams p;
   memset(&p, 0, sizeof(p));
   p.src = dy; p.out = dx; p.bias = nullptr; p.addend = addend; p.mask_src = relu_src;
@@ -1473,13 +1524,24 @@
   p.ld_add = ld_add; p.ld_mask = ld_rs;
   p.relu = 0;
   PP_CHECK_ARG(ctx, (dx_hi == nullptr) == (dx_lo == nullptr) && (!dx_hi || (d->ld_x % 4 == 0 && pp_is_aligned16(dx_hi) && pp_is_aligned16(dx_lo))),
-               PP_ERR_ARG, "pp_conv2d_nhwc_bwd_data_bf16x3: output planes");
+               PP_ERR_ARG, "%s: output planes", who);
   const Igemm3Args a = {dy_hi, dy_lo, w_hi, w_lo, d->cin, cred / 8, dx_hi, dx_lo, chi, clo, skip_flags, ctx->ws};
+  if (merged) {
+    DgradS2Route s2;
+    dgrad_s2_route(d, p, igemm3_facts(ctx, p, a), &s2);
+    PP_CHECK_ARG(ctx, s2.ok, PP_ERR_ARG,
+                 "%s: needs stride 2, one level, operands all float32 or all planes, and classes the branch-free loop can run "
+                 "(pp_conv2d_nhwc_bwd_data_bf16x3 takes every other call)", who);
+    IgemmParams q = s2.cls[0];
+    dispatch3m(ctx, q, a, s2);
+    PP_CHECK_LAUNCH(ctx, who);
+    return PP_OK;
+  }
   DgradRoute route;
   dgrad_route(d, p, igemm3_facts(ctx, p, a), skip_scratch_ok, &route);
   PP_CHECK_ARG(ctx, !opts->lazy_in || route.listed, PP_ERR_ARG,
-               "pp_conv2d_nhwc_bwd_data_bf16x3: dy was declared lazy (unwritten outside its flagged blocks) but the listed-block launch "
-               "does not apply to this call");
+               "%s: dy was declared lazy (unwritten outside its flagged blocks) but the listed-block launch "
+               "does not apply to this call", who);
   const int nb = (p.M + 31) / 32;
   if (skip_scratch_ok && !route.listed) PP_HIP(ctx, hipMemsetAsync(skip_flags + nb, 1, (size_t)nb, ctx->stream));
   const Igemm3Args ac = {dy_hi, dy_lo, w_hi, w_lo, d->cin, cred / 8, dx_hi, dx_lo, nullptr, nullptr, nullptr, ctx->ws};
@@ -1494,8 +1556,23 @@
         hipLaunchKernelGGL(class_fill_kernel, dim3(pp_finish_blocks(q.M, q.Nout, pp_cus(ctx->n_cu))), dim3(256), 0, ctx->stream, q, addend, relu_src,
                            dx, dx_hi, dx_lo);
       });
-  PP_CHECK_LAUNCH(ctx, "pp_conv2d_nhwc_bwd_data_bf16x3");
+  PP_CHECK_LAUNCH(ctx, who);
   return PP_OK;
+}
+}
+extern "C" int PP_API(pp_conv2d_nhwc_bwd_data_bf16x3)(pp_ctx* ctx, const pp_conv_desc* d, const float* dy, const void* dy_hi, const void* dy_lo,
+                                              const void* w_hi, const void* w_lo, const float* addend, int ld_add,
+                                              const float* relu_src, int ld_rs, float* dx, void* dx_hi, void* dx_lo,
+                                              const pp_conv_opts* opts) {
+  return bwd_data_impl(ctx, "pp_conv2d_nhwc_bwd_data_bf16x3", false, d, dy, dy_hi, dy_lo, w_hi, w_lo, addend, ld_add, relu_src, ld_rs, dx, dx_hi,
+                       dx_lo, opts);
+}
+extern "C" int PP_API(pp_conv2d_nhwc_bwd_data_s2_bf16x3)(pp_ctx* ctx, const pp_conv_desc* d, const float* dy, const void* dy_hi, const void* dy_lo,
+                                                 const void* w_hi, const void* w_lo, const float* addend, int ld_add,
+                                                 const float* relu_src, int ld_rs, float* dx, void* dx_hi, void* dx_lo,
+                                                 const pp_conv_opts* opts) {
+  return bwd_data_impl(ctx, "pp_conv2d_nhwc_bwd_data_s2_bf16x3", true, d, dy, dy_hi, dy_lo, w_hi, w_lo, addend, ld_add, relu_src, ld_rs, dx,
+                       dx_hi, dx_lo, opts);
 }
 namespace {
 
diff --git a/pyrapose_amd/csrc/conv3_dispatch.hip b/pyrapose_amd/csrc/conv3_dispatch.hip
--- a/pyrapose_amd/csrc/conv3_dispatch.hip
+++ b/pyrapose_amd/csrc/conv3_dispatch.hip
@@ -25,7 +25,9 @@
 extern "C" int pp_stem7x7s2_fwd_bf16x3_fmt0(pp_ctx* ctx, int n_img, int H, int W, int Hp, int Wp, const float* x4p, const void* w_hi, const void* w_lo, int cout, const float* bias, int relu, float* y, int ld_y);
 extern "C" int pp_stem7x7s2_fwd_bf16x3_fmt1(pp_ctx* ctx, int n_img, int H, int W, int Hp, int Wp, const float* x4p, const void* w_hi, const void* w_lo, int cout, const float* bias, int relu, float* y, int ld_y);
 extern "C" int pp_conv2d_nhwc_bwd_data_bf16x3_fmt0(pp_ctx* ctx, const pp_conv_desc* d, const float* dy, const void* dy_hi, const void* dy_lo, const void* w_dgrad_hi, const void* w_dgrad_lo, const float* addend, int ld_add, const float* relu_src, int ld_rs, float* dx, void* dx_hi, void* dx_lo, const pp_conv_opts* opts);
+extern "C" int pp_conv2d_nhwc_bwd_data_s2_bf16x3_fmt0(pp_ctx* ctx, const pp_conv_desc* d, const float* dy, const void* dy_hi, const void* dy_lo, const void* w_dgrad_hi, const void* w_dgrad_lo, const float* addend, int ld_add, const float* relu_src, int ld_rs, float* dx, void* dx_hi, void* dx_lo, const pp_conv_opts* opts);
 extern "C" int pp_conv2d_nhwc_bwd_data_bf16x3_fmt1(pp_ctx* ctx, const pp_conv_desc* d, const float* dy, const void* dy_hi, const void* dy_lo, const void* w_dgrad_hi, const void* w_dgrad_lo, const float* addend, int ld_add, const float* relu_src, int ld_rs, float* dx, void* dx_hi, void* dx_lo, const pp_conv_opts* opts);
+extern "C" int pp_conv2d_nhwc_bwd_data_s2_bf16x3_fmt1(pp_ctx* ctx, const pp_conv_desc* d, const float* dy, const void* dy_hi, const void* dy_lo, const void* w_dgrad_hi, const void* w_dgrad_lo, const float* addend, int ld_add, const float* relu_src, int ld_rs, float* dx, void* dx_hi, void* dx_lo, const pp_conv_opts* opts);
 extern "C" int pp_conv2d_nhwc_bwd_weight_bf16x3_fmt0(pp_ctx* ctx, const pp_conv_desc* d, const float* x, const float* dy, const void* x_hi, const void* x_lo, const void* dy_hi, const void* dy_lo, float* dw, float* dbias, const pp_conv_opts* opts);
 extern "C" int pp_conv2d_nhwc_bwd_weight_bf16x3_fmt1(pp_ctx* ctx, const pp_conv_desc* d, const float* x, const float* dy, const void* x_hi, const void* x_lo, const void* dy_hi, const void* dy_lo, float* dw, float* dbias, const pp_conv_opts* opts);
 
@@ -68,13 +70,18 @@
 extern "C" int pp_conv2d_nhwc_bwd_data_bf16x3(pp_ctx* ctx, const pp_conv_desc* d, const float* dy, const void* dy_hi, const void* dy_lo, const void* w_dgrad_hi, const void* w_dgrad_lo, const float* addend, int ld_add, const float* relu_src, int ld_rs, float* dx, void* dx_hi, void* dx_lo, const pp_conv_opts* opts) {
   return (ctx && ctx->planes_fmt == 1) ? pp_conv2d_nhwc_bwd_data_bf16x3_fmt1(ctx, d, dy, dy_hi, dy_lo, w_dgrad_hi, w_dgrad_lo, addend, ld_add, relu_src, ld_rs, dx, dx_hi, dx_lo, opts) : pp_conv2d_nhwc_bwd_data_bf16x3_fmt0(ctx, d, dy, dy_hi, dy_lo, w_dgrad_hi, w_dgrad_lo, addend, ld_add, relu_src, ld_rs, dx, dx_hi, dx_lo, opts);
 }
+extern "C" int pp_conv2d_nhwc_bwd_data_s2_bf16x3(pp_ctx* ctx, const pp_conv_desc* d, const float* dy, const void* dy_hi, const void* dy_lo, const void* w_dgrad_hi, const void* w_dgrad_lo, const float* addend, int ld_add, const float* relu_src, int ld_rs, float* dx, void* dx_hi, void* dx_lo, const pp_conv_opts* opts) {
+  return (ctx && ctx->planes_fmt == 1) ? pp_conv2d_nhwc_bwd_data_s2_bf16x3_fmt1(ctx, d, dy, dy_hi, dy_lo, w_dgrad_hi, w_dgrad_lo, addend, ld_add, relu_src, ld_rs, dx, dx_hi, dx_lo, opts) : pp_conv2d_nhwc_bwd_data_s2_bf16x3_fmt0(ctx, d, dy, dy_hi, dy_lo, w_dgrad_hi, w_dgrad_lo, addend, ld_add, relu_src, ld_rs, dx, dx_hi, dx_lo, opts);
+}
 extern "C" int pp_conv2d_nhwc_bwd_weight_bf16x3(pp_ctx* ctx, const pp_conv_desc* d, const float* x, const float* dy, const void* x_hi, const void* x_lo, const void* dy_hi, const void* dy_lo, float* dw, float* dbias, const pp_conv_opts* opts) {
   return (ctx && ctx->planes_fmt == 1) ? pp_conv2d_nhwc_bwd_weight_bf16x3_fmt1(ctx, d, x, dy, x_hi, x_lo, dy_hi, dy_lo, dw, dbias, opts) : pp_conv2d_nhwc_bwd_weight_bf16x3_fmt0(ctx, d, x, dy, x_hi, x_lo, dy_hi, dy_lo, dw, dbias, opts);
 }
 
+extern "C" int pp_conv_s2_merged(void) { return pp_sw_s2_merged() ? 1 : 0; }
+
 extern "C" int pp_conv_plan_text(const pp_conv_desc* d, int pass, unsigned forms, int planes_fmt, int n_cu, size_t ws_bytes, char* buf,
                                  int buf_bytes) {
-  if (!buf || buf_bytes <= 0 || pass < PP_PLAN_FWD || pass > PP_PLAN_BWD_WEIGHT) return PP_ERR_ARG;
+  if (!buf || buf_bytes <= 0 || pass < PP_PLAN_FWD || pass > PP_PLAN_BWD_DATA_S2) return PP_ERR_ARG;
   const int rc = check_desc(nullptr, d, "pp_conv_plan_text");
   if (rc) return rc;
   const bool planes_in = forms & PP_PLAN_PLANES_IN, planes_out = forms & PP_PLAN_PLANES_OUT, f32_out = (forms & PP_PLAN_F32_OUT) || !planes_out,
@@ -107,6 +114,13 @@
   igemm_geometry_bwd_data(nullptr, d, p);
   const int w_rows = d->cin, w_ld8 = p.Cred / 8;
   const PpIgemmFacts f = igemm_facts(p, w_rows, w_ld8, planes_in, !planes_in, planes_out, f32_out, capture, list, n_cu, ws, (long long)ws_bytes);
+  if (pass == PP_PLAN_BWD_DATA_S2) {
+    DgradS2Route s2;
+    s2.ok = false;
+    if (!(forms & (PP_PLAN_LIST | PP_PLAN_LAZY_IN | PP_PLAN_LAZY_OUT))) dgrad_s2_route(d, p, f, &s2);
+    if (!s2.ok) return pp_plan_append(buf, buf_bytes, at, "igemm3 s2 refused: not a stride-2, one-level, all-f32 or all-planes data gradient\n");
+    return pp_plan_print(buf, buf_bytes, at, s2.f, s2.pl, s2.g, true);
+  }
   DgradRoute route;
   dgrad_route(d, p, f, list, &route);
   if (lazy_in && !route.listed) return pp_plan_append(buf, buf_bytes, at, "igemm3 refused: lazy dy without a listed-block launch\n");
diff --git a/pyrapose_amd/csrc/conv_common.h b/pyrapose_amd/csrc/conv_common.h
--- a/pyrapose_amd/csrc/conv_common.h
+++ b/pyrapose_amd/csrc/conv_common.h
@@ -232,24 +232,25 @@
   return f;
 }
 
+__host__ __device__ __forceinline__ void igemm_set_class(IgemmParams& r, const PpS2Class& c) {
+  r.kh = c.kh; r.kw = c.kw;
+  r.off_y = c.off_y; r.off_x = c.off_x;
+  r.w_ty0 = c.w_ty0; r.w_tx0 = c.w_tx0;
+  r.seg[0].OH = c.OH; r.seg[0].OW = c.OW;
+  r.M = c.M;
+  r.sc_cy = c.cy; r.sc_cx = c.cx;
+}
 static bool igemm_parity_classes(const pp_conv_desc* d, const IgemmParams& p, bool all_planes, IgemmParams cls[4]) {
   const int H = d->in.h[0], W = d->in.w[0];
+  PpS2Class geo[4];
+  pp_s2_classes(d->in.n_img, H, W, d->kh, d->kw, d->pad_t, d->pad_l, geo);
   for (int c = 0; c < 4; ++c) {
-    const int cy = c >> 1, cx = c & 1;
     IgemmParams& r = cls[c];
     r = p;
     r.div = 1;
-    const int ty0 = (cy + d->pad_t) & 1, tx0 = (cx + d->pad_l) & 1;
-    r.kh = ty0 < d->kh ? (d->kh - ty0 + 1) / 2 : 0;
-    r.kw = tx0 < d->kw ? (d->kw - tx0 + 1) / 2 : 0;
-    r.off_y = (cy + d->pad_t - ty0) / 2;
-    r.off_x = (cx + d->pad_l - tx0) / 2;
-    r.w_ty0 = ty0; r.w_tx0 = tx0; r.w_tstep = 2; r.w_kw = d->kw;
-    if (r.kh == 0 || r.kw == 0) r.kh = r.kw = 0;
-    r.seg[0].OH = (H - cy + 1) / 2;
-    r.seg[0].OW = (W - cx + 1) / 2;
-    r.M = d->in.n_img * r.seg[0].OH * r.seg[0].OW;
-    r.sc_on = 1; r.sc_H = H; r.sc_W = W; r.sc_cy = cy; r.sc_cx = cx;
+    r.w_tstep = 2; r.w_kw = d->kw;
+    igemm_set_class(r, geo[c]);
+    r.sc_on = 1; r.sc_H = H; r.sc_W = W;
     if (r.M > 0 && r.kh > 0 &&
         !(pp_igemm_fast_ok(igemm_facts(r, d->cin, r.Cred / 8, all_planes, !all_planes, all_planes, !all_planes, false, false, 0, false, 0)) && r.M < (1 << 24)))
       return false;
@@ -276,6 +277,30 @@
   r->listed_tm = pp_conv_switches().sparse_dgrad == 22 ? 2 : 1;
   r->classes = pp_dgrad_classes_ok(rf) && igemm_parity_classes(d, p, all_planes, r->cls);
 }
+struct DgradS2Route {
+  bool ok;
+  IgemmParams cls[4];
+  PpIgemmFacts f;
+  PpIgemmPlan pl;
+  PpS2Merged g;
+};
+static void dgrad_s2_route(const pp_conv_desc* d, const IgemmParams& p, const PpIgemmFacts& f_all, DgradS2Route* r) {
+  const bool all_f32 = f_all.f32_in && f_all.f32_out && !f_all.planes_in && !f_all.planes_out,
+             all_planes = f_all.planes_in && f_all.planes_out && !f_all.f32_out;
+  const PpDgradRouteFacts rf = {d->stride, d->kh, d->kw, d->pad_t, d->pad_l, d->in.n_seg, all_f32, all_planes, f_all.capture, p.bias != nullptr,
+                                f_all.flags, false, pp_igemm_fast_ok(f_all), f_all.same_grid};
+  r->ok = pp_dgrad_s2_ok(rf) && !f_all.capture && !f_all.flags && igemm_parity_classes(d, p, all_planes, r->cls);
+  if (!r->ok) return;
+  PpS2Class geo[4];
+  pp_s2_classes(d->in.n_img, d->in.h[0], d->in.w[0], d->kh, d->kw, d->pad_t, d->pad_l, geo);
+  const PpS2Merged order = pp_s2_merge(geo, 64, 64, p.Nout);
+  const IgemmParams& heavy = r->cls[2 * order.c[0].cy + order.c[0].cx];
+  r->f = igemm_facts(heavy, f_all.w_rows, f_all.w_ld8, all_planes, !all_planes, all_planes, !all_planes, false, false, f_all.n_cu, f_all.ws,
+                     f_all.ws_bytes);
+  r->pl = pp_plan_igemm(r->f);
+  r->g = pp_s2_merge(geo, 64 * r->pl.tm, 64 * r->pl.tn, p.Nout);
+  r->ok = r->pl.family == PP_IGEMM3F_CLASS && r->pl.splits == 1 && order.c[0].kh > 0;
+}
 template <class Gemm, class Fill>
 static void dgrad_launches(DgradRoute& r, IgemmParams& p, Gemm gemm, Fill fill) {
   if (!r.classes) {
diff --git a/pyrapose_amd/csrc/conv_plan.h b/pyrapose_amd/csrc/conv_plan.h
--- a/pyrapose_amd/csrc/conv_plan.h
+++ b/pyrapose_amd/csrc/conv_plan.h
@@ -55,6 +55,7 @@
 inline int pp_sw_conv4p_nst() { const char* e = getenv("PP_CONV4P_NST"); return e && atoi(e) == 3 ? 3 : 4; }
 inline int pp_sw_conv4p_splits() { return pp_env_int("PP_CONV4P_SPLITS", 0); }
 inline bool pp_sw_wgrad_det() { return pp_env_is1("PP_WGRAD3_DETERMINISTIC"); }
+inline bool pp_sw_s2_merged() { return pp_env_not0("PP_CONV3_S2MERGED"); }
 inline int pp_sw_wgrad3r() { const char* e = getenv("PP_WGRAD3R"); return !e ? -1 : ((e[0] == '1' || e[0] == '2') ? e[0] - '0' : 0); }
 inline bool pp_sw_tile(const char* name, char* a, char* b) {
   const char* e = getenv(name);
@@ -103,11 +104,11 @@
 
 enum PpIgemmFamily {
   PP_IGEMM3, PP_IGEMM3F, PP_IGEMM3F_CLASS, PP_IGEMM3X_CAPTURE, PP_IGEMM3X_PP, PP_IGEMM3X_PF, PP_IGEMM3X_FP, PP_IGEMM3X_FF, PP_IGEMM4X,
-  PP_IGEMM4X2, PP_IGEMM4P, PP_IGEMM3F_LIST
+  PP_IGEMM4X2, PP_IGEMM4P, PP_IGEMM3F_LIST, PP_IGEMM3F_S2
 };
 static const char* const pp_igemm_family_name[] = {
     "igemm3", "igemm3f", "igemm3f[parity class]", "igemm3x[capture]", "igemm3x[planes->planes]", "igemm3x[planes->f32]",
-    "igemm3x[f32->planes]", "igemm3x[f32->f32]", "igemm4x", "igemm4x<NWM=2>", "igemm4p", "igemm3f[row list]"};
+    "igemm3x[f32->planes]", "igemm3x[f32->f32]", "igemm4x", "igemm4x<NWM=2>", "igemm4p", "igemm3f[row list]", "igemm3f[stride-2 merged]"};
 
 struct PpIgemmPlan {
   int family;
@@ -328,6 +329,57 @@
   return r.stride == 2 && pp_conv_switches().s2_classes && (r.all_f32 || r.all_planes) && r.n_seg == 1;
 }
 
+struct PpS2Class {
+  int cy, cx;
+  int kh, kw;
+  int off_y, off_x, w_ty0, w_tx0;
+  int OH, OW, M;
+  int tiles, blk_begin;
+};
+inline void pp_s2_classes(int n_img, int H, int W, int kh, int kw, int pad_t, int pad_l, PpS2Class cls[4]) {
+  for (int c = 0; c < 4; ++c) {
+    PpS2Class& r = cls[c];
+    r.cy = c >> 1;
+    r.cx = c & 1;
+    const int ty0 = (r.cy + pad_t) & 1, tx0 = (r.cx + pad_l) & 1;
+    r.kh = ty0 < kh ? (kh - ty0 + 1) / 2 : 0;
+    r.kw = tx0 < kw ? (kw - tx0 + 1) / 2 : 0;
+    r.off_y = (r.cy + pad_t - ty0) / 2;
+    r.off_x = (r.cx + pad_l - tx0) / 2;
+    r.w_ty0 = ty0;
+    r.w_tx0 = tx0;
+    if (r.kh == 0 || r.kw == 0) r.kh = r.kw = 0;
+    r.OH = (H - r.cy + 1) / 2;
+    r.OW = (W - r.cx + 1) / 2;
+    r.M = n_img * r.OH * r.OW;
+    r.tiles = r.blk_begin = 0;
+  }
+}
+struct PpS2Merged {
+  int n_cls;
+  unsigned grid;
+  PpS2Class c[4];
+};
+inline PpS2Merged pp_s2_merge(const PpS2Class cls[4], int BM, int BN, int Nout) {
+  PpS2Merged g = {};
+  for (int c = 0; c < 4; ++c) {
+    if (cls[c].M <= 0) continue;
+    int at = g.n_cls++;
+    for (; at > 0 && g.c[at - 1].kh * g.c[at - 1].kw < cls[c].kh * cls[c].kw; --at) g.c[at] = g.c[at - 1];
+    g.c[at] = cls[c];
+  }
+  const long long ntn = (Nout + BN - 1) / BN;
+  long long at = 0;
+  for (int i = 0; i < g.n_cls; ++i) {
+    g.c[i].tiles = (int)(((g.c[i].M + BM - 1) / BM) * ntn);
+    g.c[i].blk_begin = (int)at;
+    at += g.c[i].tiles;
+  }
+  g.grid = (unsigned)at;
+  return g;
+}
+inline bool pp_dgrad_s2_ok(const PpDgradRouteFacts& r) { return r.stride == 2 && (r.all_f32 || r.all_planes) && r.n_seg == 1; }
+
 struct PpWgradFacts {
   int M, Cin, Cout, kh, kw, stride, pad_t, pad_l, ld_src, ld_dy, ld_w;
   long long src_rows;
@@ -521,6 +573,17 @@
                         pl.finish_blocks, pl.ws_need);
   return pp_plan_append(buf, cap, at, "\n");
 }
+inline int pp_plan_print(char* buf, int cap, int at, const PpIgemmFacts& f, const PpIgemmPlan& pl, const PpS2Merged& g, bool detail) {
+  at = pp_plan_append(buf, cap, at, "igemm3 s2 N %d -> tile %dx%d, %d classes:", f.Nout, 64 * pl.tm, 64 * pl.tn, g.n_cls);
+  for (int i = 0; i < g.n_cls; ++i)
+    at = pp_plan_append(buf, cap, at, " (%d,%d) M %d steps %d", g.c[i].cy, g.c[i].cx, g.c[i].M, g.c[i].kh * g.c[i].kw * (f.Cred / 32));
+  at = pp_plan_append(buf, cap, at, " %s", pp_igemm_family_name[PP_IGEMM3F_S2]);
+  if (detail) {
+    at = pp_plan_append(buf, cap, at, " | grid=%u n_tiles_n=%d class_grids=", g.grid, pl.n_tiles_n);
+    for (int i = 0; i < g.n_cls; ++i) at = pp_plan_append(buf, cap, at, i ? "+%d" : "%d", g.c[i].tiles);
+  }
+  return pp_plan_append(buf, cap, at, "\n");
+}
 template <class Facts, class Plan>
 inline void pp_plan_debug(const Facts& f, const Plan& pl) {
   if (!pp_sw_debug()) return;
@@ -528,3 +591,9 @@
   pp_plan_print(line, (int)sizeof(line), 0, f, pl, false);
   fputs(line, stderr);
 }
+inline void pp_plan_debug(const PpIgemmFacts& f, const PpIgemmPlan& pl, const PpS2Merged& g) {
+  if (!pp_sw_debug()) return;
+  char line[512];
+  pp_plan_print(line, (int)sizeof(line), 0, f, pl, g, false);
+  fputs(line, stderr);
+}
diff --git a/pyrapose_amd/engine.py b/pyrapose_amd/engine.py
--- a/pyrapose_amd/engine.py
+++ b/pyrapose_amd/engine.py
@@ -305,6 +305,7 @@
             self.prefix_lane = len(self.streams) - 1
         self.acts = OrderedDict()
         self._plane_grads = []
+        self._s2_grads = []
         self.step_count = 0
         self._build_forward()
         self.levels = arch.level_shapes(self.H, self.W, arch.PYRAMID_LEVELS[pyramid])
@@ -771,11 +772,23 @@
                     m_t, m_hi = (mask.t, None) if mask.t is not None else (None, mask.pl[0])
                 if gcap is not None:
                     assert dy_t is not None
-                self.bwd_ops.append(Op(lambda d=op["desc"], dy_t=dy_t, dy_pl=dy_pl, dh=pl["dg_hi"], dl=pl["dg_lo"], a_t=a_t, a_pl=a_pl, m_t=m_t,
-                                       m_hi=m_hi, out=out, gcap=gcap, sk=sk, lazy_out=lazy_out, lazy_in=lazy_in:
-                                       ops.conv_bwd_data3(ctx, d, dy_t, dh, dl, a_t, m_t, out.t, dy_pl, out.pl, gcap, sk, a_pl, m_hi,
-                                                          lazy_out=lazy_out, lazy_in=lazy_in), "conv_dgrad",
-                                       op["spec"].name, op["flops"]))
+                forms = (ops.PLAN_PLANES_IN if dy_pl is not None else 0) | (ops.PLAN_PLANES_OUT if out.pl is not None else 0) | \
+                        (ops.PLAN_F32_OUT if out.t is not None else 0)
+                if (op["desc"].stride == 2 and gcap is None and sk is None and ops.conv_s2_merged()
+                        and "refused" not in ops.conv_plan_text(op["desc"], ops.PLAN_BWD_DATA_S2, forms, act.fmt)):
+                    self.bwd_ops.append(Op(lambda d=op["desc"], dy_t=dy_t, dy_pl=dy_pl, dh=pl["dg_hi"], dl=pl["dg_lo"], a_t=a_t, a_pl=a_pl, m_t=m_t,
+                                           m_hi=m_hi, out=out:
+                                           ops.conv_bwd_data3_s2(ctx, d, dy_t, dh, dl, a_t, m_t, out.t, dy_pl, out.pl, a_pl, m_hi), "conv_dgrad",
+                                           op["spec"].name, op["flops"]))
+                    self._s2_grads.append((op["spec"].name, out, "merged"))
+                else:
+                    if op["desc"].stride == 2:
+                        self._s2_grads.append((op["spec"].name, out, "classes"))
+                    self.bwd_ops.append(Op(lambda d=op["desc"], dy_t=dy_t, dy_pl=dy_pl, dh=pl["dg_hi"], dl=pl["dg_lo"], a_t=a_t, a_pl=a_pl, m_t=m_t,
+                                           m_hi=m_hi, out=out, gcap=gcap, sk=sk, lazy_out=lazy_out, lazy_in=lazy_in:
+                                           ops.conv_bwd_data3(ctx, d, dy_t, dh, dl, a_t, m_t, out.t, dy_pl, out.pl, gcap, sk, a_pl, m_hi,
+                                                              lazy_out=lazy_out, lazy_in=lazy_in), "conv_dgrad",
+                                           op["spec"].name, op["flops"]))
                 out.within = sk[0][sk[0].numel() // 2:] if (sk is not None and acc is None and _os.environ.get("PP_SPARSE_WITHIN", "1") != "0") else None
                 out.lazy = lazy_out
                 assert not lazy_out or out.within is not None
diff --git a/pyrapose_amd/ops.py b/pyrapose_amd/ops.py
--- a/pyrapose_amd/ops.py
+++ b/pyrapose_amd/ops.py
@@ -85,7 +85,7 @@
     return d
 
 
-PLAN_FWD, PLAN_BWD_DATA, PLAN_BWD_WEIGHT = 0, 1, 2
+PLAN_FWD, PLAN_BWD_DATA, PLAN_BWD_WEIGHT, PLAN_BWD_DATA_S2 = 0, 1, 2, 3
 PLAN_PLANES_IN, PLAN_PLANES_OUT, PLAN_F32_OUT, PLAN_CAPTURE, PLAN_LIST, PLAN_LAZY_IN, PLAN_LAZY_OUT = 1, 2, 4, 8, 16, 32, 64
 
 
@@ -315,6 +315,21 @@
                                              _conv_opts(capture=dy_capture, add=addend_planes, mask_hi=relu_src_hi, skip=dy_skip,
                                                         lazy_out=lazy_out, lazy_in=lazy_in)), ctx.handle,
           "pp_conv2d_nhwc_bwd_data_bf16x3")
+
+
+def conv_bwd_data3_s2(ctx, d, dy, w_hi, w_lo, addend, relu_src, dx, dy_planes=None, dx_planes=None, addend_planes=None, relu_src_hi=None):
+    ld_add = addend.stride(0) if addend is not None else (planes_ld(addend_planes) if addend_planes is not None else 0)
+    ld_rs = relu_src.stride(0) if relu_src is not None else (relu_src_hi.stride(0) // 2 if relu_src_hi is not None else 0)
+    dh, dl = dy_planes if dy_planes is not None else (None, None)
+    xh, xl = dx_planes if dx_planes is not None else (None, None)
+    check(lib.pp_conv2d_nhwc_bwd_data_s2_bf16x3(ctx.handle, C.byref(d), _ptr(dy), _ptr(dh), _ptr(dl), _ptr(w_hi), _ptr(w_lo), _ptr(addend),
+                                                ld_add, _ptr(relu_src), ld_rs, _ptr(dx), _ptr(xh), _ptr(xl),
+                                                _conv_opts(add=addend_planes, mask_hi=relu_src_hi)), ctx.handle,
+          "pp_conv2d_nhwc_bwd_data_s2_bf16x3")
+
+
+def conv_s2_merged():
+    return bool(lib.pp_conv_s2_merged())
 
 
 def conv_bwd_weight3(ctx, d, x, dy, dw, dbias, x_planes=None, dy_planes=None, dy_skip=None, lazy_in=False):
```

Measured after the change: 611.6, median of 6. 1.01x the previous value.
